# emilk/field_interpolation

Measured on NVIDIA B200. Metric: 3D SDF solve: lattice cells x CG iterations per second, higher is better.
Workload: dtype f32

## Files before the change

field_interpolation_b200/_lib.py:

```python
from __future__ import annotations

import ctypes as C
import os

HERE = os.path.dirname(os.path.abspath(__file__))
LIB_PATH = os.path.join(HERE, "libfi_b200.so")

FI_OK, FI_ERR_INVALID, FI_ERR_CUDA, FI_ERR_RANGE, FI_ERR_UNSUPPORTED, FI_ERR_COMM = range(6)
FI_HOST, FI_DEVICE = 0, 1
FI_F32, FI_F64, FI_MIXED = 0, 1, 2
FI_PRECOND_JACOBI, FI_PRECOND_MULTIGRID = 0, 1


class FiError(RuntimeError):
    def __init__(self, code, text):
        super().__init__(f"libfi_b200 status {code}: {text}")
        self.code = code


class fi_weights(C.Structure):
    _fields_ = [(n, C.c_float) for n in ("data_pos", "data_gradient", "model_0", "model_1", "model_2", "model_3",
                                         "model_4", "gradient_smoothness")] + [("value_kernel", C.c_int32),
                                                                               ("gradient_kernel", C.c_int32)]


class fi_triplet(C.Structure):
    _fields_ = [("row", C.c_int32), ("col", C.c_int32), ("value", C.c_float)]


class fi_solve_options(C.Structure):
    _fields_ = [("precision", C.c_int32), ("max_iterations", C.c_int32), ("tolerance", C.c_double),
                ("check_every", C.c_int32), ("use_fast_stencil", C.c_int32), ("refine_max_outer", C.c_int32),
                ("refine_inner_tolerance", C.c_double), ("preconditioner", C.c_int32), ("mg_smoothing_steps", C.c_int32),
                ("mg_cheb_ratio", C.c_double)]


class fi_solve_stats(C.Structure):
    _fields_ = [("iterations", C.c_int64), ("relative_residual", C.c_double), ("true_residual", C.c_double),
                ("initial_residual", C.c_double), ("setup_ms", C.c_double), ("solve_ms", C.c_double),
                ("converged", C.c_int32), ("outer_sweeps", C.c_int32), ("occupied_cells", C.c_int64),
                ("generic_rows", C.c_int64), ("widened_after", C.c_int64)]

    def as_dict(self):
        return {n: getattr(self, n) for n, _ in self._fields_}


class fi_cascade_options(C.Structure):
    _fields_ = [("fine", fi_solve_options), ("factor", C.c_int32), ("coarsest_size", C.c_int32),
                ("coarse_tolerance", C.c_double), ("max_levels", C.c_int32)]


class fi_cascade_stats(C.Structure):
    _fields_ = [("levels", C.c_int32), ("level_cells", C.c_int64 * 16), ("level_iterations", C.c_int64 * 16),
                ("level_ms", C.c_double * 16), ("level_initial_residual", C.c_double * 16), ("total_ms", C.c_double),
                ("cell_iterations", C.c_int64), ("finest", fi_solve_stats)]

    def as_dict(self):
        L = self.levels
        return {"levels": L, "level_cells": list(self.level_cells[:L]), "level_iterations": list(self.level_iterations[:L]),
                "level_ms": list(self.level_ms[:L]), "level_initial_residual": list(self.level_initial_residual[:L]),
                "total_ms": self.total_ms, "cell_iterations": self.cell_iterations, "finest": self.finest.as_dict()}


_p = C.POINTER
_vp, _i32, _i64, _f, _d = C.c_void_p, C.c_int32, C.c_int64, C.c_float, C.c_double
_pf, _pi32, _pi64, _pd = _p(C.c_float), _p(C.c_int32), _p(C.c_int64), _p(C.c_double)

SIGNATURES = {
    "fi_abi_version": (C.c_int, []),
    "fi_last_error": (C.c_char_p, []),
    "fi_device_count": (C.c_int, [_pi32]),
    "fi_set_device": (C.c_int, [_i32]),
    "fi_weights_default": (None, [_p(fi_weights)]),
    "fi_solve_options_default": (None, [_p(fi_solve_options)]),
    "fi_field_create": (C.c_int, [_i32, _pi32, _p(_vp)]),
    "fi_field_destroy": (C.c_int, [_vp]),
    "fi_field_clone": (C.c_int, [_vp, _p(_vp)]),
    "fi_field_add_model": (C.c_int, [_vp, _p(fi_weights)]),
    "fi_field_add_points": (C.c_int, [_vp, _f, _i32, _f, _i32, _i64, _vp, _vp, _vp, _vp, _i32, _pi64]),
    "fi_field_add_rows": (C.c_int, [_vp, _i64, _i64, _pi32, _pi32, _pf, _pf]),
    "fi_sdf_from_points": (C.c_int, [_i32, _pi32, _p(fi_weights), _i64, _vp, _vp, _vp, _i32, _p(_vp)]),
    "fi_field_counts": (C.c_int, [_vp, _pi64, _pi64]),
    "fi_field_export": (C.c_int, [_vp, _vp, _vp]),
    "fi_field_export_rows": (C.c_int, [_vp, _i64, _vp, _vp]),
    "fi_field_apply": (C.c_int, [_vp, _i32, _vp, _vp]),
    "fi_field_use_fast_stencil": (C.c_int, [_vp, _i32]),
    "fi_field_rhs": (C.c_int, [_vp, _i32, _vp]),
    "fi_field_diagonal": (C.c_int, [_vp, _i32, _vp]),
    "fi_field_solve": (C.c_int, [_vp, _p(fi_solve_options), _vp, _vp, _i32, _p(fi_solve_stats)]),
    "fi_field_solve_tiled": (C.c_int, [_vp, _p(fi_solve_options), _i32, _i32, _i32, _vp, _vp, _i32, _p(fi_solve_stats), _p(fi_solve_stats)]),
    "fi_field_jacobi": (C.c_int, [_vp, _pf, _i32, _f, _pf]),
    "fi_upscale_field": (C.c_int, [_i32, _pi32, _pi32, _vp, _vp, _i32]),
    "fi_error_map": (C.c_int, [_i64, _vp, _i64, _pf, _i64, _pf, _pf]),
    "fi_marching_squares": (C.c_int, [_i32, _i32, _vp, _f, _i32, _vp, _i64, _pi64, _pf]),
    "fi_calc_area": (C.c_int, [_i64, _vp, _i32, _pf]),
    "fi_bicubic_upsample": (C.c_int, [_i32, _i32, _vp, _i32, _vp, _i32]),
    "fi_sdf_solve_cascade": (C.c_int, [_i32, _pi32, _p(fi_weights), _i64, _vp, _vp, _vp, _p(fi_cascade_options), _vp, _i32,
                                       _p(fi_cascade_stats)]),
    "fi_comm_unique_id": (C.c_int, [_vp, _i64]),
    "fi_comm_create": (C.c_int, [_i32, _i32, _vp, _p(_vp)]),
    "fi_comm_destroy": (C.c_int, [_vp]),
    "fi_slab_balanced_cuts": (C.c_int, [_pi32, _i32, _i64, _vp, _i32, _d, _i32, _pi32]),
    "fi_comm_set_slab_cuts": (C.c_int, [_vp, _i32, _pi32]),
    "fi_slab_range": (C.c_int, [_i32, _i32, _i32, _pi32, _pi32]),
    "fi_slab_mg_plan": (C.c_int, [_pi32, _i32, _i32, _i64, _pi32, _pi32, _pi32, _pi32]),
    "fi_slab_sdf_solve": (C.c_int, [_vp, _pi32, _p(fi_weights), _i64, _vp, _vp, _vp, _i32, _p(fi_solve_options), _vp, _vp, _i32,
                                    _p(fi_solve_stats)]),
    "fi_trim_memory": (C.c_int, []),
    "fi_cached_bytes": (_i64, []),
    "fi_kernel_launches": (_i64, []),
    "fi_kernel_launches_reset": (None, []),
    "fi_field_time_iterations": (C.c_int, [_vp, _p(fi_solve_options), _i32, _pd]),
}

_dll = None


def lib():
    global _dll
    if _dll is None:
        if not os.path.exists(LIB_PATH):
            raise FiError(FI_ERR_CUDA, f"{LIB_PATH} not built; run python -m field_interpolation_b200.build "
                                       "(or __graft_entry__.build())")
        dll = C.CDLL(LIB_PATH)
        for name, (res, args) in SIGNATURES.items():
            fn = getattr(dll, name)
            fn.restype, fn.argtypes = res, args
        _dll = dll
    return _dll


def check(status):
    if status != FI_OK:
        raise FiError(status, lib().fi_last_error().decode("utf-8", "replace"))
```

field_interpolation_b200/api.py:

```python
from __future__ import annotations

import ctypes as C
import math
from dataclasses import dataclass, field as dc_field
from typing import Optional, Sequence

import numpy as np

from . import _lib as L
from ._lib import (FI_DEVICE, FI_F32, FI_F64, FI_HOST, FI_MIXED, FI_PRECOND_JACOBI, FI_PRECOND_MULTIGRID,
                   FiError)


class ValueKernel:
    kNearestNeighbor = 0
    kLinearInterpolation = 1


class GradientKernel:
    kNearestNeighbor = 0
    kCellEdges = 1
    kLinearInterpolation = 2


@dataclass
class Weights:
    data_pos: float = 1.0
    data_gradient: float = 1.0
    model_0: float = 0.0
    model_1: float = 0.0
    model_2: float = 0.5
    model_3: float = 0.0
    model_4: float = 0.0
    gradient_smoothness: float = 0.0
    value_kernel: int = ValueKernel.kLinearInterpolation
    gradient_kernel: int = GradientKernel.kCellEdges

    def c(self) -> L.fi_weights:
        return L.fi_weights(self.data_pos, self.data_gradient, self.model_0, self.model_1, self.model_2, self.model_3,
                            self.model_4, self.gradient_smoothness, int(self.value_kernel), int(self.gradient_kernel))


@dataclass
class SolveOptions:
    tile: bool = False
    tile_size: int = 16
    cg: bool = True
    max_iterations: int = 0
    error_tolerance: float = 1e-3


@dataclass
class LinearEquation:
    rows: np.ndarray
    cols: np.ndarray
    vals: np.ndarray
    rhs: np.ndarray

    @property
    def num_rows(self):
        return int(self.rhs.shape[0])

    @property
    def num_triplets(self):
        return int(self.vals.shape[0])


def _is_device(a) -> bool:
    return hasattr(a, "data_ptr") and bool(getattr(a, "is_cuda", False))


def _f32_host(a):
    return np.ascontiguousarray(a, dtype=np.float32)


class _Buf:

    def __init__(self, a, n_expected: Optional[int] = None):
        self.keep, self.ptr, self.loc = None, None, None
        if a is None:
            return
        if _is_device(a):
            import torch
            assert a.dtype == torch.float32 and a.is_contiguous(), "device inputs must be contiguous float32"
            self.keep, self.ptr, self.loc, n = a, C.c_void_p(a.data_ptr()), FI_DEVICE, a.numel()
        else:
            h = _f32_host(a)
            self.keep, self.ptr, self.loc, n = h, C.c_void_p(h.ctypes.data), FI_HOST, h.size
        if n_expected is not None and n != n_expected:
            raise ValueError(f"expected {n_expected} floats, got {n}")


def _common_loc(bufs):
    locs = {b.loc for b in bufs if b.loc is not None}
    if len(locs) > 1:
        raise ValueError("all point arrays must live in the same place (all host or all device)")
    return locs.pop() if locs else FI_HOST


def solve_options(precision=FI_F32, max_iterations=0, tolerance=1e-3, check_every=32, use_fast_stencil=True,
                  refine_max_outer=20, refine_inner_tolerance=1e-3, preconditioner=FI_PRECOND_JACOBI, mg_smoothing_steps=0,
                  mg_cheb_ratio=12.0) -> L.fi_solve_options:
    return L.fi_solve_options(int(precision), int(max_iterations), float(tolerance), int(check_every),
                              int(use_fast_stencil), int(refine_max_outer), float(refine_inner_tolerance), int(preconditioner),
                              int(mg_smoothing_steps), float(mg_cheb_ratio))


class LatticeField:

    def __init__(self, sizes: Sequence[int], _handle=None):
        self.sizes = [int(s) for s in sizes]
        self.strides = []
        s = 1
        for n in self.sizes:
            self.strides.append(s)
            s *= n
        self.num_unknowns = s
        if _handle is None:
            h = C.c_void_p()
            sz = (C.c_int32 * len(self.sizes))(*self.sizes)
            L.check(L.lib().fi_field_create(len(self.sizes), sz, C.byref(h)))
            _handle = h
        self._h = _handle

    def num_dim(self):
        return len(self.sizes)

    def close(self):
        if getattr(self, "_h", None):
            L.lib().fi_field_destroy(self._h)
            self._h = None

    def __del__(self):
        try:
            self.close()
        except Exception:
            pass

    def counts(self):
        r, t = C.c_int64(0), C.c_int64(0)
        L.check(L.lib().fi_field_counts(self._h, C.byref(r), C.byref(t)))
        return int(r.value), int(t.value)

    @property
    def eq(self) -> LinearEquation:
        nr, nt = self.counts()
        trips = np.empty(nt, dtype=np.dtype([("row", np.int32), ("col", np.int32), ("value", np.float32)]))
        rhs = np.empty(nr, np.float32)
        L.check(L.lib().fi_field_export(self._h, C.c_void_p(trips.ctypes.data), C.c_void_p(rhs.ctypes.data)))
        return LinearEquation(trips["row"].copy(), trips["col"].copy(), trips["value"].copy(), rhs)

    def _vec(self, fn, precision):
        out = np.empty(self.num_unknowns, np.float32 if precision == FI_F32 else np.float64)
        L.check(fn(self._h, precision, C.c_void_p(out.ctypes.data)))
        return out

    def rhs(self, precision=FI_F64):
        return self._vec(L.lib().fi_field_rhs, precision)

    def diagonal(self, precision=FI_F64):
        return self._vec(L.lib().fi_field_diagonal, precision)

    def use_fast_stencil(self, mode):
        L.check(L.lib().fi_field_use_fast_stencil(self._h, int(mode)))

    def apply(self, x, precision=FI_F64):
        dt = np.float32 if precision == FI_F32 else np.float64
        xi = np.ascontiguousarray(x, dtype=dt)
        assert xi.size == self.num_unknowns
        y = np.empty_like(xi)
        L.check(L.lib().fi_field_apply(self._h, precision, C.c_void_p(xi.ctypes.data), C.c_void_p(y.ctypes.data)))
        return y

    def solve(self, options: Optional[L.fi_solve_options] = None, guess=None, out=None):
        opt = options if options is not None else solve_options()
        g = _Buf(guess, self.num_unknowns)
        if out is None:
            if g.loc == FI_DEVICE:
                import torch
                out = torch.empty(self.num_unknowns, dtype=torch.float32, device=guess.device)
            else:
                out = np.empty(self.num_unknowns, np.float32)
        o = _Buf(out, self.num_unknowns)
        if g.loc is not None and g.loc != o.loc:
            raise ValueError("guess and out must live in the same place")
        st = L.fi_solve_stats()
        L.check(L.lib().fi_field_solve(self._h, C.byref(opt), g.ptr, o.ptr, o.loc, C.byref(st)))
        return (out if _is_device(out) else o.keep), st.as_dict()

    def time_iterations(self, iterations: int, options: Optional[L.fi_solve_options] = None):
        opt = options if options is not None else solve_options()
        ms = (C.c_double * 8)()
        L.check(L.lib().fi_field_time_iterations(self._h, C.byref(opt), int(iterations), ms))
        return {"iteration_ms": ms[0], "apply_ms": ms[1], "update_ms": ms[2], "direction_ms": ms[3], "fused": bool(ms[4]),
                "stencil_ms": ms[5], "data_term_ms": ms[6]}



def add_field_constraints(field: LatticeField, weights: Weights) -> None:
    w = weights.c()
    L.check(L.lib().fi_field_add_model(field._h, C.byref(w)))


def add_points(field: LatticeField, value_weight: float, value_kernel: int, gradient_weight: float, gradient_kernel: int,
               positions, normals=None, point_weights=None, values=None) -> int:
    D = field.num_dim()
    p = _Buf(positions)
    n = (p.keep.numel() if p.loc == FI_DEVICE else p.keep.size) // D if p.keep is not None else 0
    nr, pw, va = _Buf(normals, n * D if normals is not None else None), _Buf(point_weights, n if point_weights is not None else None), _Buf(values, n if values is not None else None)
    loc = _common_loc([p, nr, pw, va])
    added = C.c_int64(0)
    L.check(L.lib().fi_field_add_points(field._h, float(value_weight), int(value_kernel), float(gradient_weight),
                                        int(gradient_kernel), n, p.ptr, nr.ptr, pw.ptr, va.ptr, loc, C.byref(added)))
    return int(added.value)


def add_value_constraint(field: LatticeField, pos, value: float, weight: float) -> bool:
    return add_points(field, weight, ValueKernel.kLinearInterpolation, 0.0, GradientKernel.kCellEdges,
                      np.asarray(pos, np.float32).reshape(1, -1), None, None, np.asarray([value], np.float32)) > 0


def _round_half_away(x: float) -> int:
    return int(math.floor(abs(x) + 0.5) * (1 if x >= 0 else -1))


def add_value_constraint_nearest_neighbor(field: LatticeField, pos, gradient, value: float, weight: float) -> bool:
    p = np.asarray(pos, np.float32).reshape(-1)
    inside = all(0 <= _round_half_away(float(p[d])) < field.sizes[d] for d in range(field.num_dim()))
    if not inside:
        return False
    add_points(field, weight, ValueKernel.kNearestNeighbor, 0.0, GradientKernel.kCellEdges, p.reshape(1, -1),
               np.asarray(gradient, np.float32).reshape(1, -1), None, np.asarray([value], np.float32))
    return True


def add_gradient_constraint(field: LatticeField, pos, gradient, weight: float, kernel: int) -> bool:
    if kernel not in (0, 1, 2):
        raise FiError(L.FI_ERR_INVALID, f"Unknown gradient kernel: {kernel}")
    return add_points(field, 0.0, ValueKernel.kLinearInterpolation, weight, kernel,
                      np.asarray(pos, np.float32).reshape(1, -1), np.asarray(gradient, np.float32).reshape(1, -1)) > 0


def add_equation(field: LatticeField, weight: float, rhs: float, pairs) -> None:
    w = np.float32(weight)
    if w == 0:
        return
    cols = [int(c) for c, v in pairs if np.float32(v) != 0]
    vals = np.array([np.float32(v) * w for c, v in pairs if np.float32(v) != 0], np.float32)
    if not cols:
        return
    r = np.zeros(len(cols), np.int32)
    c = np.asarray(cols, np.int32)
    b = np.array([np.float32(rhs) * w], np.float32)
    L.check(L.lib().fi_field_add_rows(field._h, 1, len(cols), r.ctypes.data_as(L._pi32), c.ctypes.data_as(L._pi32),
                                      vals.ctypes.data_as(L._pf), b.ctypes.data_as(L._pf)))


def add_rows(field: LatticeField, trip_row, trip_col, trip_val, rhs) -> None:
    r, c = np.ascontiguousarray(trip_row, np.int32), np.ascontiguousarray(trip_col, np.int32)
    v, b = _f32_host(trip_val), _f32_host(rhs)
    L.check(L.lib().fi_field_add_rows(field._h, b.size, v.size, r.ctypes.data_as(L._pi32), c.ctypes.data_as(L._pi32),
                                      v.ctypes.data_as(L._pf), b.ctypes.data_as(L._pf)))


def sdf_from_points(sizes: Sequence[int], weights: Weights, positions, normals=None, point_weights=None) -> LatticeField:
    D = len(sizes)
    p = _Buf(positions)
    if p.keep is None:
        raise FiError(L.FI_ERR_INVALID, "positions is null")
    n = (p.keep.numel() if p.loc == FI_DEVICE else p.keep.size) // D
    nr, pw = _Buf(normals, n * D if normals is not None else None), _Buf(point_weights, n if point_weights is not None else None)
    loc = _common_loc([p, nr, pw])
    h = C.c_void_p()
    sz = (C.c_int32 * D)(*[int(s) for s in sizes])
    w = weights.c()
    L.check(L.lib().fi_sdf_from_points(D, sz, C.byref(w), n, p.ptr, nr.ptr, pw.ptr, loc, C.byref(h)))
    return LatticeField(sizes, _handle=h)


def upscale_field(small_field, small_sizes: Sequence[int], large_sizes: Sequence[int]):
    D = len(small_sizes)
    ss, ls = (C.c_int32 * D)(*map(int, small_sizes)), (C.c_int32 * D)(*map(int, large_sizes))
    src = _Buf(small_field, int(np.prod(small_sizes, dtype=np.int64)))
    nl = int(np.prod(large_sizes, dtype=np.int64))
    if src.loc == FI_DEVICE:
        import torch
        out = torch.empty(nl, dtype=torch.float32, device=small_field.device)
        dst = C.c_void_p(out.data_ptr())
    else:
        out = np.empty(nl, np.float32)
        dst = C.c_void_p(out.ctypes.data)
    L.check(L.lib().fi_upscale_field(D, ss, ls, src.ptr, dst, src.loc))
    return out


def _field_2d(values):
    shape = tuple(values.shape)
    if len(shape) != 2:
        raise ValueError("a 2D (height, width) field is expected")
    if _is_device(values):
        values = values.contiguous()
    return _Buf(values, shape[0] * shape[1]), int(shape[0]), int(shape[1])


def iso_surface(values, iso: float = 0.0, want_area: bool = False):
    buf, h, w = _field_2d(values)
    n = C.c_int64(0)
    L.check(L.lib().fi_marching_squares(w, h, buf.ptr, float(iso), buf.loc, None, 0, C.byref(n), None))
    ns = int(n.value)
    area = C.c_float(0.0)
    if buf.loc == FI_DEVICE:
        import torch
        out = torch.empty((ns, 4), dtype=torch.float32, device=values.device)
        dst = C.c_void_p(out.data_ptr()) if ns else None
# ... 113 lines not shown
```

field_interpolation_b200/csrc/abi.cu:

```cuda
#include <time.h>

#include <algorithm>
#include <cmath>
#include <cstdlib>
#include <exception>
#include <map>
#include <mutex>
#include <new>

#include "solver.hpp"

namespace fi {

int64_t                   g_launches = 0;
static thread_local std::string t_last_error;

void set_last_error(const std::string& s) { t_last_error = s; }

int sm_count()
{
	static thread_local int cached_dev = -1, cached = 0;
	int dev = 0;
	if (cudaGetDevice(&dev) != cudaSuccess) { return 148; }
	if (dev != cached_dev) {
// ... 697 lines not shown
}

int fi_field_counts(fi_field* f, int64_t* num_rows, int64_t* num_triplets)
{
	return guarded([&] {
		FI_REQUIRE(f != nullptr, FI_ERR_INVALID, "field is null");
		int64_t r = 0, t = 0;
		for (Segment& sg : f->segs) {
			segment_counts(f, sg);
			r += sg.rows;
			t += sg.trips;
		}
		if (num_rows) { *num_rows = r; }
		if (num_triplets) { *num_triplets = t; }
	});
}

static void export_impl(fi_field* f, int64_t row_begin, fi_triplet* triplets, float* rhs)
{
	FI_REQUIRE(f != nullptr, FI_ERR_INVALID, "field is null");
	FI_REQUIRE(row_begin >= 0, FI_ERR_INVALID, "negative row_begin");
	int64_t R = 0, T = 0;
	for (Segment& sg : f->segs) {
		segment_counts(f, sg);
		R += sg.rows;
		T += sg.trips;
	}
	FI_REQUIRE(R <= INT32_MAX && T <= INT32_MAX && f->g.N <= INT32_MAX, FI_ERR_RANGE,
	           "system does not fit the reference's int32 triplet view");
	size_t  first = 0;
	int64_t row_base = 0, trip_base = 0;
	while (first < f->segs.size() && row_base < row_begin) {
		row_base += f->segs[first].rows;
		trip_base += f->segs[first].trips;
		++first;
	}
	FI_REQUIRE(row_base == row_begin || (first == f->segs.size() && row_begin == R), FI_ERR_INVALID,
	           "row_begin is not a boundary between builder calls");
	const int64_t outR = R - row_base, outT = T - trip_base;
	if (outR == 0 && outT == 0) { return; }
	FI_REQUIRE((triplets || outT == 0) && (rhs || outR == 0), FI_ERR_INVALID, "output buffers are null");
	cudaStream_t       s = f->stream;
	DevBuf<fi_triplet> d_trips(std::max<int64_t>(outT, 1));
	DevBuf<float>      d_rhs(std::max<int64_t>(outR, 1));
	const int64_t      row0 = row_base, trip0 = trip_base;
	fi_triplet*        dt = d_trips.data() - trip0;
	float*             dr = d_rhs.data() - row0;
	for (size_t k = first; k < f->segs.size(); ++k) {
		Segment& sg = f->segs[k];
		if (sg.kind == Segment::kModel) {
			DevBuf<uint64_t> ro(f->g.N), to(f->g.N);
			uint64_t         hr = 0, ht = 0;
			count_model_rows(f->g, sg.w, ro.data(), to.data(), &hr, &ht, s);
			FI_REQUIRE(static_cast<int64_t>(hr) == sg.rows && static_cast<int64_t>(ht) == sg.trips, FI_ERR_INVALID,
			           "internal: model row count mismatch");
			emit_model_rows(f->g, sg.w, ro.data(), to.data(), row_base, trip_base, dt, dr, s);
			FI_CUDA(cudaStreamSynchronize(s));
		} else if (sg.kind == Segment::kPoints) {
			const int64_t    n = sg.p1 - sg.p0;
			DevBuf<uint64_t> ro(std::max<int64_t>(n, 1)), to(std::max<int64_t>(n, 1));
			uint64_t         hr = 0, ht = 0;
			count_point_rows(f->g, view(f->pts), sg.p0, sg.p1, ro.data(), to.data(), &hr, &ht, s);
			emit_point_rows(f->g, view(f->pts), sg.p0, sg.p1, ro.data(), to.data(), row_base, trip_base, dt, dr, s);
			FI_CUDA(cudaStreamSynchronize(s));
		} else {
			std::vector<fi_triplet> ht(static_cast<size_t>(sg.trips));
			size_t                  at = 0;
			for (int64_t r = sg.r0; r < sg.r1; ++r) {
				for (uint64_t kk = f->rows.ptr[r]; kk < f->rows.ptr[r + 1]; ++kk) {
					ht[at++] = fi_triplet{static_cast<int32_t>(row_base + (r - sg.r0)), f->rows.col[kk], f->rows.val[kk]};
				}
			}
			if (!ht.empty()) {
				FI_CUDA(cudaMemcpyAsync(dt + trip_base, ht.data(), ht.size() * sizeof(fi_triplet), cudaMemcpyHostToDevice, s));
			}
			if (sg.rows > 0) {
				FI_CUDA(cudaMemcpyAsync(dr + row_base, f->rows.rhs.data() + sg.r0, sg.rows * sizeof(float), cudaMemcpyHostToDevice, s));
			}
			FI_CUDA(cudaStreamSynchronize(s));
		}
		row_base += sg.rows;
		trip_base += sg.trips;
	}
	if (outT > 0) { FI_CUDA(cudaMemcpyAsync(triplets, d_trips.data(), outT * sizeof(fi_triplet), cudaMemcpyDeviceToHost, s)); }
	if (outR > 0) { FI_CUDA(cudaMemcpyAsync(rhs, d_rhs.data(), outR * sizeof(float), cudaMemcpyDeviceToHost, s)); }
	FI_CUDA(cudaStreamSynchronize(s));
}

int fi_field_export(fi_field* f, fi_triplet* triplets, float* rhs)
{
	return guarded([&] { export_impl(f, 0, triplets, rhs); });
}

int fi_field_export_rows(fi_field* f, int64_t row_begin, fi_triplet* triplets, float* rhs)
{
	return guarded([&] { export_impl(f, row_begin, triplets, rhs); });
}

int fi_field_use_fast_stencil(fi_field* f, int32_t enable)
{
	return guarded([&] {
		FI_REQUIRE(f != nullptr, FI_ERR_INVALID, "field is null");
		f->fast = enable;
	});
}

int fi_field_apply(fi_field* f, int32_t precision, const void* x, void* y)
{
	return guarded([&] {
		FI_REQUIRE(f && x && y, FI_ERR_INVALID, "null argument");
		const int64_t N = f->g.N;
		cudaStream_t  s = f->stream;
		if (precision == FI_F32) {
			Operator<float>& op = f->get32();
			op.use_fast = f->fast;
			DevBuf<float>    dx(N), dy(N);
			FI_CUDA(cudaMemcpyAsync(dx.data(), x, N * sizeof(float), cudaMemcpyHostToDevice, s));
			op.apply(dx.data(), dy.data(), nullptr, nullptr, s);
			FI_CUDA(cudaMemcpyAsync(y, dy.data(), N * sizeof(float), cudaMemcpyDeviceToHost, s));
		} else if (precision == FI_F64) {
			Operator<double>& op = f->get64();
			op.use_fast = f->fast;
			DevBuf<double>    dx(N), dy(N);
			FI_CUDA(cudaMemcpyAsync(dx.data(), x, N * sizeof(double), cudaMemcpyHostToDevice, s));
			op.apply(dx.data(), dy.data(), nullptr, nullptr, s);
			FI_CUDA(cudaMemcpyAsync(y, dy.data(), N * sizeof(double), cudaMemcpyDeviceToHost, s));
		} else {
			throw Error{FI_ERR_INVALID, "precision must be FI_F32 or FI_F64"};
		}
		FI_CUDA(cudaStreamSynchronize(s));
	});
}

static int copy_vector(fi_field* f, int32_t precision, void* out, int which)
{
	return guarded([&] {
		FI_REQUIRE(f && out, FI_ERR_INVALID, "null argument");
		const int64_t N = f->g.N;
		if (precision == FI_F32) {
			Operator<float>& op = f->get32();
			FI_CUDA(cudaMemcpy(out, which == 0 ? op.atb.data() : op.diag.data(), N * sizeof(float), cudaMemcpyDeviceToHost));
		} else if (precision == FI_F64) {
			Operator<double>& op = f->get64();
			FI_CUDA(cudaMemcpy(out, which == 0 ? op.atb.data() : op.diag.data(), N * sizeof(double), cudaMemcpyDeviceToHost));
		} else {
			throw Error{FI_ERR_INVALID, "precision must be FI_F32 or FI_F64"};
		}
	});
}

int fi_field_rhs(fi_field* f, int32_t precision, void* atb) { return copy_vector(f, precision, atb, 0); }
int fi_field_diagonal(fi_field* f, int32_t precision, void* diag) { return copy_vector(f, precision, diag, 1); }

int fi_field_solve(fi_field* f, const fi_solve_options* opt, const float* guess, float* solution, int32_t loc, fi_solve_stats* stats)
{
	return guarded([&] {
		TraceScope trace("fi_field_solve");
		FI_REQUIRE(f && solution, FI_ERR_INVALID, "null argument");
		fi_solve_options o;
		if (opt) { o = *opt; } else { fi_solve_options_default(&o); }
		const int64_t N = f->g.N;
		if (loc == FI_DEVICE) {
			FI_REQUIRE((reinterpret_cast<uintptr_t>(solution) & 15u) == 0 && (reinterpret_cast<uintptr_t>(guess) & 15u) == 0, FI_ERR_INVALID,
			           "FI_DEVICE solution / guess buffers must be 16-byte aligned");
			solve_device(f, o, guess, solution, stats);
		} else {
			DevBuf<float> d(N);
			if (guess) { FI_CUDA(cudaMemcpyAsync(d.data(), guess, N * sizeof(float), cudaMemcpyHostToDevice, f->stream)); }
			solve_device(f, o, guess ? d.data() : nullptr, d.data(), stats);
			FI_CUDA(cudaMemcpyAsync(solution, d.data(), N * sizeof(float), cudaMemcpyDeviceToHost, f->stream));
			FI_CUDA(cudaStreamSynchronize(f->stream));
		}
	});
}

int fi_field_solve_tiled(fi_field* f, const fi_solve_options* opt, int32_t tile, int32_t tile_size, int32_t cg, const float* guess,
                         float* solution, int32_t loc, fi_solve_stats* stats, fi_solve_stats* tile_stats)
{
	return guarded([&] {
		TraceScope trace("fi_field_solve_tiled");
		FI_REQUIRE(f && solution, FI_ERR_INVALID, "null argument");
		FI_REQUIRE(guess != nullptr, FI_ERR_INVALID, "incomplete guess");
		fi_solve_options o;
		if (opt) { o = *opt; } else { fi_solve_options_default(&o); }
		FI_REQUIRE(o.precision == FI_F32 || o.precision == FI_F64 || o.precision == FI_MIXED, FI_ERR_INVALID, "unknown precision");
		const int64_t N = f->g.N;
		cudaStream_t  s = f->stream;
		DevBuf<float> staged;
		float*        d_x = solution;
		if (loc == FI_DEVICE) {
			FI_REQUIRE((reinterpret_cast<uintptr_t>(solution) & 15u) == 0, FI_ERR_INVALID, "FI_DEVICE solution buffer must be 16-byte aligned");
			if (guess != solution) { FI_CUDA(cudaMemcpyAsync(solution, guess, N * sizeof(float), cudaMemcpyDeviceToDevice, s)); }
		} else {
			staged.resize(N);
			d_x = staged.data();
			FI_CUDA(cudaMemcpyAsync(d_x, guess, N * sizeof(float), cudaMemcpyHostToDevice, s));
		}
		if (stats) { std::memset(stats, 0, sizeof(*stats)); }
		if (tile_stats) { std::memset(tile_stats, 0, sizeof(*tile_stats)); }
		if (tile) {
			if (o.precision == FI_F32) {
				const bool       fresh = !f->op32;
				Operator<float>& op    = f->get32();
				op.use_fast            = o.use_fast_stencil;
				const PcgResult r      = tile_phase<float>(op, tile_size, d_x, 1e-6, 0, o.check_every, s);
				fill_stats(tile_stats, r, fresh ? op.setup_ms : 0.0, op.data.nocc, op.data.nrows);
			} else {
				const bool        fresh = !f->op64;
				Operator<double>& op    = f->get64();
				op.use_fast             = o.use_fast_stencil;
				DevBuf<double> x(N);
				convert(d_x, x.data(), N, s);
				const PcgResult r = tile_phase<double>(op, tile_size, x.data(), 1e-12, 0, o.check_every, s);
				convert(x.data(), d_x, N, s);
				fill_stats(tile_stats, r, fresh ? op.setup_ms : 0.0, op.data.nocc, op.data.nrows);
			}
		}
		if (cg) { solve_device(f, o, d_x, d_x, stats); }
		if (loc != FI_DEVICE) { FI_CUDA(cudaMemcpyAsync(solution, d_x, N * sizeof(float), cudaMemcpyDeviceToHost, s)); }
		FI_CUDA(cudaStreamSynchronize(s));
	});
}

int fi_field_jacobi(fi_field* f, const float* guess, int32_t num_iterations, float weight, float* solution)
{
	return guarded([&] {
		FI_REQUIRE(f && guess && solution, FI_ERR_INVALID, "null argument");
		const int64_t N = f->g.N;
		if (num_iterations <= 0) {
			if (solution != guess) { std::memcpy(solution, guess, N * sizeof(float)); }
			return;
		}
		Operator<float>& op = f->get32();
		DevBuf<float>    x(N);
		FI_CUDA(cudaMemcpyAsync(x.data(), guess, N * sizeof(float), cudaMemcpyHostToDevice, f->stream));
		jacobi_sweeps<float>(op, x.data(), num_iterations, weight, f->stream);
		FI_CUDA(cudaMemcpyAsync(solution, x.data(), N * sizeof(float), cudaMemcpyDeviceToHost, f->stream));
		FI_CUDA(cudaStreamSynchronize(f->stream));
	});
}

int fi_upscale_field(int32_t ndim, const int32_t* small_sizes, const int32_t* large_sizes, const float* small_field,
                     float* large_field, int32_t loc)
{
	return guarded([&] {
		FI_REQUIRE(1 <= ndim && ndim <= kMaxDim, FI_ERR_INVALID, "ndim must be 1..3");
		FI_REQUIRE(small_sizes && large_sizes && small_field && large_field, FI_ERR_INVALID, "null argument");
		for (int d = 0; d < ndim; ++d) { FI_REQUIRE(small_sizes[d] >= 1 && large_sizes[d] >= 1, FI_ERR_INVALID, "size must be >= 1"); }
		const Geom gs = make_geom(ndim, small_sizes), gl = make_geom(ndim, large_sizes);
		if (loc == FI_DEVICE) {
			upscale_device(gs, gl, small_field, large_field, 1.0f, nullptr);
			FI_CUDA(cudaStreamSynchronize(nullptr));
		} else {
			DevBuf<float> a(gs.N), b(gl.N);
			FI_CUDA(cudaMemcpy(a.data(), small_field, gs.N * sizeof(float), cudaMemcpyHostToDevice));
			upscale_device(gs, gl, a.data(), b.data(), 1.0f, nullptr);
			FI_CUDA(cudaMemcpy(large_field, b.data(), gl.N * sizeof(float), cudaMemcpyDeviceToHost));
		}
	});
}

int fi_error_map(int64_t num_triplets, const fi_triplet* triplets, int64_t num_columns, const float* solution, int64_t num_rows,
                 const float* rhs, float* heatmap)
{
	return guarded([&] {
		FI_REQUIRE(num_triplets >= 0 && num_columns >= 0 && num_rows >= 0, FI_ERR_INVALID, "negative count");
		FI_REQUIRE((triplets || num_triplets == 0) && (solution || num_columns == 0) && (rhs || num_rows == 0) && (heatmap || num_columns == 0),
		           FI_ERR_INVALID, "null argument");
		error_map(num_triplets, triplets, num_columns, solution, num_rows, rhs, heatmap);
	});
}

int fi_marching_squares(int32_t width, int32_t height, const float* values, float iso, int32_t loc, float* lines, int64_t capacity_segments,
                        int64_t* num_segments, float* area)
{
	return guarded([&] {
		FI_REQUIRE(width >= 1 && height >= 1 && values && num_segments, FI_ERR_INVALID, "marching squares: bad argument");
		FI_REQUIRE(lines == nullptr || capacity_segments >= 0, FI_ERR_INVALID, "marching squares: negative capacity");
		*num_segments = 0;
		if (area) { *area = 0.0f; }
		cudaStream_t  s = nullptr;
		Staged<float> v(values, static_cast<size_t>(width) * height, loc, s);
		const int64_t n = marching_squares_device(width, height, v.ptr, iso, nullptr, 0, s);
		*num_segments   = n;
		FI_REQUIRE(lines == nullptr || n <= capacity_segments, FI_ERR_RANGE, "marching squares: segment buffer too small");
		if (n == 0 || (lines == nullptr && area == nullptr)) { return; }
		DevBuf<float> own;
		float*        d_lines = lines;
		if (lines == nullptr || loc != FI_DEVICE) {
			own.resize(static_cast<size_t>(n) * 4);
			d_lines = own.data();
		}
		marching_squares_device(width, height, v.ptr, iso, d_lines, n, s);
		if (area) { *area = static_cast<float>(area_twice_device(n, d_lines, s) / 2); }
		if (lines && loc != FI_DEVICE) { FI_CUDA(cudaMemcpy(lines, d_lines, static_cast<size_t>(n) * 4 * sizeof(float), cudaMemcpyDeviceToHost)); }
	});
}

int fi_calc_area(int64_t num_segments, const float* lines, int32_t loc, float* area)
{
	return guarded([&] {
		FI_REQUIRE(num_segments >= 0 && area && (lines || num_segments == 0), FI_ERR_INVALID, "calc_area: bad argument");
		cudaStream_t  s = nullptr;
		Staged<float> l(lines, static_cast<size_t>(num_segments) * 4, loc, s);
		*area = static_cast<float>(area_twice_device(num_segments, l.ptr, s) / 2);
	});
// ... 216 lines not shown
```

field_interpolation_b200/csrc/internal.hpp:

```cpp
#pragma once

#include <memory>

#include "common.cuh"

namespace fi {

struct Geom
{
	int     ndim = 0;
	int     size[kMaxDim]   = {1, 1, 1};
	int64_t stride[kMaxDim] = {1, 1, 1};
	int64_t N = 1;
	int     zoff = 0;
	int     nzl = 1;
	int     zown0 = 0, zown1 = 1;
	int64_t shift = 0;
	int     tile = 0;
	float   tile_reg = 0.0f;

	__host__ __device__ bool sharded() const { return zown0 != 0 || zown1 != nzl; }
	__host__ __device__ int64_t own_offset() const { return static_cast<int64_t>(zown0) * (ndim == 3 ? stride[2] : 0); }
	__host__ __device__ int64_t own_cells() const { return ndim == 3 ? static_cast<int64_t>(zown1 - zown0) * stride[2] : N; }
};

__host__ __device__ inline int64_t tile_of_node(const Geom& g, int64_t index)
{
	int64_t t = 0, ts = 1;
	for (int d = 0; d < g.ndim; ++d) {
		const int c = static_cast<int>(index % g.size[d]);
		index /= g.size[d];
		t += static_cast<int64_t>(c / g.tile) * ts;
		ts *= (g.size[d] + g.tile - 1) / g.tile;
	}
	return t;
}

inline Geom make_geom(int ndim, const int32_t* sizes)
{
	Geom g;
	g.ndim    = ndim;
	int64_t s = 1;
	for (int d = 0; d < ndim; ++d) {
		g.size[d]   = sizes[d];
		g.stride[d] = s;
		s *= sizes[d];
	}
	g.N = s;
	g.nzl   = ndim == 3 ? sizes[2] : 1;
	g.zown1 = g.nzl;
	return g;
}

inline Geom make_slab_geom(const int32_t* sizes, int z0, int z1, int halo)
{
	Geom g  = make_geom(3, sizes);
	g.zoff  = z0 - halo;
	g.nzl   = (z1 - z0) + 2 * halo;
	g.zown0 = halo;
	g.zown1 = halo + (z1 - z0);
	g.shift = -g.stride[2] * g.zoff;
	g.N     = g.stride[2] * g.nzl;
	return g;
}

struct PointStore
{
	DevBuf<float>   pos, grad;
	DevBuf<float>   value, vw, gw;
	DevBuf<uint8_t> kind;
	int64_t         count = 0;
};

struct PointView
{
	const float *  pos, *grad, *value, *vw, *gw;
	const uint8_t* kind;
};

inline PointView view(const PointStore& s)
{
	return PointView{s.pos.data(), s.grad.data(), s.value.data(), s.vw.data(), s.gw.data(), s.kind.data()};
}

void exclusive_scan_u64(const uint64_t* in, uint64_t* out, int64_t n, uint64_t* total_dev, cudaStream_t s);
void radix_sort_pairs(DevBuf<uint64_t>& keys, DevBuf<uint32_t>& vals, int64_t n, int bits, cudaStream_t s);

void canonicalise_points(const Geom& g, PointStore& store, float value_weight, int value_kernel, float gradient_weight,
                         int gradient_kernel, int64_t n, const float* d_pos, const float* d_nrm, const float* d_pw,
                         const float* d_val, cudaStream_t s);
void count_point_rows(const Geom& g, PointView pv, int64_t p0, int64_t p1, uint64_t* d_rowoff, uint64_t* d_tripoff,
                      uint64_t* h_rows, uint64_t* h_trips, cudaStream_t s);
void emit_point_rows(const Geom& g, PointView pv, int64_t p0, int64_t p1, const uint64_t* d_rowoff,
                     const uint64_t* d_tripoff, int64_t row_base, int64_t trip_base, fi_triplet* d_trips, float* d_rhs,
                     cudaStream_t s);
void count_model_rows(const Geom& g, const fi_weights& w, uint64_t* d_rowoff, uint64_t* d_tripoff, uint64_t* h_rows,
                      uint64_t* h_trips, cudaStream_t s);
void emit_model_rows(const Geom& g, const fi_weights& w, const uint64_t* d_rowoff, const uint64_t* d_tripoff,
                     int64_t row_base, int64_t trip_base, fi_triplet* d_trips, float* d_rhs, cudaStream_t s);
void upscale_device(const Geom& small, const Geom& large, const float* d_small, float* d_large, float post_scale,
                    cudaStream_t s);

template <typename T>
struct DataTerm
{
	int64_t            nocc = 0;
	DevBuf<uint64_t>   cell_key;
	DevBuf<int64_t>    cell_base;
	DevBuf<uint32_t>   cell_mask;
	DevBuf<T>          blocks;
	int64_t            nnode = 0;
	DevBuf<int64_t>    node_index;
	DevBuf<T>          node_coef;
	int64_t            nrows = 0;
	DevBuf<uint64_t>   row_ptr;
	DevBuf<int32_t>    col;
	DevBuf<float>      val;
	DevBuf<double>     partial;
	DevBuf<unsigned>   ticket;
};

struct HostRows
{
	std::vector<uint64_t> ptr{0};
	std::vector<int32_t>  col;
	std::vector<float>    val, rhs;
	int64_t rows() const { return static_cast<int64_t>(rhs.size()); }
};

template <typename T>
void build_data_term(const Geom& g, const PointStore& pts, const HostRows& user_rows, DataTerm<T>& out, T* d_atb,
                     T* d_diag, cudaStream_t s);

struct PeerPublish;
template <typename T>
bool apply_data_term(const Geom& g, const DataTerm<T>& dt, const T* p, T* q, double* d_dot_accum, const int* d_done,
                     cudaStream_t s, const PeerPublish* pub = nullptr);

template <typename T>
bool apply_data_term_epilogue(const Geom& g, const DataTerm<T>& dt, const T* in, T* res_out, const T* minv, T* e, T* d_new, T b,
                              cudaStream_t s);

void error_map(int64_t nt, const fi_triplet* h_trips, int64_t n, const float* h_x, int64_t nrows, const float* h_rhs, float* h_out);

int64_t marching_squares_device(int width, int height, const float* d_values, float iso, float* d_lines, int64_t capacity, cudaStream_t s);
double  area_twice_device(int64_t nseg, const float* d_lines, cudaStream_t s);
void    bicubic_upsample_device(int width, int height, const float* d_values, int upsample, float* d_large, cudaStream_t s);

struct StencilTables
{
	double band[kMaxDim][9][9];
	double gs2;
	int    radius;
	bool   any;
};

struct ModelAccum
{
	double cc[5][5][5] = {};
	bool   on[5]       = {false, false, false, false, false};
	double gs_sq       = 0;
};

StencilTables make_tables(const Geom& g, const ModelAccum& m);

template <typename T>
void stencil_diagonal(const Geom& g, const StencilTables& t, T* d_diag , T* d_minv , cudaStream_t s);

enum StencilMode { kStencilGeneric = 0, kStencilAuto = 1, kStencilTiled = 2 };
template <typename T>
void stencil_apply(const Geom& g, const StencilTables& t, const T* p, T* q, double* d_dot_out, double* d_partial,
                   unsigned* d_ticket, const int* d_done, int mode, cudaStream_t s);
int stencil_partial_slots(const Geom& g);

void     slab_range(int nz, int world, int rank, int* z0, int* z1);
void     comm_slab_range(const fi_comm* c, int nz, int rank, int* z0, int* z1);
const int* comm_cuts(const fi_comm* c, int nz);
void     comm_set_cuts(fi_comm* c, int nz, const int32_t* cuts);
void     balanced_cuts(const int32_t* sizes, int world, int64_t num_points, const float* positions, int loc, double point_weight, int min_planes,
                       int32_t* cuts);
void     comm_unique_id(void* id, int64_t capacity);
fi_comm* comm_create(int rank, int world, const void* id);
void     comm_destroy(fi_comm* c);
void     slab_sdf_solve(fi_comm* c, const int32_t* sizes, const fi_weights& w, int64_t num_points, const float* positions, const float* normals,
                        const float* point_weights, int loc, const fi_solve_options& o, const float* guess_own, float* solution_own,
                        int sol_loc, fi_solve_stats* st);

}
```

field_interpolation_b200/csrc/solver.cu:

```cuda
#include "solver.hpp"

#include <algorithm>
#include <cmath>
#include <cstdlib>

namespace fi {

namespace {

constexpr int kThreads = 256;

int vec_grid(int64_t n)
{
	const int64_t want = (n + kThreads - 1) / kThreads;
	return static_cast<int>(std::max<int64_t>(1, std::min<int64_t>(want, static_cast<int64_t>(sm_count()) * 8)));
}

template <typename T>
struct Pack;
template <>
struct Pack<float>
{
	using type = float4;
	static constexpr int V = 4;
};
template <>
struct Pack<double>
{
	using type = double2;
	static constexpr int V = 2;
};

template <typename T, typename F>
__device__ __forceinline__ void for_each_pack(int64_t n, F&& f)
{
	constexpr int V      = Pack<T>::V;
	const int64_t npacks = n / V;
	const int64_t stride = static_cast<int64_t>(gridDim.x) * blockDim.x;
	for (int64_t k = static_cast<int64_t>(blockIdx.x) * blockDim.x + threadIdx.x; k < npacks; k += stride) { f(k, true); }
	if (blockIdx.x == 0) {
		for (int64_t i = npacks * V + threadIdx.x; i < n; i += blockDim.x) { f(i, false); }
	}
}

template <typename T, typename F>
__device__ __forceinline__ void for_each_pack_blocked(int64_t n, int64_t* first, int64_t* last, F&& f)
{
	constexpr int V      = Pack<T>::V;
	const int64_t npacks = n / V;
	const int64_t chunk  = (npacks + gridDim.x - 1) / gridDim.x;
	const int64_t k0 = static_cast<int64_t>(blockIdx.x) * chunk, k1 = min(k0 + chunk, npacks);
	for (int64_t k = k0 + threadIdx.x; k < k1; k += blockDim.x) { f(k, true); }
	*first = k0 * V;
	*last  = k1 * V;
	if (blockIdx.x == gridDim.x - 1) {
		for (int64_t i = npacks * V + threadIdx.x; i < n; i += blockDim.x) { f(i, false); }
		*last = n;
	}
}

template <typename T>
__global__ void __launch_bounds__(kThreads) pcg_init_kernel(int64_t n, const T* __restrict__ b, const T* __restrict__ q,
                                                            const T* __restrict__ minv, T* __restrict__ r, T* __restrict__ p,
                                                            PcgState* st, double tol, long long max_iters, double* partial,
                                                            unsigned* ticket, int dist)
{
	__shared__ double red[32];
	double            acc[3] = {0, 0, 0};
	const int64_t     stride = static_cast<int64_t>(gridDim.x) * blockDim.x;
	for (int64_t i = static_cast<int64_t>(blockIdx.x) * blockDim.x + threadIdx.x; i < n; i += stride) {
		const T bi = b[i], ri = q ? bi - q[i] : bi, zi = minv[i] * ri;
		r[i] = ri;
		p[i] = zi;
		acc[0] += static_cast<double>(ri) * static_cast<double>(zi);
		acc[1] += static_cast<double>(ri) * static_cast<double>(ri);
		acc[2] += static_cast<double>(bi) * static_cast<double>(bi);
	}
	acc[0] = block_sum(acc[0], red);
	acc[1] = block_sum(acc[1], red);
	acc[2] = block_sum(acc[2], red);
	grid_sum<3>(acc, partial, ticket, red, [&](const double(&tot)[3]) {
		if (dist) {
			st->part[0] = tot[0];
			st->part[1] = tot[1];
			st->part[2] = tot[2];
			return;
		}
		st->rho[0]    = tot[0];
		st->rho[1]    = 0;
		st->pq        = 0;
		st->rr        = tot[1];
		st->rr0       = tot[1];
		st->bb        = tot[2];
		st->tol2bb    = tol * tol * tot[2];
		st->iters     = 0;
		st->max_iters = max_iters;
		st->breakdown = 0;
		st->done      = (tot[2] == 0.0 || tot[1] <= tol * tol * tot[2] || max_iters <= 0) ? 1 : 0;
	});
}

__global__ void peer_publish_kernel(PeerLink L, int which, int par, unsigned long long base, const PcgState* st, const double* src, int count,
                                    const int* done)
{
	if (blockIdx.x != 0 || threadIdx.x >= 32) { return; }
	const unsigned long long seq = seq_of(base, st, which);
	double v[2] = {0.0, 0.0};
	if (!(done && *done)) {
		for (int k = 0; k < count; ++k) { v[k] = src[k]; }
		if (threadIdx.x == 0) { L.local->stamp[0][st->iters & 511] = global_ns(); }
	}
	peer_publish_warp(L, which, par, seq, v, count);
}

__global__ void pcg_update_finish_peer_kernel(PcgState* st, int par, PeerLink L, unsigned long long base)
{
	if (blockIdx.x != 0 || threadIdx.x >= 32) { return; }
	const unsigned long long seq = seq_of(base, st, 1);
	double tot[2];
	const bool ok = peer_collect_warp(L, 1, par, seq, tot, 2);
	if (threadIdx.x != 0 || st->done) { return; }
	if (!ok) {
		st->breakdown = 2;
		st->done      = 1;
		return;
	}
	L.local->stamp[2][st->iters & 511] = global_ns();
	st->rho[par ^ 1] = tot[0];
	st->rr           = tot[1];
	st->iters += 1;
	if (tot[1] <= st->tol2bb || st->iters >= st->max_iters || !(tot[0] > 0.0)) { st->done = 1; }
}

__global__ void pcg_init_finish_kernel(PcgState* st, double tol, long long max_iters)
{
	const double rho = st->part[0], rr = st->part[1], bb = st->part[2];
	st->rho[0]    = rho;
	st->rho[1]    = 0;
	st->pq        = 0;
	st->rr        = rr;
	st->rr0       = rr;
	st->bb        = bb;
	st->tol2bb    = tol * tol * bb;
	st->iters     = 0;
	st->max_iters = max_iters;
	st->breakdown = 0;
	st->done      = (bb == 0.0 || rr <= tol * tol * bb || max_iters <= 0) ? 1 : 0;
}

__global__ void pcg_update_finish_kernel(PcgState* st, int par)
{
	if (st->done) { return; }
	const double rho = st->part[0], rr = st->part[1];
	st->rho[par ^ 1] = rho;
	st->rr           = rr;
	st->iters += 1;
	if (rr <= st->tol2bb || st->iters >= st->max_iters || !(rho > 0.0)) { st->done = 1; }
}

enum XMode { kXClassic = 0, kXSkip = 1, kXBoth = 2 };

template <typename T, int XM, bool PACKED>
__device__ __forceinline__ void update_elements(int64_t k, T* __restrict__ x, T* __restrict__ r, const T* __restrict__ p, const T* __restrict__ p_prev,
                                                const T* __restrict__ q, const T* __restrict__ minv, T alpha, T alpha_prev, double (&acc)[2],
                                                typename Pack<T>::type* r_out)
{
	using P         = typename Pack<T>::type;
	constexpr int V = PACKED ? Pack<T>::V : 1;
	T xa[V], ra[V], pa[V], ppa[V], qa[V], ma[V];
	if (PACKED) {
		*reinterpret_cast<P*>(ra) = reinterpret_cast<const P*>(r)[k];
		*reinterpret_cast<P*>(qa) = reinterpret_cast<const P*>(q)[k];
		*reinterpret_cast<P*>(ma) = reinterpret_cast<const P*>(minv)[k];
		if (XM != kXSkip) {
			*reinterpret_cast<P*>(xa) = reinterpret_cast<const P*>(x)[k];
			*reinterpret_cast<P*>(pa) = reinterpret_cast<const P*>(p)[k];
		}
		if (XM == kXBoth) { *reinterpret_cast<P*>(ppa) = reinterpret_cast<const P*>(p_prev)[k]; }
	} else {
		ra[0] = r[k];
		qa[0] = q[k];
		ma[0] = minv[k];
		if (XM != kXSkip) {
			xa[0] = x[k];
			pa[0] = p[k];
		}
		if (XM == kXBoth) { ppa[0] = p_prev[k]; }
	}
#pragma unroll
	for (int j = 0; j < V; ++j) {
		if (XM == kXClassic) { xa[j] += alpha * pa[j]; }
		if (XM == kXBoth) { xa[j] += alpha_prev * ppa[j] + alpha * pa[j]; }
		ra[j] -= alpha * qa[j];
		const double rd = static_cast<double>(ra[j]);
		acc[0] += rd * static_cast<double>(ma[j] * ra[j]);
		acc[1] += rd * rd;
	}
	if (PACKED) {
		if (XM != kXSkip) { reinterpret_cast<P*>(x)[k] = *reinterpret_cast<const P*>(xa); }
		reinterpret_cast<P*>(r)[k] = *reinterpret_cast<const P*>(ra);
		if (r_out) { *r_out = *reinterpret_cast<const P*>(ra); }
	} else {
		if (XM != kXSkip) { x[k] = xa[0]; }
		r[k] = ra[0];
		if (r_out) { reinterpret_cast<T*>(r_out)[0] = ra[0]; }
	}
}

template <typename T, int XM>
__global__ void __launch_bounds__(kThreads) pcg_update_kernel(int64_t n, T* __restrict__ x, T* __restrict__ r,
                                                              const T* __restrict__ p, const T* __restrict__ p_prev, const T* __restrict__ q,
                                                              const T* __restrict__ minv, PcgState* st, int par,
                                                              double* partial, unsigned* ticket, int dist)
{
	__shared__ double red[32];
	if (st->done) { return; }
	const double pq = st->pq;
	if (!(pq > 0.0)) {
		if (blockIdx.x == 0 && threadIdx.x == 0) {
			st->breakdown = 1;
			st->done      = 1;
		}
		return;
	}
	const double alpha_d = st->rho[par] / pq;
	const T      alpha = static_cast<T>(alpha_d), alpha_prev = XM == kXBoth ? static_cast<T>(st->alpha_prev) : T(0);
	double acc[2] = {0, 0};
	for_each_pack<T>(n, [&](int64_t k, bool packed) {
		if (packed) {
			update_elements<T, XM, true>(k, x, r, p, p_prev, q, minv, alpha, alpha_prev, acc, nullptr);
		} else {
			update_elements<T, XM, false>(k, x, r, p, p_prev, q, minv, alpha, alpha_prev, acc, nullptr);
		}
	});
	acc[0] = block_sum(acc[0], red);
	acc[1] = block_sum(acc[1], red);
	grid_sum<2>(acc, partial, ticket, red, [&](const double(&tot)[2]) {
		if (XM == kXSkip) { st->alpha_prev = alpha_d; }
		if (dist) {
			st->part[0] = tot[0];
			st->part[1] = tot[1];
			return;
		}
		st->rho[par ^ 1] = tot[0];
		st->rr           = tot[1];
		st->iters += 1;
		if (tot[1] <= st->tol2bb || st->iters >= st->max_iters || !(tot[0] > 0.0)) { st->done = 1; }
	});
}

template <typename T, int XM>
__global__ void __launch_bounds__(kThreads) pcg_update_peer_kernel(int64_t n, T* __restrict__ x, T* __restrict__ r,
                                                                   const T* __restrict__ p, const T* __restrict__ p_prev, const T* __restrict__ q,
                                                                   const T* __restrict__ minv, PcgState* st, int par, double* partial,
                                                                   unsigned* ticket, PeerLink L, HaloPush<T> push, unsigned long long base, int fold,
                                                                   int blocked)
{
	__shared__ double red[32];
	__shared__ double s_pq, s_tot[2];
	__shared__ int    s_ok, s_pub;
	const bool was_done = st->done != 0;
	const unsigned long long seq_pq = seq_of(base, st, 0), seq_rr = seq_of(base, st, 1);
	if ((fold & 1) && blockIdx.x == 0 && threadIdx.x < 32) {
		double mine[1] = {was_done ? 0.0 : st->pq};
		if (threadIdx.x == 0 && !was_done) { L.local->stamp[0][st->iters & 511] = global_ns(); }
		peer_publish_warp(L, 0, par, seq_pq, mine, 1);
	}
	if (threadIdx.x < 32) {
		double     pq = 0.0;
		const bool ok = peer_collect_warp(L, 0, par, seq_pq, &pq, 1);
		if (threadIdx.x == 0) {
			s_ok  = ok ? 1 : 0;
			s_pq  = pq;
			s_pub = 0;
			if (blockIdx.x == 0 && !was_done) { L.local->stamp[1][st->iters & 511] = global_ns(); }
		}
	}
	__syncthreads();
	const double pq    = s_pq;
	const bool   bad   = !s_ok || !(pq > 0.0);
	double       acc[2] = {0, 0};
	const double alpha_d = (!was_done && !bad) ? st->rho[par] / pq : 0.0;
	bool         pushed  = false;
	if (!was_done && !bad) {
		const T alpha = static_cast<T>(alpha_d), alpha_prev = XM == kXBoth ? static_cast<T>(st->alpha_prev) : T(0);
		using P       = typename Pack<T>::type;
		constexpr int V = Pack<T>::V;
		const int64_t hi_from = n - push.count;
		auto element = [&](int64_t k, bool packed) {
			if (packed) {
				P rv;
				update_elements<T, XM, true>(k, x, r, p, p_prev, q, minv, alpha, alpha_prev, acc, &rv);
				const int64_t i = k * V;
				if (push.lo && i < push.count) { *reinterpret_cast<P*>(push.lo + i) = rv; }
				if (push.hi && i >= hi_from) { *reinterpret_cast<P*>(push.hi + (i - hi_from)) = rv; }
			} else {
				P rv;
				update_elements<T, XM, false>(k, x, r, p, p_prev, q, minv, alpha, alpha_prev, acc, &rv);
				const T ri = reinterpret_cast<const T*>(&rv)[0];
				if (push.lo && k < push.count) { push.lo[k] = ri; }
				if (push.hi && k >= hi_from) { push.hi[k - hi_from] = ri; }
			}
		};
		if (blocked) {
			int64_t first = 0, last = 0;
			for_each_pack_blocked<T>(n, &first, &last, element);
			pushed = (push.lo && first < push.count) || (push.hi && last > hi_from);
		} else {
			for_each_pack<T>(n, element);
			pushed = push.lo != nullptr || push.hi != nullptr;
		}
	}
	acc[0] = block_sum(acc[0], red);
	acc[1] = block_sum(acc[1], red);
	if (threadIdx.x == 0 && pushed) { __threadfence_system(); }
	grid_sum<2>(acc, partial, ticket, red, [&](const double(&tot)[2]) {
		if (!was_done && bad) {
			st->breakdown = s_ok ? 1 : 2;
			st->done      = 1;
		}
		if (XM == kXSkip && !was_done && !bad) { st->alpha_prev = alpha_d; }
		s_tot[0] = tot[0];
		s_tot[1] = tot[1];
		s_pub    = 1;
	});
	__syncthreads();
	if (s_pub && threadIdx.x < 32) {
		const double tot[2] = {s_tot[0], s_tot[1]};
		peer_publish_warp(L, 1, par, seq_rr, tot, 2);
		if (fold & 2) {
			double     all[2];
			const bool ok = peer_collect_warp(L, 1, par, seq_rr, all, 2);
			if (threadIdx.x == 0 && !st->done) {
				if (!ok) {
					st->breakdown = 2;
					st->done      = 1;
				} else {
					L.local->stamp[2][st->iters & 511] = global_ns();
					st->rho[par ^ 1] = all[0];
					st->rr           = all[1];
					st->iters += 1;
					if (all[1] <= st->tol2bb || st->iters >= st->max_iters || !(all[0] > 0.0)) { st->done = 1; }
				}
			}
		}
	}
}

template <typename T>
__global__ void __launch_bounds__(kThreads) pcg_direction_kernel(int64_t n, const T* __restrict__ r, const T* __restrict__ minv,
                                                                 T* __restrict__ p, const PcgState* st, int par)
{
	if (st->done) { return; }
	const T beta  = static_cast<T>(st->rho[par ^ 1] / st->rho[par]);
	using P       = typename Pack<T>::type;
	constexpr int V = Pack<T>::V;
	for_each_pack<T>(n, [&](int64_t k, bool packed) {
		if (packed) {
			const P  rv = reinterpret_cast<const P*>(r)[k], mv = reinterpret_cast<const P*>(minv)[k];
			P        pv = reinterpret_cast<P*>(p)[k];
			const T* ra = reinterpret_cast<const T*>(&rv);
			const T* ma = reinterpret_cast<const T*>(&mv);
			T*       pa = reinterpret_cast<T*>(&pv);
#pragma unroll
			for (int j = 0; j < V; ++j) { pa[j] = ma[j] * ra[j] + beta * pa[j]; }
			reinterpret_cast<P*>(p)[k] = pv;
		} else {
			p[k] = minv[k] * r[k] + beta * p[k];
		}
	});
}

template <typename T>
__global__ void __launch_bounds__(kThreads) residual_kernel(int64_t n, const T* __restrict__ b, const T* __restrict__ q, T* __restrict__ r,
                                                            double* out, double* partial, unsigned* ticket)
{
	__shared__ double red[32];
	double            acc[2] = {0, 0};
	const int64_t     stride = static_cast<int64_t>(gridDim.x) * blockDim.x;
	for (int64_t i = static_cast<int64_t>(blockIdx.x) * blockDim.x + threadIdx.x; i < n; i += stride) {
		const T bi = b[i], ri = bi - q[i];
		if (r) { r[i] = ri; }
		acc[0] += static_cast<double>(ri) * static_cast<double>(ri);
		acc[1] += static_cast<double>(bi) * static_cast<double>(bi);
	}
	acc[0] = block_sum(acc[0], red);
	acc[1] = block_sum(acc[1], red);
	grid_sum<2>(acc, partial, ticket, red, [&](const double(&tot)[2]) {
		out[0] = tot[0];
		out[1] = tot[1];
	});
}

template <typename T>
__global__ void jacobi_kernel(int64_t n, const T* __restrict__ atb, const T* __restrict__ q, const T* __restrict__ diag, T* __restrict__ x, T w)
{
	const int64_t stride = static_cast<int64_t>(gridDim.x) * blockDim.x;
	for (int64_t i = static_cast<int64_t>(blockIdx.x) * blockDim.x + threadIdx.x; i < n; i += stride) {
		const T temp = atb[i] - (q[i] - diag[i] * x[i]);
		x[i]         = w * temp / diag[i] + (T(1) - w) * x[i];
	}
}

template <typename A, typename B>
__global__ void convert_kernel(int64_t n, const A* __restrict__ a, B* __restrict__ b)
{
	const int64_t stride = static_cast<int64_t>(gridDim.x) * blockDim.x;
	for (int64_t i = static_cast<int64_t>(blockIdx.x) * blockDim.x + threadIdx.x; i < n; i += stride) { b[i] = static_cast<B>(a[i]); }
}

__global__ void add_f32_f64_kernel(int64_t n, const float* __restrict__ e, double* __restrict__ x)
{
	const int64_t stride = static_cast<int64_t>(gridDim.x) * blockDim.x;
	for (int64_t i = static_cast<int64_t>(blockIdx.x) * blockDim.x + threadIdx.x; i < n; i += stride) { x[i] += static_cast<double>(e[i]); }
}

template <typename T>
__global__ void __launch_bounds__(kThreads) pcg_flush_x_kernel(int64_t n, T* __restrict__ x, const T* __restrict__ p, const PcgState* st)
{
	const T       a      = static_cast<T>(st->alpha_prev);
	const int64_t stride = static_cast<int64_t>(gridDim.x) * blockDim.x;
	for (int64_t i = static_cast<int64_t>(blockIdx.x) * blockDim.x + threadIdx.x; i < n; i += stride) { x[i] += a * p[i]; }
}

template <typename T>
void ensure_work(Operator<T>& op, cudaStream_t s)
{
	PcgWork<T>& w = op.work;
	const size_t n = static_cast<size_t>(op.g.N);
	if (w.r.size() != n) {
		w.r.resize(n);
		w.p.resize(n);
		w.q.resize(n);
		w.p2.resize(n);
		w.p.zero(s);
		w.p2.zero(s);
		if (op.g.sharded()) {
			w.r.zero(s);
			w.q.zero(s);
		}
		w.partial.resize(static_cast<size_t>(3) * (static_cast<size_t>(sm_count()) * 8 + 8));
		w.ticket.resize(1);
		w.state.resize(1);
		w.ticket.zero(s);
	}
}

}

void convert(const float* src, double* dst, int64_t n, cudaStream_t s)
{
	auto kern = convert_kernel<float, double>;
	FI_LAUNCH(kern, vec_grid(n), kThreads, 0, s, n, src, dst);
}
void convert(const double* src, float* dst, int64_t n, cudaStream_t s)
{
	auto kern = convert_kernel<double, float>;
	FI_LAUNCH(kern, vec_grid(n), kThreads, 0, s, n, src, dst);
}
void axpy_f32_into_f64(const float* e, double* x, int64_t n, cudaStream_t s)
{
	FI_LAUNCH(add_f32_f64_kernel, vec_grid(n), kThreads, 0, s, n, e, x);
}

template <typename T>
std::unique_ptr<Operator<T>> build_operator(const Geom& g, const ModelAccum& m, const PointStore& pts, const HostRows& rows,
                                            cudaStream_t s)
{
	TraceScope  trace("build_operator (data term, diagonal, preconditioner)");
	cudaEvent_t e0, e1;
	FI_CUDA(cudaEventCreate(&e0));
	FI_CUDA(cudaEventCreate(&e1));
	FI_CUDA(cudaEventRecord(e0, s));
	auto op  = std::make_unique<Operator<T>>();
	op->g    = g;
	op->tabs = make_tables(g, m);
	op->atb.resize(g.N);
	op->diag.resize(g.N);
	op->minv.resize(g.N);
	op->atb.zero(s);
	op->diag.zero(s);
	build_data_term<T>(g, pts, rows, op->data, op->atb.data(), op->diag.data(), s);
	stencil_diagonal<T>(g, op->tabs, op->diag.data(), op->minv.data(), s);
	op->partial.resize(static_cast<size_t>(stencil_partial_slots(g)));
	op->ticket.resize(1);
	op->ticket.zero(s);
	FI_CUDA(cudaEventRecord(e1, s));
	FI_CUDA(cudaEventSynchronize(e1));
	float ms = 0;
	FI_CUDA(cudaEventElapsedTime(&ms, e0, e1));
	op->setup_ms = ms;
	cudaEventDestroy(e0);
	cudaEventDestroy(e1);
	return op;
}

template <typename T>
void residual(Operator<T>& op, const T* b, const T* x, T* r, double* rr, double* bb, cudaStream_t s)
{
	ensure_work(op, s);
	PcgWork<T>&   w   = op.work;
	const int64_t off = op.g.own_offset(), n = op.g.own_cells();
	if (op.dist) { op.dist->exchange_halo(const_cast<T*>(x), sizeof(T), s); }
	op.apply(x, w.q.data(), nullptr, nullptr, s);
	DevBuf<double> out(2);
	auto kern = residual_kernel<T>;
	FI_LAUNCH(kern, vec_grid(n), kThreads, 0, s, n, (b ? b : op.atb.data()) + off, w.q.data() + off, r ? r + off : nullptr, out.data(),
	          w.partial.data(), w.ticket.data());
	if (op.dist) { op.dist->allreduce(out.data(), 2, s); }
	double h[2];
	FI_CUDA(cudaMemcpyAsync(h, out.data(), sizeof(h), cudaMemcpyDeviceToHost, s));
	FI_CUDA(cudaStreamSynchronize(s));
	*rr = h[0];
	*bb = h[1];
}

template <typename T>
PcgResult pcg_solve(Operator<T>& op, const T* b, T* x, double tol, long long max_iter, int check_every, bool want_true_residual,
                    cudaStream_t s)
{
	TraceScope trace("pcg_solve");
	ensure_work(op, s);
	PcgWork<T>&   w = op.work;
	const int64_t off = op.g.own_offset(), n = op.g.own_cells();
	DistHooks*    dist = op.dist;
	const T*      rhs = b ? b : op.atb.data();
	if (max_iter <= 0) {
		max_iter = 2 * static_cast<long long>(op.g.size[0]) * op.g.size[1] * op.g.size[2];
	}
	if (!(tol > 0)) { tol = std::is_same<T, float>::value ? 1.1920929e-07 : 2.220446049250313e-16; }
	check_every = std::max(2, check_every <= 0 ? 32 : check_every);
	check_every += check_every & 1;

	cudaEvent_t e0, e1;
	FI_CUDA(cudaEventCreate(&e0));
	FI_CUDA(cudaEventCreate(&e1));
	FI_CUDA(cudaEventRecord(e0, s));

	const int grid = vec_grid(n);
	const PeerLink* link = dist ? dist->link() : nullptr;
	T*              r_vec = w.r.data();
	HaloPush<T>     push;
	if (link) {
		void *lo = nullptr, *hi = nullptr;
		r_vec = static_cast<T*>(dist->shared_vector(static_cast<size_t>(op.g.N) * sizeof(T), &lo, &hi, s));
		const int64_t plane = op.g.stride[2], halo = op.g.zown0;
		push.count = halo * plane;
		if (lo) { push.lo = static_cast<T*>(lo) + halo * plane + dist->peer_own_cells(link->rank - 1); }
		if (hi) { push.hi = static_cast<T*>(hi); }
	}
	const bool zero_guess = op.guess_is_zero;
	op.guess_is_zero      = false;
	if (!zero_guess) {
		if (dist) { dist->exchange_halo(x, sizeof(T), s); }
		op.apply(x, w.q.data(), nullptr, nullptr, s);
	}
	{
		auto kern = pcg_init_kernel<T>;
		FI_LAUNCH(kern, grid, kThreads, 0, s, n, rhs + off, zero_guess ? static_cast<const T*>(nullptr) : w.q.data() + off, op.minv.data() + off, r_vec + off, w.p.data() + off,
		          w.state.data(), tol, max_iter, w.partial.data(), w.ticket.data(), dist ? 1 : 0);
		if (dist) {
			dist->allreduce(w.state.data()->part, 3, s);
			FI_LAUNCH(pcg_init_finish_kernel, 1, 1, 0, s, w.state.data(), tol, max_iter);
			dist->exchange_halo(r_vec, sizeof(T), s);
		}
	}
	PcgState h;
	FI_CUDA(cudaMemcpyAsync(&h, w.state.data(), sizeof(h), cudaMemcpyDeviceToHost, s));
	FI_CUDA(cudaStreamSynchronize(s));

	PcgResult res;
	res.zero_rhs         = (h.bb == 0.0);
	res.initial_residual = h.bb > 0 ? std::sqrt(h.rr0 / h.bb) : 0.0;
	if (res.zero_rhs) {
		FI_CUDA(cudaMemsetAsync(x + off, 0, n * sizeof(T), s));
	} else if (!h.done) {
		const int* d_done = &w.state.data()->done;
		double*    d_pq   = &w.state.data()->pq;
		T*   pp[2] = {w.p.data(), w.p2.data()};
		const unsigned long long seq_base = link ? (dist->next_seq() << 40) : 0ull;
		const char* fold_env  = std::getenv("FI_B200_PEER_FOLD");
		const int   fold_mode = !link ? 0 : (fold_env && *fold_env >= '0' && *fold_env <= '3' ? *fold_env - '0' : 2);
		const bool  data_publishes = fold_mode >= 2, update_finishes = fold_mode == 1 || fold_mode == 2;
		const char* walk_env = std::getenv("FI_B200_PEER_UPDATE");
		const bool  peer_update_blocked = walk_env ? walk_env[0] == 'b' : n < (48ll << 20);
		bool deferred_x = false;
		auto enqueue_round = [&] {
			for (int it = 0; it < check_every; ++it) {
				const int par = it & 1;
				const bool fused = stencil_fused_step<T>(op.use_fast, op.g, op.tabs, r_vec, op.minv.data(), pp[par], pp[par ^ 1], w.q.data(),
				                                         w.state.data(), par, d_pq, op.partial.data(), op.ticket.data(), d_done, s);
				deferred_x = deferred_x || fused;
				if (fused && link) {
					PeerPublish pub;
					pub.link  = *link;
					pub.which = 0;
					pub.par   = par;
					pub.base  = seq_base;
					pub.st    = w.state.data();
					const bool published = apply_data_term<T>(op.g, op.data, pp[par ^ 1], w.q.data(), d_pq, d_done, s, data_publishes ? &pub : nullptr);
					const bool in_update = fold_mode == 1;
					if (!published && !in_update) { FI_LAUNCH(peer_publish_kernel, 1, 32, 0, s, *link, 0, par, seq_base, w.state.data(), d_pq, 1, d_done); }
					auto ku = par == 0 ? pcg_update_peer_kernel<T, kXSkip> : pcg_update_peer_kernel<T, kXBoth>;
					FI_LAUNCH(ku, grid, kThreads, 0, s, n, x + off, r_vec + off, pp[par ^ 1] + off, pp[par] + off, w.q.data() + off, op.minv.data() + off,
					          w.state.data(), par, w.partial.data(), w.ticket.data(), *link, push, seq_base, (in_update ? 1 : 0) | (update_finishes ? 2 : 0),
					          peer_update_blocked ? 1 : 0);
					if (!update_finishes) { FI_LAUNCH(pcg_update_finish_peer_kernel, 1, 32, 0, s, w.state.data(), par, *link, seq_base); }
				} else if (fused) {
					apply_data_term<T>(op.g, op.data, pp[par ^ 1], w.q.data(), d_pq, d_done, s);
					if (dist) { dist->allreduce(d_pq, 1, s); }
					auto ku = par == 0 ? pcg_update_kernel<T, kXSkip> : pcg_update_kernel<T, kXBoth>;
					FI_LAUNCH(ku, grid, kThreads, 0, s, n, x + off, r_vec + off, pp[par ^ 1] + off, pp[par] + off, w.q.data() + off, op.minv.data() + off,
					          w.state.data(), par, w.partial.data(), w.ticket.data(), dist ? 1 : 0);
					if (dist) {
						dist->allreduce(w.state.data()->part, 2, s);
						FI_LAUNCH(pcg_update_finish_kernel, 1, 1, 0, s, w.state.data(), par);
						dist->exchange_halo(r_vec, sizeof(T), s);
					}
				} else {
					FI_REQUIRE(dist == nullptr, FI_ERR_UNSUPPORTED, "a slab-sharded solve needs the fused 3D stencil kernel");
					op.apply(w.p.data(), w.q.data(), d_pq, d_done, s);
					auto ku = pcg_update_kernel<T, kXClassic>;
					FI_LAUNCH(ku, grid, kThreads, 0, s, n, x, w.r.data(), w.p.data(), static_cast<const T*>(nullptr), w.q.data(), op.minv.data(), w.state.data(), par,
					          w.partial.data(), w.ticket.data(), 0);
					auto kd = pcg_direction_kernel<T>;
					FI_LAUNCH(kd, grid, kThreads, 0, s, n, w.r.data(), op.minv.data(), w.p.data(), w.state.data(), par);
				}
			}
		};
		cudaEvent_t l0, l1;
		FI_CUDA(cudaEventCreate(&l0));
		FI_CUDA(cudaEventCreate(&l1));
		if (dist && !link) {
			TraceScope trl("iteration loop (direct launches)");
			FI_CUDA(cudaEventRecord(l0, s));
			while (true) {
				enqueue_round();
				FI_CUDA(cudaMemcpyAsync(&h, w.state.data(), sizeof(h), cudaMemcpyDeviceToHost, s));
				FI_CUDA(cudaStreamSynchronize(s));
				if (h.done) { break; }
			}
		} else {
			cudaGraph_t     graph = nullptr;
			cudaGraphExec_t exec  = nullptr;
			const int64_t   before = g_launches;
			FI_CUDA(cudaStreamBeginCapture(s, cudaStreamCaptureModeThreadLocal));
			try {
				enqueue_round();
			} catch (...) {
				cudaStreamEndCapture(s, &graph);
				if (graph) { cudaGraphDestroy(graph); }
				throw;
			}
			FI_CUDA(cudaStreamEndCapture(s, &graph));
			const int64_t per_graph = g_launches - before;
			g_launches              = before;
			{
				TraceScope tr("cudaGraphInstantiate");
				FI_CUDA(cudaGraphInstantiate(&exec, graph, 0));
			}
			TraceScope trl("iteration loop (graph launches)");
			FI_CUDA(cudaEventRecord(l0, s));
			while (true) {
				FI_CUDA(cudaGraphLaunch(exec, s));
				count_launch(static_cast<int>(per_graph));
				FI_CUDA(cudaMemcpyAsync(&h, w.state.data(), sizeof(h), cudaMemcpyDeviceToHost, s));
				FI_CUDA(cudaStreamSynchronize(s));
				if (h.done) { break; }
			}
			cudaGraphExecDestroy(exec);
			cudaGraphDestroy(graph);
		}
		if (deferred_x && (h.iters & 1)) {
			auto kf = pcg_flush_x_kernel<T>;
			FI_LAUNCH(kf, grid, kThreads, 0, s, n, x + off, static_cast<const T*>(pp[1] + off), static_cast<const PcgState*>(w.state.data()));
		}
		FI_CUDA(cudaEventRecord(l1, s));
		FI_CUDA(cudaEventSynchronize(l1));
		if (link && trace_enabled() && h.iters >= 8) {
			std::vector<unsigned long long> st3(3 * 512);
			FI_CUDA(cudaMemcpy(st3.data(), link->local->stamp, sizeof(unsigned long long) * 3 * 512, cudaMemcpyDeviceToHost));
			const long long last = h.iters - 1, first = std::max<long long>(1, h.iters - 400);
			double a = 0, b = 0, c = 0;
			for (long long k = first; k <= last; ++k) {
				a += static_cast<double>(st3[0 * 512 + (k & 511)] - st3[2 * 512 + ((k - 1) & 511)]);
				b += static_cast<double>(st3[1 * 512 + (k & 511)] - st3[0 * 512 + (k & 511)]);
				c += static_cast<double>(st3[2 * 512 + (k & 511)] - st3[1 * 512 + (k & 511)]);
			}
			const double cnt = static_cast<double>(last - first + 1) * 1e3;
			fprintf(stderr, "[fi_b200] rank %d per-iteration us: stencil+data %.1f | wait p.Ap %.1f | update+wait r.r %.1f\n", link->rank, a / cnt,
			        b / cnt, c / cnt);
		}
		float lms = 0;
		FI_CUDA(cudaEventElapsedTime(&lms, l0, l1));
		res.loop_ms = lms;
		cudaEventDestroy(l0);
		cudaEventDestroy(l1);
	}
	FI_CUDA(cudaEventRecord(e1, s));
	FI_CUDA(cudaEventSynchronize(e1));
	float ms = 0;
	FI_CUDA(cudaEventElapsedTime(&ms, e0, e1));
	cudaEventDestroy(e0);
	cudaEventDestroy(e1);

	res.solve_ms     = ms;
	res.iterations   = h.iters;
	res.rel_residual = h.bb > 0 ? std::sqrt(h.rr / h.bb) : 0.0;
	res.converged    = res.zero_rhs || (h.rr <= h.tol2bb);
	res.true_residual = res.rel_residual;
	if (want_true_residual && !res.zero_rhs) {
		double rr = 0, bb = 0;
		residual<T>(op, rhs, x, nullptr, &rr, &bb, s);
		res.true_residual = bb > 0 ? std::sqrt(rr / bb) : 0.0;
		const bool recurrence_met = res.converged;
		res.converged             = res.true_residual <= kConvergedSlack * tol;
		res.stalled               = (recurrence_met && !res.converged) || h.breakdown != 0;
	}
	return res;
}

template <typename T>
void jacobi_sweeps(Operator<T>& op, T* x, int iterations, T weight, cudaStream_t s)
{
	ensure_work(op, s);
	PcgWork<T>& w = op.work;
	for (int it = 0; it < iterations; ++it) {
		op.apply(x, w.q.data(), nullptr, nullptr, s);
		auto kern = jacobi_kernel<T>;
		FI_LAUNCH(kern, vec_grid(op.g.N), kThreads, 0, s, op.g.N, op.atb.data(), w.q.data(), op.diag.data(), x, weight);
	}
	FI_CUDA(cudaStreamSynchronize(s));
}

template <typename T>
__global__ void tile_prepare_kernel(Geom g, const T* __restrict__ atb, const T* __restrict__ Ag, const T* __restrict__ Bg,
                                    const T* __restrict__ diag, T* __restrict__ rhs, T* __restrict__ minv, int* __restrict__ tile_active)
{
	const int64_t i = static_cast<int64_t>(blockIdx.x) * blockDim.x + threadIdx.x;
	if (i >= g.N) { return; }
	rhs[i]  = atb[i] - T(2) * (Ag[i] - Bg[i]);
	minv[i] = T(1) / (diag[i] + static_cast<T>(g.tile_reg));
	if (diag[i] != T(0)) { tile_active[tile_of_node(g, i)] = 1; }
}

template <typename T>
__global__ void tile_merge_kernel(Geom g, const T* __restrict__ y, const int* __restrict__ tile_active, T* __restrict__ x)
{
	const int64_t i = static_cast<int64_t>(blockIdx.x) * blockDim.x + threadIdx.x;
	if (i >= g.N) { return; }
	if (tile_active[tile_of_node(g, i)]) { x[i] = y[i]; }
}

template <typename T>
PcgResult tile_phase(Operator<T>& op, int tile_size, T* x, double tol, long long max_iter, int check_every, cudaStream_t s)
{
	TraceScope trace("tile_phase");
	FI_REQUIRE(tile_size >= 2, FI_ERR_INVALID, "tile_size must be >= 2");
	FI_REQUIRE(op.dist == nullptr && !op.g.sharded(), FI_ERR_UNSUPPORTED, "the tile phase runs on an unsharded lattice");
	const int64_t n = op.g.N;
	int64_t       tiles = 1;
	for (int d = 0; d < op.g.ndim; ++d) { tiles *= (op.g.size[d] + tile_size - 1) / tile_size; }
	DevBuf<T>   Ag(n), Bg(n), rhs(n), y(n), minv(n);
	DevBuf<int> active(static_cast<size_t>(tiles));
	active.zero(s);
	const int  old_fast = op.use_fast;
	const Geom old_g    = op.g;
	bool       swapped  = false;
	auto restore = [&] {
		op.g        = old_g;
		op.use_fast = old_fast;
		if (swapped) { op.minv.swap(minv); swapped = false; }
	};
	PcgResult r;
	try {
		op.apply(x, Ag.data(), nullptr, nullptr, s);
		op.g.tile     = tile_size;
		op.g.tile_reg = 0.0f;
		op.use_fast   = kStencilGeneric;
		op.apply(x, Bg.data(), nullptr, nullptr, s);
		op.g.tile_reg = 1e-6f;
		{
			auto kern = tile_prepare_kernel<T>;
			FI_LAUNCH(kern, div_up(n, kThreads), kThreads, 0, s, op.g, op.atb.data(), Ag.data(), Bg.data(), op.diag.data(), rhs.data(), minv.data(),
			          active.data());
		}
		op.minv.swap(minv);
		swapped = true;
		FI_CUDA(cudaMemcpyAsync(y.data(), x, n * sizeof(T), cudaMemcpyDeviceToDevice, s));
		r = pcg_solve<T>(op, rhs.data(), y.data(), tol, max_iter, check_every, false, s);
		auto kern = tile_merge_kernel<T>;
		FI_LAUNCH(kern, div_up(n, kThreads), kThreads, 0, s, op.g, y.data(), active.data(), x);
		FI_CUDA(cudaStreamSynchronize(s));
	} catch (...) {
		restore();
		throw;
	}
	restore();
	return r;
}

template <typename T>
void time_kernels(Operator<T>& op, int iterations, int check_every, double* out, cudaStream_t s)
{
	ensure_work(op, s);
	PcgWork<T>&   w = op.work;
	const int64_t n = op.g.N;
	DevBuf<T>     x(n);
	x.zero(s);
	const PcgResult r = pcg_solve<T>(op, nullptr, x.data(), 1e-300, iterations, check_every, false, s);
	out[0] = r.loop_ms;
	PcgState h;
	FI_CUDA(cudaMemcpyAsync(&h, w.state.data(), sizeof(h), cudaMemcpyDeviceToHost, s));
	FI_CUDA(cudaStreamSynchronize(s));
	h.done      = 0;
	h.max_iters = 1ll << 60;
	h.tol2bb    = 0;
	h.iters     = 1;
	h.alpha_prev = 0;
	if (!(h.rho[0] > 0)) { h.rho[0] = 1; }
	if (!(h.rho[1] > 0)) { h.rho[1] = 1; }
	if (!(h.pq > 0)) { h.pq = 1; }
	FI_CUDA(cudaMemcpyAsync(w.state.data(), &h, sizeof(h), cudaMemcpyHostToDevice, s));
	FI_CUDA(cudaStreamSynchronize(s));
	cudaEvent_t e0, e1;
	FI_CUDA(cudaEventCreate(&e0));
	FI_CUDA(cudaEventCreate(&e1));
	auto timed = [&](auto&& body) {
		FI_CUDA(cudaEventRecord(e0, s));
		for (int i = 0; i < iterations; ++i) { body(i); }
		FI_CUDA(cudaEventRecord(e1, s));
		FI_CUDA(cudaEventSynchronize(e1));
		float ms = 0;
		FI_CUDA(cudaEventElapsedTime(&ms, e0, e1));
		return static_cast<double>(ms);
	};
	DevBuf<double> dot(1);
	T*             pp[2] = {w.p.data(), w.p2.data()};
	bool           fused = false;
	out[1] = timed([&](int i) {
		const int par = i & 1;
		fused = stencil_fused_step<T>(op.use_fast, op.g, op.tabs, w.r.data(), op.minv.data(), pp[par], pp[par ^ 1], w.q.data(),
		                              w.state.data(), par, dot.data(), op.partial.data(), op.ticket.data(), nullptr, s);
		if (fused) {
			apply_data_term<T>(op.g, op.data, pp[par ^ 1], w.q.data(), dot.data(), nullptr, s);
		} else {
			op.apply(w.p.data(), w.q.data(), dot.data(), nullptr, s);
		}
	});
	h.pq = 1e30;
	FI_CUDA(cudaMemcpyAsync(w.state.data(), &h, sizeof(h), cudaMemcpyHostToDevice, s));
	FI_CUDA(cudaStreamSynchronize(s));
	out[2] = timed([&](int i) {
		if (!fused) {
			auto ku = pcg_update_kernel<T, kXClassic>;
			FI_LAUNCH(ku, vec_grid(n), kThreads, 0, s, n, x.data(), w.r.data(), w.p.data(), static_cast<const T*>(nullptr), w.q.data(), op.minv.data(), w.state.data(), 0,
			          w.partial.data(), w.ticket.data(), 0);
		} else if ((i & 1) == 0) {
			auto ku = pcg_update_kernel<T, kXSkip>;
			FI_LAUNCH(ku, vec_grid(n), kThreads, 0, s, n, x.data(), w.r.data(), w.p2.data(), w.p.data(), w.q.data(), op.minv.data(), w.state.data(), 0,
			          w.partial.data(), w.ticket.data(), 0);
		} else {
			auto ku = pcg_update_kernel<T, kXBoth>;
			FI_LAUNCH(ku, vec_grid(n), kThreads, 0, s, n, x.data(), w.r.data(), w.p.data(), w.p2.data(), w.q.data(), op.minv.data(), w.state.data(), 0,
			          w.partial.data(), w.ticket.data(), 0);
		}
	});
	out[3] = 0.0;
	if (!fused) {
		out[3] = timed([&](int) {
			auto kd = pcg_direction_kernel<T>;
			FI_LAUNCH(kd, vec_grid(n), kThreads, 0, s, n, w.r.data(), op.minv.data(), w.p.data(), w.state.data(), 0);
		});
	}
	out[4] = fused ? 1.0 : 0.0;
	out[7] = 0.0;
	out[5] = timed([&](int i) {
		const int par = i & 1;
		if (fused) {
			stencil_fused_step<T>(op.use_fast, op.g, op.tabs, w.r.data(), op.minv.data(), pp[par], pp[par ^ 1], w.q.data(), w.state.data(), par,
			                      dot.data(), op.partial.data(), op.ticket.data(), nullptr, s);
		} else {
			stencil_apply<T>(op.g, op.tabs, w.p.data(), w.q.data(), dot.data(), op.partial.data(), op.ticket.data(), nullptr, op.use_fast, s);
		}
	});
	out[6] = timed([&](int i) {
		const int par = i & 1;
		apply_data_term<T>(op.g, op.data, fused ? pp[par ^ 1] : w.p.data(), w.q.data(), dot.data(), nullptr, s);
	});
	cudaEventDestroy(e0);
	cudaEventDestroy(e1);
}

template void time_kernels<float>(Operator<float>&, int, int, double*, cudaStream_t);
template void time_kernels<double>(Operator<double>&, int, int, double*, cudaStream_t);
template std::unique_ptr<Operator<float>> build_operator<float>(const Geom&, const ModelAccum&, const PointStore&, const HostRows&, cudaStream_t);
template std::unique_ptr<Operator<double>> build_operator<double>(const Geom&, const ModelAccum&, const PointStore&, const HostRows&, cudaStream_t);
template PcgResult pcg_solve<float>(Operator<float>&, const float*, float*, double, long long, int, bool, cudaStream_t);
template PcgResult pcg_solve<double>(Operator<double>&, const double*, double*, double, long long, int, bool, cudaStream_t);
template PcgResult tile_phase<float>(Operator<float>&, int, float*, double, long long, int, cudaStream_t);
template PcgResult tile_phase<double>(Operator<double>&, int, double*, double, long long, int, cudaStream_t);
template void jacobi_sweeps<float>(Operator<float>&, float*, int, float, cudaStream_t);
template void jacobi_sweeps<double>(Operator<double>&, double*, int, double, cudaStream_t);
template void residual<float>(Operator<float>&, const float*, const float*, float*, double*, double*, cudaStream_t);
template void residual<double>(Operator<double>&, const double*, const double*, double*, double*, double*, cudaStream_t);

}
```

field_interpolation_b200/csrc/solver.hpp:

```cpp
#pragma once

#include <utility>
#include <vector>

#include "internal.hpp"
#include "peer.cuh"

namespace fi {

struct DistHooks
{
	virtual ~DistHooks() = default;
	virtual const PeerLink* link() { return nullptr; }
	virtual void* shared_vector(size_t bytes, void** lo, void** hi, cudaStream_t s)
	{
		(void)bytes; (void)lo; (void)hi; (void)s;
		return nullptr;
	}
	virtual int64_t peer_own_cells(int peer) { (void)peer; return 0; }
	virtual unsigned long long next_seq() { return 0; }
	virtual void allreduce(double* d_ptr, int count, cudaStream_t s) = 0;
	virtual void exchange_halo(void* d_vec, size_t elem_size, cudaStream_t s) = 0;
	virtual int rank() const { return 0; }
	virtual int world() const { return 1; }
	virtual std::unique_ptr<DistHooks> for_geom(const Geom& g, int halo)
	{
		(void)g; (void)halo;
		return nullptr;
	}
	virtual void allgather_planes(float* full, int64_t plane_cells, const std::vector<std::pair<int, int>>& own, cudaStream_t s)
	{
		(void)full; (void)plane_cells; (void)own; (void)s;
	}
};

template <typename T>
struct PcgWork
{
	DevBuf<T>        r, p, q;
	DevBuf<T>        p2;
	DevBuf<double>   partial;
	DevBuf<unsigned> ticket;
	DevBuf<PcgState> state;
};

template <typename T>
struct Operator
{
	Geom             g;
	StencilTables    tabs;
	DataTerm<T>      data;
	DevBuf<T>        atb, diag, minv;
	DevBuf<double>   partial;
	DevBuf<unsigned> ticket;
	int              use_fast = kStencilAuto;
	double           setup_ms = 0;
	PcgWork<T>       work;
	DistHooks*       dist = nullptr;
	bool             guess_is_zero = false;

	void apply(const T* p, T* q, double* d_dot, const int* d_done, cudaStream_t s)
	{
		stencil_apply<T>(g, tabs, p, q, d_dot, partial.data(), ticket.data(), d_done, use_fast, s);
		apply_data_term<T>(g, data, p, q, d_dot, d_done, s);
	}
};

template <typename T>
std::unique_ptr<Operator<T>> build_operator(const Geom& g, const ModelAccum& m, const PointStore& pts, const HostRows& rows,
                                            cudaStream_t s);

struct PcgResult
{
	long long iterations = 0;
	double    rel_residual = 0, initial_residual = 0, true_residual = 0, solve_ms = 0;
	double    loop_ms = 0;
	bool      converged = false, zero_rhs = false;
	bool      stalled = false;
};

constexpr double kConvergedSlack = 1.25;

template <typename T>
PcgResult pcg_solve(Operator<T>& op, const T* b, T* x, double tol, long long max_iter, int check_every, bool want_true_residual,
                    cudaStream_t s);

template <typename T>
bool stencil_fast_3d_fused(const Geom& g, const StencilTables& t, const T* r, const T* minv, const T* p_old, T* p_new, T* q,
                           const PcgState* st, int par, double* d_dot_out, double* d_partial, unsigned* d_ticket, const int* d_done,
                           cudaStream_t s);

template <typename T>
bool stencil_tma_3d_fused(const Geom& g, const StencilTables& t, const T* r, const T* minv, const T* p_old, T* p_new, T* q,
                          const PcgState* st, int par, double* d_dot_out, double* d_partial, unsigned* d_ticket, const int* d_done,
                          cudaStream_t s);

template <typename T>
bool stencil_tma_3d_epilogue(const Geom& g, const StencilTables& t, const T* in, const T* res_in, T* res_out, const T* minv, T* e, T* d_new,
                             T a, T b, cudaStream_t s);

template <typename T>
bool stencil_tma_2d_fused(const Geom& g, const StencilTables& t, const T* r, const T* minv, const T* p_old, T* p_new, T* q, const PcgState* st, int par,
                          double* d_dot_out, double* d_partial, unsigned* d_ticket, const int* d_done, cudaStream_t s);
template <typename T>
bool stencil_tma_2d_epilogue(const Geom& g, const StencilTables& t, const T* in, const T* res_in, T* res_out, const T* minv, T* e, T* d_new, T a, T b,
                             cudaStream_t s);

template <typename T>
inline bool stencil_fused_step(int mode, const Geom& g, const StencilTables& t, const T* r, const T* minv, const T* p_old, T* p_new,
                               T* q, const PcgState* st, int par, double* d_dot_out, double* d_partial, unsigned* d_ticket,
                               const int* d_done, cudaStream_t s)
{
	if (g.tile) { return false; }
	if (mode == kStencilAuto && g.ndim == 2) { return stencil_tma_2d_fused<T>(g, t, r, minv, p_old, p_new, q, st, par, d_dot_out, d_partial, d_ticket, d_done, s); }
	if (mode == kStencilAuto && stencil_tma_3d_fused<T>(g, t, r, minv, p_old, p_new, q, st, par, d_dot_out, d_partial, d_ticket, d_done, s)) { return true; }
	if (mode != kStencilGeneric && stencil_fast_3d_fused<T>(g, t, r, minv, p_old, p_new, q, st, par, d_dot_out, d_partial, d_ticket, d_done, s)) { return true; }
	return false;
}

struct MgOptions
{
	int    nu               = 3;
	int    nu_coarse        = 0;
	int    gamma            = 1;
	int    w_levels         = 3;
	double cheb_ratio       = 12.0;
	int    coarsest_cells   = 600;
	int    power_iterations = 12;
	int    tail_cells       = 0;
};

inline MgOptions default_mg_options(const ModelAccum& m, const Geom& g, bool sharded, int user_nu, double user_ratio)
{
	MgOptions o;
	const bool high_order = m.on[3] || m.on[4];
	o.nu        = high_order ? 5 : 2;
	o.nu_coarse = high_order ? 0 : 4;
	const int64_t cells = static_cast<int64_t>(g.size[0]) * g.size[1] * g.size[2];
	if (g.ndim == 3 && !sharded && !high_order && cells >= 50000000) {
		o.gamma     = 2;
		o.nu_coarse = 6;
		o.w_levels  = 3;
	}
	if (user_nu > 0) {
		o.nu = user_nu;
		if (o.nu_coarse > 0 && o.nu_coarse < user_nu) { o.nu_coarse = user_nu; }
	}
	if (user_ratio > 1.0) { o.cheb_ratio = user_ratio; }
	return o;
}

void mg_options_from_env(MgOptions& o);

struct Multigrid
{
	struct Level;
	MgOptions                           opt;
	std::vector<std::unique_ptr<Level>> levels;
	DevBuf<float>                       coarse_inv;
	int                                 nc = 0;
	int                                 base_level = 0;
	DevBuf<unsigned char>               tail_plan;
	int                                 tail_from = 0, tail_nlev = 0;
	cudaGraphExec_t                     exec = nullptr;
	const float*                        graph_r = nullptr;
	float*                              graph_z = nullptr;
	int64_t                             graph_launches = 0;

	Multigrid();
	~Multigrid();
	void vcycle(const float* r, float* z, cudaStream_t s);
	bool demote_to_v_cycle();
};

std::unique_ptr<Multigrid> build_multigrid(Operator<float>& fine, const ModelAccum& model, const PointStore& pts, const MgOptions& opt, cudaStream_t s,
                                           const int* root_size = nullptr, int fine_level = 0);

constexpr int kMaxSlabLevels = 8;

struct SlabMgPlan
{
	int nd   = 0;
	int halo = 2;
	int world = 1;
	int size[kMaxSlabLevels + 1][kMaxDim] = {};
	std::vector<std::pair<int, int>> own[kMaxSlabLevels + 1];
};

SlabMgPlan plan_slab_multigrid(const int32_t* sizes, int world, int radius, int64_t gather_cells, const int* cuts = nullptr);

struct SlabMultigrid
{
	struct DLevel;
	MgOptions                             opt;
	SlabMgPlan                            plan;
	int                                   rank = 0;
	std::vector<std::unique_ptr<DLevel>>  dl;
	std::unique_ptr<Operator<float>>      tail_op;
	PointStore                            tail_pts;
	std::unique_ptr<Multigrid>            tail;
	DevBuf<float>                         tail_r, tail_e;

	SlabMultigrid();
	~SlabMultigrid();
	void vcycle(const float* r, float* z, cudaStream_t s);
	bool demote_to_v_cycle() { return false; }
};

std::unique_ptr<SlabMultigrid> build_slab_multigrid(Operator<float>& fine, const ModelAccum& model, const PointStore& pts, const MgOptions& opt,
                                                    const SlabMgPlan& plan, cudaStream_t s);

template <typename T>
PcgResult mgpcg_solve(Operator<T>& op, Multigrid& mg, const T* b, T* x, double tol, long long max_iter, cudaStream_t s, int guard_every = 0);
template <typename T>
PcgResult slab_mgpcg_solve(Operator<T>& op, SlabMultigrid& mg, const T* b, T* x, double tol, long long max_iter, cudaStream_t s, int guard_every = 0);

template <typename T>
PcgResult tile_phase(Operator<T>& op, int tile_size, T* x, double tol, long long max_iter, int check_every, cudaStream_t s);

template <typename T>
void jacobi_sweeps(Operator<T>& op, T* x, int iterations, T weight, cudaStream_t s);

template <typename T>
void time_kernels(Operator<T>& op, int iterations, int check_every, double* out, cudaStream_t s);

template <typename T>
void residual(Operator<T>& op, const T* b, const T* x, T* r, double* rr, double* bb, cudaStream_t s);

void convert(const float* src, double* dst, int64_t n, cudaStream_t s);
void convert(const double* src, float* dst, int64_t n, cudaStream_t s);
void axpy_f32_into_f64(const float* e, double* x, int64_t n, cudaStream_t s);

}
```

field_interpolation_b200/csrc/stencil.cu:

```cuda
#include <algorithm>

#include "internal.hpp"

namespace fi {

namespace {

constexpr int kThreads = 256;

__host__ __device__ __forceinline__ int row_class(int i, int n)
{
	return n <= 9 ? i : (i < 4 ? i : (i >= n - 4 ? i - n + 9 : 4));
}

template <typename T>
struct DevTables
{
	T   band[kMaxDim][9][9];
	T   gs2;
	int radius;
	bool any;
};

template <typename T>
DevTables<T> to_dev(const StencilTables& t)
{
	DevTables<T> d;
	for (int a = 0; a < kMaxDim; ++a) {
		for (int c = 0; c < 9; ++c) {
			for (int k = 0; k < 9; ++k) { d.band[a][c][k] = static_cast<T>(t.band[a][c][k]); }
		}
	}
	d.gs2    = static_cast<T>(t.gs2);
	d.radius = t.radius;
	d.any    = t.any;
	return d;
}

__device__ __forceinline__ int lap1(int i, int n, int o)
{
	if (o == 0) { return (i > 0 ? 1 : 0) + (i < n - 1 ? 1 : 0); }
	const int j = i + o;
	return (j >= 0 && j < n) ? -1 : 0;
}

__device__ __forceinline__ void coords_of(const Geom& g, int64_t index, int* c)
{
	c[0] = c[1] = c[2] = 0;
	for (int d = 0; d < g.ndim; ++d) {
		if (d == g.ndim - 1) {
			c[d] = static_cast<int>(index) + (d == 2 ? g.zoff : 0);
		} else {
			c[d] = static_cast<int>(index % g.size[d]);
			index /= g.size[d];
		}
	}
}

constexpr int kDiagRows = 8;

template <typename T>
__global__ void __launch_bounds__(kThreads) diagonal_kernel(Geom g, DevTables<T> tab, T* __restrict__ diag, T* __restrict__ minv)
{
	const int nx = g.size[0], ny = g.ndim >= 2 ? g.size[1] : 1;
	const int zl = blockIdx.z;
	const int z  = g.ndim == 3 ? zl + g.zoff : 0;
	const bool outside = g.ndim == 3 && (z < 0 || z >= g.size[2]);
	T   zpart = 0;
	int lz    = 0;
	if (g.ndim == 3 && !outside) {
		zpart = tab.band[2][row_class(z, g.size[2])][4];
		lz    = lap1(z, g.size[2], 0);
	}
	for (int r = 0; r < kDiagRows; ++r) {
		const int y = blockIdx.y * kDiagRows + r;
		if (y >= ny) { break; }
		T   rest = zpart;
		int ly   = 0;
		if (g.ndim >= 2) {
			rest += tab.band[1][row_class(y, ny)][4];
			ly = lap1(y, ny, 0);
			if (tab.gs2 != T(0)) { rest += tab.gs2 * static_cast<T>(ly * lz); }
		}
		const int64_t at = (static_cast<int64_t>(zl) * ny + y) * nx;
		for (int x = blockIdx.x * blockDim.x + threadIdx.x; x < nx; x += gridDim.x * blockDim.x) {
			T d = diag[at + x];
			if (!outside && tab.any) {
				T acc = rest + tab.band[0][row_class(x, nx)][4];
				if (tab.gs2 != T(0) && g.ndim >= 2) { acc += tab.gs2 * static_cast<T>(lap1(x, nx, 0) * (ly + lz)); }
				d += acc;
				diag[at + x] = d;
			}
			if (minv) { minv[at + x] = d != T(0) ? T(1) / d : T(1); }
		}
	}
}

template <typename T>
__global__ void __launch_bounds__(kThreads) stencil_generic_kernel(Geom g, DevTables<T> tab, const T* __restrict__ p, T* __restrict__ q,
                                                                   double* dot_out, double* partial, unsigned* ticket, const int* done)
{
	__shared__ T      band[kMaxDim][9][9];
	__shared__ double red[32];
	if (done && *done) { return; }
	for (int k = threadIdx.x; k < kMaxDim * 81; k += blockDim.x) { (&band[0][0][0])[k] = (&tab.band[0][0][0])[k]; }
	__syncthreads();
	const int64_t i = static_cast<int64_t>(blockIdx.x) * blockDim.x + threadIdx.x;
	double        mine[1] = {0.0};
	if (i < g.N) {
		int c[kMaxDim];
		coords_of(g, i, c);
		T         acc = 0;
		const int R   = tab.radius;
		const int tl  = g.tile;
		for (int d = 0; d < g.ndim; ++d) {
			const T* row = band[d][row_class(c[d], g.size[d])];
			for (int o = -R; o <= R; ++o) {
				const T coef = row[o + 4];
				if (coef == T(0)) { continue; }
				if (tl && (c[d] + o < 0 || (c[d] + o) / tl != c[d] / tl)) { continue; }
				acc += coef * p[i + o * g.stride[d]];
			}
		}
		if (tl) { acc += static_cast<T>(g.tile_reg) * p[i]; }
		if (tab.gs2 != T(0)) {
			for (int d = 0; d < g.ndim; ++d) {
				for (int o = d + 1; o < g.ndim; ++o) {
					for (int a = -1; a <= 1; ++a) {
						const int la = lap1(c[d], g.size[d], a);
						if (la == 0) { continue; }
						for (int b = -1; b <= 1; ++b) {
							const int lb = lap1(c[o], g.size[o], b);
							if (lb == 0) { continue; }
							if (tl && ((c[d] + a) / tl != c[d] / tl || (c[o] + b) / tl != c[o] / tl)) { continue; }
							acc += tab.gs2 * static_cast<T>(la * lb) * p[i + a * g.stride[d] + b * g.stride[o]];
						}
					}
				}
			}
		}
		q[i]    = acc;
		mine[0] = static_cast<double>(p[i]) * static_cast<double>(acc);
	}
	if (dot_out) {
		mine[0] = block_sum(mine[0], red);
		grid_sum<1>(mine, partial, ticket, red, [&](const double(&tot)[1]) { *dot_out = tot[0]; });
	}
}

}

StencilTables make_tables(const Geom& g, const ModelAccum& m)
{
	StencilTables t;
	std::memset(&t, 0, sizeof(t));
	t.gs2    = 2.0 * m.gs_sq;
	t.radius = 0;
	for (int k = 0; k <= 4; ++k) {
		if (m.on[k]) { t.radius = k; }
	}
	t.any = t.gs2 > 0;
	for (int k = 0; k <= 4; ++k) { t.any = t.any || m.on[k]; }
	for (int d = 0; d < g.ndim; ++d) {
		const int n = g.size[d];
		for (int cls = 0; cls < 9; ++cls) {
			int i;
			if (n <= 9) {
				if (cls >= n) { continue; }
				i = cls;
			} else {
				i = cls < 4 ? cls : (cls == 4 ? 4 : n - 9 + cls);
			}
			for (int k = 0; k <= 4; ++k) {
				if (!m.on[k]) { continue; }
				for (int j = std::max(0, i - k); j <= std::min(i, n - k - 1); ++j) {
					for (int mm = 0; mm <= k; ++mm) {
						const int o = j + mm - i;
						t.band[d][cls][o + 4] += m.cc[k][i - j][mm];
					}
				}
			}
		}
	}
	if (g.ndim > 1 && t.gs2 > 0 && t.radius < 1) { t.radius = 1; }
	return t;
}

template <typename T>
void stencil_diagonal(const Geom& g, const StencilTables& t, T* d_diag, T* d_minv, cudaStream_t s)
{
	if (!t.any && !d_minv) { return; }
	auto kern = diagonal_kernel<T>;
	const dim3 grid(std::min(div_up(g.size[0], kThreads), 64), g.ndim >= 2 ? div_up(g.size[1], kDiagRows) : 1, g.ndim == 3 ? g.nzl : 1);
	FI_REQUIRE(grid.y <= 65535 && grid.z <= 65535, FI_ERR_RANGE, "lattice too large along y or z for the diagonal kernel's grid");
	FI_LAUNCH(kern, grid, kThreads, 0, s, g, to_dev<T>(t), d_diag, d_minv);
}

int stencil_partial_slots(const Geom& g) { return div_up(g.N, kThreads) + 8; }

template <typename T>
bool stencil_fast_3d(const Geom& g, const StencilTables& t, const T* p, T* q, double* d_dot_out, double* d_partial,
                     unsigned* d_ticket, const int* d_done, cudaStream_t s);
template <typename T>
bool stencil_tma_3d(const Geom& g, const StencilTables& t, const T* p, T* q, double* d_dot_out, double* d_partial,
                    unsigned* d_ticket, const int* d_done, cudaStream_t s);
template <typename T>
bool stencil_tma_2d(const Geom& g, const StencilTables& t, const T* p, T* q, double* d_dot_out, double* d_partial,
                    unsigned* d_ticket, const int* d_done, cudaStream_t s);

template <typename T>
void stencil_apply(const Geom& g, const StencilTables& t, const T* p, T* q, double* d_dot_out, double* d_partial,
                   unsigned* d_ticket, const int* d_done, int mode, cudaStream_t s)
{
	if (g.tile) { mode = kStencilGeneric; }
	if (mode == kStencilAuto && g.ndim == 2 && stencil_tma_2d<T>(g, t, p, q, d_dot_out, d_partial, d_ticket, d_done, s)) { return; }
	if (mode == kStencilAuto && stencil_tma_3d<T>(g, t, p, q, d_dot_out, d_partial, d_ticket, d_done, s)) { return; }
	if (mode != kStencilGeneric && stencil_fast_3d<T>(g, t, p, q, d_dot_out, d_partial, d_ticket, d_done, s)) { return; }
	FI_REQUIRE(!g.sharded(), FI_ERR_UNSUPPORTED, "a slab-sharded lattice needs the TMA-staged 3D stencil kernel (x size a multiple of 16 bytes and >= 32, y size >= 8)");
	auto kern = stencil_generic_kernel<T>;
	FI_LAUNCH(kern, div_up(g.N, kThreads), kThreads, 0, s, g, to_dev<T>(t), p, q, d_dot_out, d_partial, d_ticket, d_done);
}

template void stencil_diagonal<float>(const Geom&, const StencilTables&, float*, float*, cudaStream_t);
template void stencil_diagonal<double>(const Geom&, const StencilTables&, double*, double*, cudaStream_t);
template void stencil_apply<float>(const Geom&, const StencilTables&, const float*, float*, double*, double*, unsigned*, const int*, int, cudaStream_t);
template void stencil_apply<double>(const Geom&, const StencilTables&, const double*, double*, double*, double*, unsigned*, const int*, int, cudaStream_t);

}
```

field_interpolation_b200/csrc/stencil_tma.cu:

```cuda
#include <cstdlib>
#include <type_traits>

#include "solver.hpp"
#include "tma.cuh"

namespace fi {

namespace {

using namespace tma;

template <typename T, int R, int TY_ = 8>
struct Tile
{
	static constexpr int V    = 16 / sizeof(T);
	static constexpr int NP   = (R + V - 1) / V;
	static constexpr int TXP  = 32;
	static constexpr int TY   = TY_;
	static constexpr int BXP  = TXP + 2 * NP;
	static constexpr int BY   = TY + 2 * R;
	__host__ __device__ static constexpr int ring(bool gs) { return R + 2 + (gs ? 1 : 0); }
	static constexpr int TILE_BYTES = ((BXP * BY * 16 + 127) / 128) * 128;
	static constexpr int BOX_BYTES  = BXP * BY * 16;
};

template <typename T, int R, int S, bool Fused, bool GS, int TY = 8>
constexpr size_t smem_bytes()
{
	using G = Tile<T, R, TY>;
	return 128  + static_cast<size_t>(S) * (Fused ? 3 : 1) * G::TILE_BYTES + static_cast<size_t>(G::ring(GS)) * G::TILE_BYTES +
	       S * sizeof(uint64_t) + 9 * (2 * R + 1) * sizeof(T) + 32 * sizeof(double) + 64;
}

template <typename T, int R, int S, bool Fused, int MINB, bool Epi, bool GS, int TY>
__global__ void __launch_bounds__(256, MINB)
    stencil3d_tma_kernel(const __grid_constant__ CUtensorMap map_a,
                         const __grid_constant__ CUtensorMap map_b,
                         const __grid_constant__ CUtensorMap map_c,
                         int nx, int ny, int nzl, int zo0, int zo1, int zoff, int nzg, int zchunk, TmaTables<T> tab, T gs2,
                         T* __restrict__ q, T* __restrict__ p_new,
                         const PcgState* st, int par, double* dot_out, double* partial, unsigned* ticket, const int* done, EpiArgs<T> epi)
{
	static_assert(!(Fused && Epi), "the epilogue mode takes a plain input");
	using G           = Tile<T, R, TY>;
	constexpr int V   = G::V;
	constexpr int NP  = G::NP;
	constexpr int NA  = Fused ? 3 : 1;
	constexpr int W   = 2 * R + 1;
	constexpr int RING = G::ring(GS);
	using Pack        = typename PackOf<T>::type;
	using PU          = PackU<T, V>;

	if (done && *done) { return; }

#ifdef FI_B200_EMU
	unsigned char* smem_raw = ::cuda_emu::dynamic_smem();
#else
	extern __shared__ unsigned char smem_raw[];
#endif
	unsigned char* base = smem_raw + ((128u - (smem_u32(smem_raw) & 127u)) & 127u);
	auto stage_ptr = [&](int s, int a) { return reinterpret_cast<Pack*>(base + (static_cast<size_t>(s) * NA + a) * G::TILE_BYTES); };
	unsigned char* ring_base = base + static_cast<size_t>(S) * NA * G::TILE_BYTES;
	auto ring_ptr = [&](int slot) { return reinterpret_cast<Pack*>(ring_base + static_cast<size_t>(slot) * G::TILE_BYTES); };
	uint64_t* full  = reinterpret_cast<uint64_t*>(ring_base + static_cast<size_t>(RING) * G::TILE_BYTES);
	T*        zband = reinterpret_cast<T*>(full + S);
	double*   red   = reinterpret_cast<double*>((reinterpret_cast<uintptr_t>(zband + 9 * W) + 7) & ~uintptr_t(7));

	const int tid = threadIdx.x, tx = tid & 31, ty = tid >> 5;
	const int x0t = blockIdx.x * (G::TXP * V);
	const int y0t = blockIdx.y * G::TY;
	const int x0  = x0t + tx * V;
	const int y   = y0t + ty;
	const int zb  = zo0 + blockIdx.z * zchunk;
	const int ze  = min(zo1, zb + zchunk);
	const int wlo = blockIdx.z == 0 ? max(0, zo0 - R) : zb;
	const int whi = ze == zo1 ? min(nzl, zo1 + R) : ze;
	const bool   has_own = ty < G::TY;
	const bool   in_xy = has_own && (x0 < nx) && (y < ny);
	const size_t plane = static_cast<size_t>(nx) * ny;

	if (tid == 0) {
#pragma unroll
		for (int s = 0; s < S; ++s) { mbar_init(&full[s], 1); }
		fence_barrier_init();
	}
	for (int k = tid; k < 9 * W; k += 256) { zband[k] = tab.band[2][k / W][k % W + 4 - R]; }

	T beta = 0;
	if (Fused) { beta = st->iters == 0 ? T(0) : static_cast<T>(st->rho[par] / st->rho[par ^ 1]); }

	T cx[V][W], cy[W];
#pragma unroll
	for (int j = 0; j < V; ++j) {
		const int cls = row_class(min(x0 + j, nx - 1), nx);
#pragma unroll
		for (int t = 0; t < W; ++t) { cx[j][t] = tab.band[0][cls][t + 4 - R]; }
	}
	{
		const int cls = row_class(min(y, ny - 1), ny);
#pragma unroll
		for (int t = 0; t < W; ++t) { cy[t] = tab.band[1][cls][t + 4 - R]; }
	}
	T lx0[V], ly0 = T(0);
	if (GS) {
#pragma unroll
		for (int j = 0; j < V; ++j) {
			const int xi = min(x0 + j, nx - 1);
			lx0[j]       = static_cast<T>((xi > 0 ? 1 : 0) + (xi < nx - 1 ? 1 : 0));
		}
		const int yi = min(y, ny - 1);
		ly0          = static_cast<T>((yi > 0 ? 1 : 0) + (yi < ny - 1 ? 1 : 0));
	}

	const int lp0    = zb - R;
	const int n_iter = ze + R - lp0;
	auto issue = [&](int i) {
		const int s = i % S;
		mbar_expect_tx(&full[s], NA * G::BOX_BYTES);
		tma_load_3d(stage_ptr(s, 0), &map_a, &full[s], x0t - NP * V, y0t - R, lp0 + i);
		if (Fused) {
			tma_load_3d(stage_ptr(s, 1), &map_b, &full[s], x0t - NP * V, y0t - R, lp0 + i);
			tma_load_3d(stage_ptr(s, 2), &map_c, &full[s], x0t - NP * V, y0t - R, lp0 + i);
		}
	};
	__syncthreads();
	if (tid == 0) {
		for (int i = 0; i < S && i < n_iter; ++i) { issue(i); }
	}

	const bool has_yh = ty < 2 * R;
	const int  yh_row = ty < R ? ty : G::TY + ty;
	const bool has_xh = tid < 2 * NP * G::TY;
	const int  xh_r   = (tid / (2 * NP)) + R;
	const int  xh_k   = tid % (2 * NP);
	const int  xh_col = xh_k < NP ? xh_k : G::TXP + xh_k;
	const int  own_at = (ty + R) * G::BXP + tx + NP;
	const int  yh_at  = yh_row * G::BXP + tx + NP;
	const int  xh_at  = xh_r * G::BXP + xh_col;
	const bool has_ch = GS && has_yh && tx < 2 * NP;
	const int  ch_at  = yh_row * G::BXP + (tx < NP ? tx : G::TXP + tx);

	auto direction = [&](const Pack* sa, const Pack* sb, const Pack* sc, int at) -> Pack {
		if (!Fused) { return sa[at]; }
		PU rr, mm, pp, out;
		rr.v = sa[at];
		mm.v = sb[at];
		pp.v = sc[at];
#pragma unroll
		for (int j = 0; j < V; ++j) { out.a[j] = mm.a[j] * rr.a[j] + beta * pp.a[j]; }
		return out.v;
	};

	PU     pipe[W];
	double acc = 0.0;
	T*       qout = q + static_cast<size_t>(y) * nx + x0;
	T*       pout = Fused ? p_new + static_cast<size_t>(y) * nx + x0 : nullptr;

	PU         pre_r, pre_m, pre_e;
	const bool epi_upd = Epi && epi.d_new != nullptr;
	const size_t xy_off = static_cast<size_t>(y) * nx + x0;
	auto epi_load = [&](int z) {
		const size_t at = static_cast<size_t>(z) * plane + xy_off;
		pre_r.v = *reinterpret_cast<const Pack*>(epi.res_in + at);
		if (epi_upd) {
			pre_m.v = *reinterpret_cast<const Pack*>(epi.minv + at);
			pre_e.v = *reinterpret_cast<const Pack*>(epi.e + at);
		}
	};
	if (Epi && in_xy && zb < ze) { epi_load(zb); }

	int stage = 0, slot = 0;
	uint32_t phase = 0;
	for (int i0 = 0; i0 < n_iter; i0 += W) {
#pragma unroll
		for (int k = 0; k < W; ++k) {
			const int i = i0 + k;
			if (i >= n_iter) { break; }
			const int lp = lp0 + i;
			mbar_wait(&full[stage], phase);
			const Pack* sa = stage_ptr(stage, 0);
			const Pack* sb = Fused ? stage_ptr(stage, 1) : nullptr;
			const Pack* sc = Fused ? stage_ptr(stage, 2) : nullptr;
			Pack*       rg = ring_ptr(slot);
			if (has_own) {
				pipe[k].v  = direction(sa, sb, sc, own_at);
				rg[own_at] = pipe[k].v;
			}
			if (has_yh) { rg[yh_at] = direction(sa, sb, sc, yh_at); }
			if (has_xh) { rg[xh_at] = direction(sa, sb, sc, xh_at); }
			if (has_ch) { rg[ch_at] = direction(sa, sb, sc, ch_at); }
			if (Fused && in_xy && lp >= wlo && lp < whi) { *reinterpret_cast<Pack*>(pout + static_cast<size_t>(lp) * plane) = pipe[k].v; }
			__syncthreads();
			if (tid == 0 && i + S < n_iter) { issue(i + S); }

			const int z = lp - R;
			if (z >= zb && in_xy) {
				int zslot = slot - R;
				if (zslot < 0) { zslot += RING; }
				const Pack* pz = ring_ptr(zslot);
				const T*    cz = zband + row_class(z + zoff, nzg) * W;
				const PU&   ctr = pipe[(k + 1 + R) % W];
				PU          out;
				PU          cur_r, cur_m, cur_e;
				if (Epi) {
					cur_r = pre_r;
					cur_m = pre_m;
					cur_e = pre_e;
					if (z + 1 < ze) { epi_load(z + 1); }
				}
#pragma unroll
				for (int j = 0; j < V; ++j) {
					T s = T(0);
#pragma unroll
					for (int t = 0; t < W; ++t) { s += cz[t] * pipe[(k + 1 + t) % W].a[j]; }
					out.a[j] = s;
				}
				PU y_lo, y_hi;
#pragma unroll
				for (int t = 0; t < W; ++t) {
					if (t == R) {
#pragma unroll
						for (int j = 0; j < V; ++j) { out.a[j] += cy[t] * ctr.a[j]; }
					} else {
						PU nb;
						nb.v = pz[(ty + t) * G::BXP + tx + NP];
#pragma unroll
						for (int j = 0; j < V; ++j) { out.a[j] += cy[t] * nb.a[j]; }
						if (GS && t == R - 1) { y_lo = nb; }
						if (GS && t == R + 1) { y_hi = nb; }
					}
				}
				T xs[(2 * NP + 1) * V];
#pragma unroll
				for (int kk = 0; kk < 2 * NP + 1; ++kk) {
					PU nb;
					if (kk == NP) { nb = ctr; } else { nb.v = pz[(ty + R) * G::BXP + tx + kk]; }
#pragma unroll
					for (int j = 0; j < V; ++j) { xs[kk * V + j] = nb.a[j]; }
				}
#pragma unroll
				for (int j = 0; j < V; ++j) {
#pragma unroll
					for (int t = 0; t < W; ++t) { out.a[j] += cx[j][t] * xs[NP * V + j + t - R]; }
				}
				if (GS) {
					const int zg  = z + zoff;
					const T   lz0 = static_cast<T>((zg > 0 ? 1 : 0) + (zg < nzg - 1 ? 1 : 0));
					int       sm  = zslot - 1, sp = zslot + 1;
					if (sm < 0) { sm += RING; }
					if (sp >= RING) { sp -= RING; }
					const Pack* pm = ring_ptr(sm);
					const Pack* pp = ring_ptr(sp);
					const PU&   z_lo = pipe[(k + R) % W];
					const PU&   z_hi = pipe[(k + 2 + R) % W];
					T a_lo[3 * V], a_hi[3 * V], b_lo[3 * V], b_hi[3 * V];
#pragma unroll
					for (int kk = 0; kk < 3; ++kk) {
						PU u0, u1, u2, u3;
						if (kk == 1) {
							u0 = y_lo;
							u1 = y_hi;
							u2 = z_lo;
							u3 = z_hi;
						} else {
							u0.v = pz[(ty + R - 1) * G::BXP + tx + NP - 1 + kk];
							u1.v = pz[(ty + R + 1) * G::BXP + tx + NP - 1 + kk];
							u2.v = pm[(ty + R) * G::BXP + tx + NP - 1 + kk];
							u3.v = pp[(ty + R) * G::BXP + tx + NP - 1 + kk];
						}
#pragma unroll
						for (int j = 0; j < V; ++j) {
							a_lo[kk * V + j] = u0.a[j];
							a_hi[kk * V + j] = u1.a[j];
							b_lo[kk * V + j] = u2.a[j];
							b_hi[kk * V + j] = u3.a[j];
						}
					}
					PU c0, c1, c2, c3;
					c0.v = pm[(ty + R - 1) * G::BXP + tx + NP];
					c1.v = pm[(ty + R + 1) * G::BXP + tx + NP];
					c2.v = pp[(ty + R - 1) * G::BXP + tx + NP];
					c3.v = pp[(ty + R + 1) * G::BXP + tx + NP];
#pragma unroll
					for (int j = 0; j < V; ++j) {
						const int cc = V + j, cx0 = NP * V + j;
						const T   lx = lx0[j];
						T g = (lx * ly0 + lx * lz0 + ly0 * lz0) * ctr.a[j];
						g -= (ly0 + lz0) * (xs[cx0 - 1] + xs[cx0 + 1]);
						g -= (lx + lz0) * (y_lo.a[j] + y_hi.a[j]);
						g -= (lx + ly0) * (z_lo.a[j] + z_hi.a[j]);
						g += a_lo[cc - 1] + a_lo[cc + 1] + a_hi[cc - 1] + a_hi[cc + 1];
						g += b_lo[cc - 1] + b_lo[cc + 1] + b_hi[cc - 1] + b_hi[cc + 1];
						g += c0.a[j] + c1.a[j] + c2.a[j] + c3.a[j];
						out.a[j] += gs2 * g;
					}
				}
				if (Epi) {
					const size_t at = static_cast<size_t>(z) * plane + xy_off;
					PU           rn;
#pragma unroll
					for (int j = 0; j < V; ++j) { rn.a[j] = cur_r.a[j] - out.a[j]; }
					if (epi.res_out) { *reinterpret_cast<Pack*>(epi.res_out + at) = rn.v; }
					if (epi_upd) {
						PU dn, en;
#pragma unroll
						for (int j = 0; j < V; ++j) {
							dn.a[j] = epi.a * ctr.a[j] + epi.b * cur_m.a[j] * rn.a[j];
							en.a[j] = cur_e.a[j] + dn.a[j];
						}
						*reinterpret_cast<Pack*>(epi.d_new + at) = dn.v;
						*reinterpret_cast<Pack*>(epi.e + at)     = en.v;
					}
				} else {
					*reinterpret_cast<Pack*>(qout + static_cast<size_t>(z) * plane) = out.v;
					T d = T(0);
#pragma unroll
					for (int j = 0; j < V; ++j) { d += out.a[j] * ctr.a[j]; }
					acc += static_cast<double>(d);
				}
			}
			if (++stage == S) { stage = 0; phase ^= 1u; }
			if (++slot == RING) { slot = 0; }
		}
	}

	if (dot_out) {
		double mine[1] = {block_sum(acc, red)};
		grid_sum<1>(mine, partial, ticket, red, [&](const double(&tot)[1]) { *dot_out = tot[0]; });
	}
}

template <typename T, int R, int TY>
CUtensorMap make_map(const Geom& g, const T* ptr)
{
	using G = Tile<T, R, TY>;
	CUtensorMap m;
	std::memset(&m, 0, sizeof(m));
	EncodeFn fn = encode_fn();
	FI_REQUIRE(fn != nullptr, FI_ERR_CUDA, "cuTensorMapEncodeTiled is not available from this driver");
	const cuuint64_t dims[3]    = {static_cast<cuuint64_t>(g.size[0]), static_cast<cuuint64_t>(g.size[1]), static_cast<cuuint64_t>(g.nzl)};
	const cuuint64_t strides[2] = {static_cast<cuuint64_t>(g.size[0]) * sizeof(T), static_cast<cuuint64_t>(g.size[0]) * g.size[1] * sizeof(T)};
	const cuuint32_t box[3]     = {static_cast<cuuint32_t>(G::BXP * G::V), static_cast<cuuint32_t>(G::BY), 1u};
	const cuuint32_t estr[3]    = {1u, 1u, 1u};
	const CUresult   r = fn(&m, sizeof(T) == 4 ? CU_TENSOR_MAP_DATA_TYPE_FLOAT32 : CU_TENSOR_MAP_DATA_TYPE_FLOAT64, 3,
	                        const_cast<T*>(ptr), dims, strides, box, estr, CU_TENSOR_MAP_INTERLEAVE_NONE, CU_TENSOR_MAP_SWIZZLE_NONE,
	                        CU_TENSOR_MAP_L2_PROMOTION_L2_256B, CU_TENSOR_MAP_FLOAT_OOB_FILL_NONE);
	FI_REQUIRE(r == CUDA_SUCCESS, FI_ERR_CUDA, "cuTensorMapEncodeTiled failed with CUresult " + std::to_string(static_cast<int>(r)));
	return m;
}

inline double plan_chunks(const Geom& g, int R, int S, int minb, int tx_cells, int ty, int* out_chunks)
{
	const int     tiles_x = div_up(g.size[0], tx_cells), tiles_y = div_up(g.size[1], ty);
	const int64_t resident = static_cast<int64_t>(sm_count()) * minb;
	const int64_t tiles    = static_cast<int64_t>(tiles_x) * tiles_y;
	const int     nown     = g.zown1 - g.zown0;
	int           chunks   = 1;
	double        best     = 1e300;
	for (int c = 1; c <= std::max(1, nown / (2 * R + 1)) && c <= 256; ++c) {
		const int     zc    = div_up(nown, c);
		const int     cc    = div_up(nown, zc);
		const int64_t waves = (tiles * cc + resident - 1) / resident;
		const double  frac  = static_cast<double>(tiles * cc) / static_cast<double>(resident);
		const double  cost  = std::max(static_cast<double>(waves) - 0.5, frac) * (zc + 2 * R + S + 1);
		if (cost < best - 1e-9) {
			best   = cost;
			chunks = cc;
		}
	}
	*out_chunks = chunks;
	return best;
}

template <typename T, int R, int S, bool Fused, int MINB, bool Epi, bool GS, int TY>
void launch_ty(const Geom& g, const StencilTables& t, int chunks, const T* a, const T* b, const T* c, T* q, T* p_new, const PcgState* st, int par,
               double* d_dot_out, double* d_partial, unsigned* d_ticket, const int* d_done, cudaStream_t s, const EpiArgs<T>& epi)
{
	using G = Tile<T, R, TY>;
	TmaTables<T> tab;
	for (int ax = 0; ax < kMaxDim; ++ax) {
		for (int cl = 0; cl < 9; ++cl) {
			for (int k = 0; k < 9; ++k) { tab.band[ax][cl][k] = static_cast<T>(t.band[ax][cl][k]); }
		}
	}
	const CUtensorMap ma = make_map<T, R, TY>(g, a);
	const CUtensorMap mb = Fused ? make_map<T, R, TY>(g, b) : ma;
	const CUtensorMap mc = Fused ? make_map<T, R, TY>(g, c) : ma;
	const int tiles_x = div_up(g.size[0], G::TXP * G::V), tiles_y = div_up(g.size[1], G::TY);
	const int nown    = g.zown1 - g.zown0;
	const int zchunk  = div_up(nown, chunks);
	chunks            = div_up(nown, zchunk);
	dim3 grid(tiles_x, tiles_y, chunks);
	auto kern = stencil3d_tma_kernel<T, R, S, Fused, MINB, Epi, GS, TY>;
	constexpr size_t smem = smem_bytes<T, R, S, Fused, GS, TY>();
	static bool configured = false;
	if (!configured) {
		FI_CUDA(cudaFuncSetAttribute(kern, cudaFuncAttributeMaxDynamicSharedMemorySize, static_cast<int>(smem)));
		configured = true;
	}
	FI_LAUNCH(kern, grid, 256, smem, s, ma, mb, mc, g.size[0], g.size[1], g.nzl, g.zown0, g.zown1, g.zoff, g.size[2], zchunk, tab,
	          static_cast<T>(t.gs2), q, p_new, st, par, d_dot_out, d_partial, d_ticket, d_done, epi);
}

template <typename T, int R, int S, bool Fused, int MINB, bool Epi, bool GS>
void launch_gs(const Geom& g, const StencilTables& t, const T* a, const T* b, const T* c, T* q, T* p_new, const PcgState* st, int par,
               double* d_dot_out, double* d_partial, unsigned* d_ticket, const int* d_done, cudaStream_t s, const EpiArgs<T>& epi = EpiArgs<T>())
{
	using G8 = Tile<T, R, 8>;
	int c8 = 1, c7 = 1;
	plan_chunks(g, R, S, MINB, G8::TXP * G8::V, 8, &c8);
	bool seven = false;
	if (R <= 2) {
		static const int forced = [] {
			const char* e = getenv("FI_B200_STENCIL_TY");
			return e ? atoi(e) : 0;
		}();
		plan_chunks(g, R, S, MINB, G8::TXP * G8::V, 7, &c7);
		auto busiest = [&](int ty, int chunks) {
			const int64_t blocks = static_cast<int64_t>(div_up(g.size[0], G8::TXP * G8::V)) * div_up(g.size[1], ty) * chunks;
			const int64_t waves  = (blocks + static_cast<int64_t>(sm_count()) * MINB - 1) / (static_cast<int64_t>(sm_count()) * MINB);
			return static_cast<double>(waves) * (div_up(g.zown1 - g.zown0, chunks) + 2 * R + S + 1) * ty;
		};
		seven = forced == 7 || (forced != 8 && busiest(7, c7) < 0.97 * busiest(8, c8));
	}
	if constexpr (R <= 2) {
		if (seven) {
			launch_ty<T, R, S, Fused, MINB, Epi, GS, 7>(g, t, c7, a, b, c, q, p_new, st, par, d_dot_out, d_partial, d_ticket, d_done, s, epi);
			return;
		}
	}
	launch_ty<T, R, S, Fused, MINB, Epi, GS, 8>(g, t, c8, a, b, c, q, p_new, st, par, d_dot_out, d_partial, d_ticket, d_done, s, epi);
}

template <typename T, int R, int S, bool Fused, int MINB, bool Epi = false>
void launch(const Geom& g, const StencilTables& t, const T* a, const T* b, const T* c, T* q, T* p_new, const PcgState* st, int par,
            double* d_dot_out, double* d_partial, unsigned* d_ticket, const int* d_done, cudaStream_t s, const EpiArgs<T>& epi = EpiArgs<T>())
{
	if (t.gs2 != 0.0) {
		launch_gs<T, R, S, Fused, MINB, Epi, true>(g, t, a, b, c, q, p_new, st, par, d_dot_out, d_partial, d_ticket, d_done, s, epi);
	} else {
		launch_gs<T, R, S, Fused, MINB, Epi, false>(g, t, a, b, c, q, p_new, st, par, d_dot_out, d_partial, d_ticket, d_done, s, epi);
	}
}

template <typename T>
bool eligible(const Geom& g, const StencilTables& t)
{
	constexpr int V = 16 / sizeof(T);
	return g.ndim == 3 && t.radius >= 1 && g.size[0] % V == 0 && g.size[0] >= 32 && g.size[1] >= 8 && g.zown1 - g.zown0 >= 1 &&
	       (g.sharded() || g.size[2] >= 8) && encode_fn() != nullptr;
}

template <typename T, bool Fused>
void dispatch(const Geom& g, const StencilTables& t, const T* a, const T* b, const T* c, T* q, T* p_new, const PcgState* st, int par,
              double* d_dot_out, double* d_partial, unsigned* d_ticket, const int* d_done, cudaStream_t s)
{
	if (t.radius <= 1) {
		launch<T, 1, 3, Fused, 2>(g, t, a, b, c, q, p_new, st, par, d_dot_out, d_partial, d_ticket, d_done, s);
	} else if (t.radius == 2) {
		static const int variant = [] {
			const char* e = getenv("FI_B200_STENCIL_VARIANT");
			return e ? atoi(e) : 0;
		}();
		if (variant == 3 && std::is_same<T, float>::value) {
			launch<T, 2, 2, Fused, 3>(g, t, a, b, c, q, p_new, st, par, d_dot_out, d_partial, d_ticket, d_done, s);
		} else if (variant == 4 && std::is_same<T, float>::value) {
			launch<T, 2, 4, Fused, 2>(g, t, a, b, c, q, p_new, st, par, d_dot_out, d_partial, d_ticket, d_done, s);
		} else {
			launch<T, 2, 3, Fused, 2>(g, t, a, b, c, q, p_new, st, par, d_dot_out, d_partial, d_ticket, d_done, s);
		}
	} else {
		launch<T, 4, 2, Fused, 1>(g, t, a, b, c, q, p_new, st, par, d_dot_out, d_partial, d_ticket, d_done, s);
	}
}

}

template <typename T>
bool stencil_tma_3d(const Geom& g, const StencilTables& t, const T* p, T* q, double* d_dot_out, double* d_partial, unsigned* d_ticket,
                    const int* d_done, cudaStream_t s)
{
	if (!eligible<T>(g, t)) { return false; }
	dispatch<T, false>(g, t, p, nullptr, nullptr, q, nullptr, nullptr, 0, d_dot_out, d_partial, d_ticket, d_done, s);
	return true;
}

template <typename T>
bool stencil_tma_3d_fused(const Geom& g, const StencilTables& t, const T* r, const T* minv, const T* p_old, T* p_new, T* q,
                          const PcgState* st, int par, double* d_dot_out, double* d_partial, unsigned* d_ticket, const int* d_done,
                          cudaStream_t s)
{
	if (!eligible<T>(g, t)) { return false; }
	dispatch<T, true>(g, t, r, minv, p_old, q, p_new, st, par, d_dot_out, d_partial, d_ticket, d_done, s);
	return true;
}

template <typename T>
bool stencil_tma_3d_epilogue(const Geom& g, const StencilTables& t, const T* in, const T* res_in, T* res_out, const T* minv, T* e, T* d_new,
                             T a, T b, cudaStream_t s)
{
	if (!eligible<T>(g, t)) { return false; }
	EpiArgs<T> epi;
	epi.res_in  = res_in;
	epi.res_out = res_out;
	epi.minv    = minv;
	epi.e       = e;
	epi.d_new   = d_new;
	epi.a       = a;
	epi.b       = b;
	if (t.radius <= 1) {
		launch<T, 1, 3, false, 2, true>(g, t, in, nullptr, nullptr, nullptr, nullptr, nullptr, 0, nullptr, nullptr, nullptr, nullptr, s, epi);
	} else if (t.radius == 2) {
		launch<T, 2, 3, false, 2, true>(g, t, in, nullptr, nullptr, nullptr, nullptr, nullptr, 0, nullptr, nullptr, nullptr, nullptr, s, epi);
	} else {
		launch<T, 4, 2, false, 1, true>(g, t, in, nullptr, nullptr, nullptr, nullptr, nullptr, 0, nullptr, nullptr, nullptr, nullptr, s, epi);
	}
	return true;
}

template bool stencil_tma_3d_epilogue<float>(const Geom&, const StencilTables&, const float*, const float*, float*, const float*, float*, float*, float, float, cudaStream_t);
template bool stencil_tma_3d<float>(const Geom&, const StencilTables&, const float*, float*, double*, double*, unsigned*, const int*, cudaStream_t);
template bool stencil_tma_3d<double>(const Geom&, const StencilTables&, const double*, double*, double*, double*, unsigned*, const int*, cudaStream_t);
template bool stencil_tma_3d_fused<float>(const Geom&, const StencilTables&, const float*, const float*, const float*, float*, float*, const PcgState*, int, double*, double*, unsigned*, const int*, cudaStream_t);
template bool stencil_tma_3d_fused<double>(const Geom&, const StencilTables&, const double*, const double*, const double*, double*, double*, const PcgState*, int, double*, double*, unsigned*, const int*, cudaStream_t);

}
```

include/fi_b200.h:

```cpp
#ifndef FI_B200_H
#define FI_B200_H

#include <stdint.h>

#ifdef __cplusplus
extern "C" {
#endif

#define FI_B200_ABI_VERSION 3

#if defined(__GNUC__)
#define FI_API __attribute__((visibility("default")))
#else
#define FI_API
#endif

enum fi_status {
	FI_OK              = 0,
	FI_ERR_INVALID     = 1,
	FI_ERR_CUDA        = 2,
	FI_ERR_RANGE       = 3,
	FI_ERR_UNSUPPORTED = 4,
	FI_ERR_COMM        = 5
};

enum fi_location { FI_HOST = 0, FI_DEVICE = 1 };

enum fi_value_kernel { FI_VALUE_NEAREST_NEIGHBOR = 0, FI_VALUE_LINEAR_INTERPOLATION = 1 };
enum fi_gradient_kernel { FI_GRADIENT_NEAREST_NEIGHBOR = 0, FI_GRADIENT_CELL_EDGES = 1, FI_GRADIENT_LINEAR_INTERPOLATION = 2 };

enum fi_precision { FI_F32 = 0, FI_F64 = 1, FI_MIXED = 2 };

enum fi_preconditioner { FI_PRECOND_JACOBI = 0, FI_PRECOND_MULTIGRID = 1 };

typedef struct fi_weights {
	float   data_pos, data_gradient;
	float   model_0, model_1, model_2, model_3, model_4;
	float   gradient_smoothness;
	int32_t value_kernel, gradient_kernel;
} fi_weights;

typedef struct fi_triplet {
	int32_t row, col;
	float   value;
} fi_triplet;

typedef struct fi_solve_options {
	int32_t precision;
	int32_t max_iterations;
	double  tolerance;
	int32_t check_every;
	int32_t use_fast_stencil;
	int32_t refine_max_outer;
	double  refine_inner_tolerance;
	int32_t preconditioner;
	int32_t mg_smoothing_steps;
	double  mg_cheb_ratio;
} fi_solve_options;

typedef struct fi_solve_stats {
	int64_t iterations;
	double  relative_residual;
	double  true_residual;
	double  initial_residual;
	double  setup_ms;
	double  solve_ms;
	int32_t converged;
	int32_t outer_sweeps;
	int64_t occupied_cells;
	int64_t generic_rows;
	int64_t widened_after;
} fi_solve_stats;

typedef struct fi_field fi_field;

FI_API int         fi_abi_version(void);
FI_API const char* fi_last_error(void);
FI_API int         fi_device_count(int32_t* count);
FI_API int         fi_set_device(int32_t device);
FI_API void        fi_weights_default(fi_weights* w);
FI_API void        fi_solve_options_default(fi_solve_options* o);

FI_API int fi_field_create(int32_t ndim, const int32_t* sizes, fi_field** out);
FI_API int fi_field_destroy(fi_field* f);
FI_API int fi_field_clone(const fi_field* f, fi_field** out);

FI_API int fi_field_add_model(fi_field* f, const fi_weights* w);

FI_API int fi_field_add_points(fi_field* f, float value_weight, int32_t value_kernel, float gradient_weight,
                        int32_t gradient_kernel, int64_t num_points, const float* positions, const float* normals,
                        const float* point_weights, const float* values, int32_t loc, int64_t* rows_added);

FI_API int fi_field_add_rows(fi_field* f, int64_t num_rows, int64_t num_triplets, const int32_t* trip_row,
                      const int32_t* trip_col, const float* trip_val, const float* rhs);

FI_API int fi_sdf_from_points(int32_t ndim, const int32_t* sizes, const fi_weights* w, int64_t num_points,
                       const float* positions, const float* normals, const float* point_weights, int32_t loc,
                       fi_field** out);

FI_API int fi_field_counts(fi_field* f, int64_t* num_rows, int64_t* num_triplets);
FI_API int fi_field_export(fi_field* f, fi_triplet* triplets, float* rhs);
FI_API int fi_field_export_rows(fi_field* f, int64_t row_begin, fi_triplet* triplets, float* rhs);

FI_API int fi_field_apply(fi_field* f, int32_t precision, const void* x, void* y);
FI_API int fi_field_use_fast_stencil(fi_field* f, int32_t enable);
FI_API int fi_field_rhs(fi_field* f, int32_t precision, void* atb);
FI_API int fi_field_diagonal(fi_field* f, int32_t precision, void* diag);

FI_API int fi_field_solve(fi_field* f, const fi_solve_options* opt, const float* guess, float* solution, int32_t loc,
                   fi_solve_stats* stats);

FI_API int fi_field_solve_tiled(fi_field* f, const fi_solve_options* opt, int32_t tile, int32_t tile_size, int32_t cg,
                         const float* guess, float* solution, int32_t loc, fi_solve_stats* stats, fi_solve_stats* tile_stats);

FI_API int fi_field_jacobi(fi_field* f, const float* guess, int32_t num_iterations, float weight, float* solution);

FI_API int fi_upscale_field(int32_t ndim, const int32_t* small_sizes, const int32_t* large_sizes, const float* small_field,
                     float* large_field, int32_t loc);

FI_API int fi_error_map(int64_t num_triplets, const fi_triplet* triplets, int64_t num_columns, const float* solution,
                 int64_t num_rows, const float* rhs, float* heatmap);

FI_API int fi_marching_squares(int32_t width, int32_t height, const float* values, float iso, int32_t loc, float* lines,
                        int64_t capacity_segments, int64_t* num_segments, float* area);
FI_API int fi_calc_area(int64_t num_segments, const float* lines, int32_t loc, float* area);
FI_API int fi_bicubic_upsample(int32_t width, int32_t height, const float* values, int32_t upsample, float* large, int32_t loc);

typedef struct fi_cascade_options {
	fi_solve_options fine;
	int32_t factor;
	int32_t coarsest_size;
	double  coarse_tolerance;
	int32_t max_levels;
} fi_cascade_options;

typedef struct fi_cascade_stats {
	int32_t levels;
	int64_t level_cells[16];
	int64_t level_iterations[16];
	double  level_ms[16];
	double  level_initial_residual[16];
	double  total_ms;
	int64_t cell_iterations;
	fi_solve_stats finest;
} fi_cascade_stats;

FI_API int fi_sdf_solve_cascade(int32_t ndim, const int32_t* sizes, const fi_weights* w, int64_t num_points,
                         const float* unit_positions, const float* normals, const float* point_weights,
                         const fi_cascade_options* opt, float* solution, int32_t loc, fi_cascade_stats* stats);

typedef struct fi_comm fi_comm;
FI_API int fi_comm_unique_id(void* id, int64_t capacity );
FI_API int fi_comm_create(int32_t rank, int32_t world, const void* id, fi_comm** out);
FI_API int fi_comm_destroy(fi_comm* c);
FI_API int fi_slab_range(int32_t nz, int32_t world, int32_t rank, int32_t* z0, int32_t* z1);
FI_API int fi_slab_balanced_cuts(const int32_t* sizes , int32_t world, int64_t num_points, const float* positions, int32_t loc,
                          double point_weight, int32_t min_planes, int32_t* cuts );
FI_API int fi_comm_set_slab_cuts(fi_comm* c, int32_t nz, const int32_t* cuts );
FI_API int fi_slab_mg_plan(const int32_t* sizes , int32_t world, int32_t stencil_radius, int64_t gather_cells, int32_t* sharded_levels,
                    int32_t* halo, int32_t* level_sizes, int32_t* plane_ranges);
FI_API int fi_slab_sdf_solve(fi_comm* c, const int32_t* sizes , const fi_weights* w, int64_t num_points,
                      const float* positions, const float* normals, const float* point_weights, int32_t loc,
                      const fi_solve_options* opt, const float* guess_own, float* solution_own, int32_t solution_loc,
                      fi_solve_stats* stats);

FI_API int     fi_trim_memory(void);
FI_API int64_t fi_cached_bytes(void);

FI_API int64_t fi_kernel_launches(void);
FI_API void    fi_kernel_launches_reset(void);

FI_API int fi_field_time_iterations(fi_field* f, const fi_solve_options* opt, int32_t iterations, double* ms);

#ifdef __cplusplus
}
#endif
#endif
```

Baseline: 134.4 billion.

## Compress Jacobi preconditioner into boundary-class table with per-segment exception bits

Result: faster. 138.5 billion, median of 6 (+3.1%).

```diff
diff --git a/field_interpolation_b200/_lib.py b/field_interpolation_b200/_lib.py
--- a/field_interpolation_b200/_lib.py
+++ b/field_interpolation_b200/_lib.py
@@ -87,6 +87,7 @@
     "fi_field_use_fast_stencil": (C.c_int, [_vp, _i32]),
     "fi_field_rhs": (C.c_int, [_vp, _i32, _vp]),
     "fi_field_diagonal": (C.c_int, [_vp, _i32, _vp]),
+    "fi_field_preconditioner": (C.c_int, [_vp, _i32, _vp, _vp, _vp, _pd]),
     "fi_field_solve": (C.c_int, [_vp, _p(fi_solve_options), _vp, _vp, _i32, _p(fi_solve_stats)]),
     "fi_field_solve_tiled": (C.c_int, [_vp, _p(fi_solve_options), _i32, _i32, _i32, _vp, _vp, _i32, _p(fi_solve_stats), _p(fi_solve_stats)]),
     "fi_field_jacobi": (C.c_int, [_vp, _pf, _i32, _f, _pf]),
diff --git a/field_interpolation_b200/api.py b/field_interpolation_b200/api.py
--- a/field_interpolation_b200/api.py
+++ b/field_interpolation_b200/api.py
@@ -160,6 +160,20 @@
 
     def diagonal(self, precision=FI_F64):
         return self._vec(L.lib().fi_field_diagonal, precision)
+
+    def preconditioner(self, precision=FI_F64, views=True):
+        dt = np.float32 if precision == FI_F32 else np.float64
+        n = self.num_unknowns
+        minv = np.empty(n, dt)
+        upd = np.empty(n, dt) if views else None
+        sten = np.empty(n, dt) if views else None
+        st = (C.c_double * 8)()
+        ptr = lambda a: C.c_void_p(a.ctypes.data) if a is not None else None
+        L.check(L.lib().fi_field_preconditioner(self._h, precision, ptr(minv), ptr(upd), ptr(sten), st))
+        stats = {"table": bool(st[0]), "segments": int(st[1]), "flagged_segments": int(st[2]), "tile_planes": int(st[3]),
+                 "flagged_tile_planes": int(st[4]), "update_uses_table": bool(int(st[5]) & 1),
+                 "stencil_uses_table": bool(int(st[5]) & 2), "tile_rows": int(st[6]), "build_ms": st[7]}
+        return minv, upd, sten, stats
 
     def use_fast_stencil(self, mode):
         L.check(L.lib().fi_field_use_fast_stencil(self._h, int(mode)))
diff --git a/field_interpolation_b200/csrc/abi.cu b/field_interpolation_b200/csrc/abi.cu
--- a/field_interpolation_b200/csrc/abi.cu
+++ b/field_interpolation_b200/csrc/abi.cu
@@ -873,6 +873,42 @@
 int fi_field_rhs(fi_field* f, int32_t precision, void* atb) { return copy_vector(f, precision, atb, 0); }
 int fi_field_diagonal(fi_field* f, int32_t precision, void* diag) { return copy_vector(f, precision, diag, 1); }
 
+int fi_field_preconditioner(fi_field* f, int32_t precision, void* minv, void* minv_update, void* minv_stencil, double* stats)
+{
+	return guarded([&] {
+		FI_REQUIRE(f, FI_ERR_INVALID, "null argument");
+		auto view = [&](auto& op) {
+			using T = typename std::remove_reference<decltype(*op.minv.data())>::type;
+			const int64_t N = f->g.N;
+			const MinvClasses<T>& mc = op.mc;
+			const bool have = mc.of != nullptr && mc.of == op.minv.data();
+			if (minv) { FI_CUDA(cudaMemcpy(minv, op.minv.data(), N * sizeof(T), cudaMemcpyDeviceToHost)); }
+			if (minv_update || minv_stencil) {
+				FI_REQUIRE(have, FI_ERR_UNSUPPORTED, "this lattice has no M^-1 class table");
+				DevBuf<T> upd(N), sten(N);
+				minv_as_seen<T>(op.g, op.minv.data(), mc, upd.data(), sten.data(), f->stream);
+				FI_CUDA(cudaStreamSynchronize(f->stream));
+				if (minv_update) { FI_CUDA(cudaMemcpy(minv_update, upd.data(), N * sizeof(T), cudaMemcpyDeviceToHost)); }
+				if (minv_stencil) { FI_CUDA(cudaMemcpy(minv_stencil, sten.data(), N * sizeof(T), cudaMemcpyDeviceToHost)); }
+			}
+			if (stats) {
+				const double v[8] = {have ? 1.0 : 0.0, static_cast<double>(mc.segments), static_cast<double>(mc.flagged_segments),
+				                     static_cast<double>(mc.tile_planes), static_cast<double>(mc.flagged_tile_planes),
+				                     static_cast<double>((mc.update_ok ? 1 : 0) | (mc.stencil_ok ? 2 : 0)), static_cast<double>(mc.tile_rows),
+				                     static_cast<double>(mc.build_ms)};
+				for (int k = 0; k < 8; ++k) { stats[k] = v[k]; }
+			}
+		};
+		if (precision == FI_F32) {
+			view(f->get32());
+		} else if (precision == FI_F64) {
+			view(f->get64());
+		} else {
+			throw Error{FI_ERR_INVALID, "precision must be FI_F32 or FI_F64"};
+		}
+	});
+}
+
 int fi_field_solve(fi_field* f, const fi_solve_options* opt, const float* guess, float* solution, int32_t loc, fi_solve_stats* stats)
 {
 	return guarded([&] {
diff --git a/field_interpolation_b200/csrc/internal.hpp b/field_interpolation_b200/csrc/internal.hpp
--- a/field_interpolation_b200/csrc/internal.hpp
+++ b/field_interpolation_b200/csrc/internal.hpp
@@ -173,6 +173,98 @@
                    unsigned* d_ticket, const int* d_done, int mode, cudaStream_t s);
 int stencil_partial_slots(const Geom& g);
 
+template <typename T>
+struct MinvClassView
+{
+	static constexpr int V   = 16 / sizeof(T);
+	static constexpr int NPX = 2 * (4 / V) + 1;
+	const T*        table       = nullptr;
+	const uint32_t* seg_bits    = nullptr;
+	const uint8_t*  plane_flags = nullptr;
+};
+
+template <typename T>
+struct MinvClasses
+{
+	const T*         of = nullptr;
+	DevBuf<T>        table;
+	DevBuf<uint32_t> seg_bits;
+	DevBuf<uint8_t>  plane_flags;
+	int              tile_rows = 0, radius = 0, tile_x = 0, halo_x = 0;
+	int64_t          segments = 0, flagged_segments = 0, tile_planes = 0, flagged_tile_planes = 0;
+	bool             update_ok = false, stencil_ok = false;
+	float            build_ms = 0;
+
+	MinvClassView<T> view() const
+	{
+		MinvClassView<T> v;
+		v.table       = table.data();
+		v.seg_bits    = seg_bits.data();
+		v.plane_flags = plane_flags.data();
+		return v;
+	}
+	bool for_update(const T* minv) const { return of != nullptr && of == minv && update_ok; }
+	bool for_stencil(const T* minv) const { return of != nullptr && of == minv && stencil_ok; }
+};
+
+__host__ __device__ __forceinline__ int minv_row_class(int i, int n)
+{
+	return n <= 9 ? i : (i < 4 ? i : (i >= n - 4 ? i - n + 9 : 4));
+}
+
+template <int V>
+__host__ __device__ __forceinline__ int minv_pack_xclass(int x0, int nx)
+{
+	return x0 < 4 ? x0 / V : (x0 >= nx - 4 ? 4 / V + 1 + (x0 - (nx - 4)) / V : 4 / V);
+}
+
+template <int V>
+__host__ __device__ __forceinline__ int minv_slot(int x0, int y, int nx, int ny)
+{
+	x0 = x0 < 0 ? 0 : (x0 > nx - V ? nx - V : x0);
+	y  = y < 0 ? 0 : (y > ny - 1 ? ny - 1 : y);
+	return minv_row_class(y, ny) * (2 * (4 / V) + 1) + minv_pack_xclass<V>(x0, nx);
+}
+template <int V>
+__host__ __device__ __forceinline__ int minv_plane_slot(int z, int nz)
+{
+	z = z < 0 ? 0 : (z > nz - 1 ? nz - 1 : z);
+	return minv_row_class(z, nz) * 9 * (2 * (4 / V) + 1);
+}
+
+template <typename T>
+struct MinvPack;
+template <>
+struct MinvPack<float>
+{
+	using type = float4;
+};
+template <>
+struct MinvPack<double>
+{
+	using type = double2;
+};
+
+template <typename T, typename P>
+__device__ __forceinline__ P minv_pack_at(const MinvClassView<T>& mc, const P* tab, const T* minv, int64_t k, int slot)
+{
+	const int64_t seg = (k * MinvClassView<T>::V) >> 5;
+	if ((mc.seg_bits[seg >> 5] >> (seg & 31)) & 1u) { return reinterpret_cast<const P*>(minv)[k]; }
+	return tab[slot];
+}
+
+template <typename T>
+bool stencil_tma_3d_fused_box(const Geom& g, const StencilTables& t, int* rows, int* radius, int* tile_x, int* halo_x);
+
+template <typename T>
+void build_minv_classes(const Geom& g, const StencilTables& t, const T* minv, MinvClasses<T>& mc, cudaStream_t s);
+
+template <typename T>
+void minv_as_seen(const Geom& g, const T* minv, const MinvClasses<T>& mc, T* upd, T* sten, cudaStream_t s);
+
+enum MinvMode { kMinvStored = 0, kMinvUpdate = 1, kMinvAll = 2 };
+int minv_classes_mode();
+
 void     slab_range(int nz, int world, int rank, int* z0, int* z1);
 void     comm_slab_range(const fi_comm* c, int nz, int rank, int* z0, int* z1);
 const int* comm_cuts(const fi_comm* c, int nz);
diff --git a/field_interpolation_b200/csrc/solver.cu b/field_interpolation_b200/csrc/solver.cu
--- a/field_interpolation_b200/csrc/solver.cu
+++ b/field_interpolation_b200/csrc/solver.cu
@@ -3,6 +3,7 @@
 #include <algorithm>
 #include <cmath>
 #include <cstdlib>
+#include <type_traits>
 
 namespace fi {
 
@@ -160,10 +161,25 @@
 
 enum XMode { kXClassic = 0, kXSkip = 1, kXBoth = 2 };
 
-template <typename T, int XM, bool PACKED>
+struct StoredMinv
+{
+};
+
+template <typename T>
+struct ClassMinv
+{
+	const T*                      minv;
+	const typename Pack<T>::type* tab;
+	MinvClassView<T>              mc;
+	int64_t                       k;
+	int                           slot;
+	__device__ __forceinline__ typename Pack<T>::type operator()() const { return minv_pack_at(mc, tab, minv, k, slot); }
+};
+
+template <typename T, int XM, bool PACKED, typename MF = StoredMinv>
 __device__ __forceinline__ void update_elements(int64_t k, T* __restrict__ x, T* __restrict__ r, const T* __restrict__ p, const T* __restrict__ p_prev,
                                                 const T* __restrict__ q, const T* __restrict__ minv, T alpha, T alpha_prev, double (&acc)[2],
-                                                typename Pack<T>::type* r_out)
+                                                typename Pack<T>::type* r_out, MF m_pack = MF())
 {
 	using P         = typename Pack<T>::type;
 	constexpr int V = PACKED ? Pack<T>::V : 1;
@@ -171,12 +187,16 @@
 	if (PACKED) {
 		*reinterpret_cast<P*>(ra) = reinterpret_cast<const P*>(r)[k];
 		*reinterpret_cast<P*>(qa) = reinterpret_cast<const P*>(q)[k];
-		*reinterpret_cast<P*>(ma) = reinterpret_cast<const P*>(minv)[k];
 		if (XM != kXSkip) {
 			*reinterpret_cast<P*>(xa) = reinterpret_cast<const P*>(x)[k];
 			*reinterpret_cast<P*>(pa) = reinterpret_cast<const P*>(p)[k];
 		}
 		if (XM == kXBoth) { *reinterpret_cast<P*>(ppa) = reinterpret_cast<const P*>(p_prev)[k]; }
+		if constexpr (std::is_same<MF, StoredMinv>::value) {
+			*reinterpret_cast<P*>(ma) = reinterpret_cast<const P*>(minv)[k];
+		} else {
+			*reinterpret_cast<P*>(ma) = m_pack();
+		}
 	} else {
 		ra[0] = r[k];
 		qa[0] = q[k];
@@ -207,13 +227,21 @@
 	}
 }
 
-template <typename T, int XM>
+template <typename T, int XM, bool CLS = false>
 __global__ void __launch_bounds__(kThreads) pcg_update_kernel(int64_t n, T* __restrict__ x, T* __restrict__ r,
                                                               const T* __restrict__ p, const T* __restrict__ p_prev, const T* __restrict__ q,
                                                               const T* __restrict__ minv, PcgState* st, int par,
-                                                              double* partial, unsigned* ticket, int dist)
-{
+                                                              double* partial, unsigned* ticket, int dist, MinvClassView<T> mc, int nx, int ny,
+                                                              int nz)
+{
+	using P         = typename Pack<T>::type;
+	constexpr int V = Pack<T>::V, NPX = MinvClassView<T>::NPX;
 	__shared__ double red[32];
+	__shared__ P      mtab[CLS ? 81 * NPX : 1];
+	if (CLS) {
+		for (int i = threadIdx.x; i < 81 * NPX; i += blockDim.x) { mtab[i] = reinterpret_cast<const P*>(mc.table)[i]; }
+		__syncthreads();
+	}
 	if (st->done) { return; }
 	const double pq = st->pq;
 	if (!(pq > 0.0)) {
@@ -226,13 +254,40 @@
 	const double alpha_d = st->rho[par] / pq;
 	const T      alpha = static_cast<T>(alpha_d), alpha_prev = XM == kXBoth ? static_cast<T>(st->alpha_prev) : T(0);
 	double acc[2] = {0, 0};
-	for_each_pack<T>(n, [&](int64_t k, bool packed) {
-		if (packed) {
-			update_elements<T, XM, true>(k, x, r, p, p_prev, q, minv, alpha, alpha_prev, acc, nullptr);
-		} else {
-			update_elements<T, XM, false>(k, x, r, p, p_prev, q, minv, alpha, alpha_prev, acc, nullptr);
-		}
-	});
+	if (CLS) {
+		const int64_t npacks = n / V, stride = static_cast<int64_t>(gridDim.x) * blockDim.x;
+		const int     nxp = nx / V;
+		int64_t       k   = static_cast<int64_t>(blockIdx.x) * blockDim.x + threadIdx.x;
+		const int64_t row = k / nxp, srow = stride / nxp;
+		int           xp = static_cast<int>(k % nxp), y = static_cast<int>(row % ny), z = static_cast<int>(row / ny);
+		const int     sx = static_cast<int>(stride % nxp), sy = static_cast<int>(srow % ny), sz = static_cast<int>(srow / ny);
+		for (; k < npacks; k += stride) {
+			const ClassMinv<T> m{minv, mtab, mc, k, minv_plane_slot<V>(z, nz) + minv_slot<V>(xp * V, y, nx, ny)};
+			update_elements<T, XM, true>(k, x, r, p, p_prev, q, minv, alpha, alpha_prev, acc, nullptr, m);
+			xp += sx;
+			const int carry = xp >= nxp ? 1 : 0;
+			xp -= carry * nxp;
+			y += sy + carry;
+			if (y >= ny) {
+				y -= ny;
+				z += 1;
+			}
+			z += sz;
+		}
+		if (blockIdx.x == 0) {
+			for (int64_t i = npacks * V + threadIdx.x; i < n; i += blockDim.x) {
+				update_elements<T, XM, false>(i, x, r, p, p_prev, q, minv, alpha, alpha_prev, acc, nullptr);
+			}
+		}
+	} else {
+		for_each_pack<T>(n, [&](int64_t k, bool packed) {
+			if (packed) {
+				update_elements<T, XM, true>(k, x, r, p, p_prev, q, minv, alpha, alpha_prev, acc, nullptr);
+			} else {
+				update_elements<T, XM, false>(k, x, r, p, p_prev, q, minv, alpha, alpha_prev, acc, nullptr);
+			}
+		});
+	}
 	acc[0] = block_sum(acc[0], red);
 	acc[1] = block_sum(acc[1], red);
 	grid_sum<2>(acc, partial, ticket, red, [&](const double(&tot)[2]) {
@@ -423,6 +478,20 @@
 	for (int64_t i = static_cast<int64_t>(blockIdx.x) * blockDim.x + threadIdx.x; i < n; i += stride) { x[i] += a * p[i]; }
 }
 
+template <typename T, int XM>
+void launch_update(const Operator<T>& op, const MinvClasses<T>* mcl, int grid, cudaStream_t s, int64_t n, T* x, T* r, const T* p, const T* p_prev,
+                   const T* q, const T* minv, PcgState* st, int par, double* partial, unsigned* ticket, int dist)
+{
+	if (mcl && mcl->for_update(minv) && !dist) {
+		auto ku = pcg_update_kernel<T, XM, true>;
+		FI_LAUNCH(ku, grid, kThreads, 0, s, n, x, r, p, p_prev, q, minv, st, par, partial, ticket, 0, mcl->view(), op.g.size[0], op.g.size[1],
+		          op.g.size[2]);
+	} else {
+		auto ku = pcg_update_kernel<T, XM>;
+		FI_LAUNCH(ku, grid, kThreads, 0, s, n, x, r, p, p_prev, q, minv, st, par, partial, ticket, dist, MinvClassView<T>(), 0, 0, 0);
+	}
+}
+
 template <typename T>
 void ensure_work(Operator<T>& op, cudaStream_t s)
 {
@@ -482,6 +551,7 @@
 	op->diag.zero(s);
 	build_data_term<T>(g, pts, rows, op->data, op->atb.data(), op->diag.data(), s);
 	stencil_diagonal<T>(g, op->tabs, op->diag.data(), op->minv.data(), s);
+	build_minv_classes<T>(g, op->tabs, op->minv.data(), op->mc, s);
 	op->partial.resize(static_cast<size_t>(stencil_partial_slots(g)));
 	op->ticket.resize(1);
 	op->ticket.zero(s);
@@ -585,11 +655,14 @@
 		const char* walk_env = std::getenv("FI_B200_PEER_UPDATE");
 		const bool  peer_update_blocked = walk_env ? walk_env[0] == 'b' : n < (48ll << 20);
 		bool deferred_x = false;
+		const int             mode = dist ? kMinvStored : minv_classes_mode();
+		const MinvClasses<T>* mcl  = mode != kMinvStored ? &op.mc : nullptr;
+		const MinvClasses<T>* mcs  = mode == kMinvAll ? &op.mc : nullptr;
 		auto enqueue_round = [&] {
 			for (int it = 0; it < check_every; ++it) {
 				const int par = it & 1;
 				const bool fused = stencil_fused_step<T>(op.use_fast, op.g, op.tabs, r_vec, op.minv.data(), pp[par], pp[par ^ 1], w.q.data(),
-				                                         w.state.data(), par, d_pq, op.partial.data(), op.ticket.data(), d_done, s);
+				                                         w.state.data(), par, d_pq, op.partial.data(), op.ticket.data(), d_done, s, mcs);
 				deferred_x = deferred_x || fused;
 				if (fused && link) {
 					PeerPublish pub;
@@ -609,9 +682,9 @@
 				} else if (fused) {
 					apply_data_term<T>(op.g, op.data, pp[par ^ 1], w.q.data(), d_pq, d_done, s);
 					if (dist) { dist->allreduce(d_pq, 1, s); }
-					auto ku = par == 0 ? pcg_update_kernel<T, kXSkip> : pcg_update_kernel<T, kXBoth>;
-					FI_LAUNCH(ku, grid, kThreads, 0, s, n, x + off, r_vec + off, pp[par ^ 1] + off, pp[par] + off, w.q.data() + off, op.minv.data() + off,
-					          w.state.data(), par, w.partial.data(), w.ticket.data(), dist ? 1 : 0);
+					auto lu = par == 0 ? launch_update<T, kXSkip> : launch_update<T, kXBoth>;
+					lu(op, mcl, grid, s, n, x + off, r_vec + off, pp[par ^ 1] + off, pp[par] + off, w.q.data() + off, op.minv.data() + off,
+					   w.state.data(), par, w.partial.data(), w.ticket.data(), dist ? 1 : 0);
 					if (dist) {
 						dist->allreduce(w.state.data()->part, 2, s);
 						FI_LAUNCH(pcg_update_finish_kernel, 1, 1, 0, s, w.state.data(), par);
@@ -622,7 +695,7 @@
 					op.apply(w.p.data(), w.q.data(), d_pq, d_done, s);
 					auto ku = pcg_update_kernel<T, kXClassic>;
 					FI_LAUNCH(ku, grid, kThreads, 0, s, n, x, w.r.data(), w.p.data(), static_cast<const T*>(nullptr), w.q.data(), op.minv.data(), w.state.data(), par,
-					          w.partial.data(), w.ticket.data(), 0);
+					          w.partial.data(), w.ticket.data(), 0, MinvClassView<T>(), 0, 0, 0);
 					auto kd = pcg_direction_kernel<T>;
 					FI_LAUNCH(kd, grid, kThreads, 0, s, n, w.r.data(), op.minv.data(), w.p.data(), w.state.data(), par);
 				}
@@ -838,10 +911,13 @@
 	DevBuf<double> dot(1);
 	T*             pp[2] = {w.p.data(), w.p2.data()};
 	bool           fused = false;
+	const int             mode = op.dist ? kMinvStored : minv_classes_mode();
+	const MinvClasses<T>* mcl  = mode != kMinvStored ? &op.mc : nullptr;
+	const MinvClasses<T>* mcs  = mode == kMinvAll ? &op.mc : nullptr;
 	out[1] = timed([&](int i) {
 		const int par = i & 1;
 		fused = stencil_fused_step<T>(op.use_fast, op.g, op.tabs, w.r.data(), op.minv.data(), pp[par], pp[par ^ 1], w.q.data(),
-		                              w.state.data(), par, dot.data(), op.partial.data(), op.ticket.data(), nullptr, s);
+		                              w.state.data(), par, dot.data(), op.partial.data(), op.ticket.data(), nullptr, s, mcs);
 		if (fused) {
 			apply_data_term<T>(op.g, op.data, pp[par ^ 1], w.q.data(), dot.data(), nullptr, s);
 		} else {
@@ -855,15 +931,13 @@
 		if (!fused) {
 			auto ku = pcg_update_kernel<T, kXClassic>;
 			FI_LAUNCH(ku, vec_grid(n), kThreads, 0, s, n, x.data(), w.r.data(), w.p.data(), static_cast<const T*>(nullptr), w.q.data(), op.minv.data(), w.state.data(), 0,
-			          w.partial.data(), w.ticket.data(), 0);
+			          w.partial.data(), w.ticket.data(), 0, MinvClassView<T>(), 0, 0, 0);
 		} else if ((i & 1) == 0) {
-			auto ku = pcg_update_kernel<T, kXSkip>;
-			FI_LAUNCH(ku, vec_grid(n), kThreads, 0, s, n, x.data(), w.r.data(), w.p2.data(), w.p.data(), w.q.data(), op.minv.data(), w.state.data(), 0,
-			          w.partial.data(), w.ticket.data(), 0);
+			launch_update<T, kXSkip>(op, mcl, vec_grid(n), s, n, x.data(), w.r.data(), w.p2.data(), w.p.data(), w.q.data(), op.minv.data(), w.state.data(), 0,
+			                         w.partial.data(), w.ticket.data(), 0);
 		} else {
-			auto ku = pcg_update_kernel<T, kXBoth>;
-			FI_LAUNCH(ku, vec_grid(n), kThreads, 0, s, n, x.data(), w.r.data(), w.p.data(), w.p2.data(), w.q.data(), op.minv.data(), w.state.data(), 0,
-			          w.partial.data(), w.ticket.data(), 0);
+			launch_update<T, kXBoth>(op, mcl, vec_grid(n), s, n, x.data(), w.r.data(), w.p.data(), w.p2.data(), w.q.data(), op.minv.data(), w.state.data(), 0,
+			                         w.partial.data(), w.ticket.data(), 0);
 		}
 	});
 	out[3] = 0.0;
@@ -879,7 +953,7 @@
 		const int par = i & 1;
 		if (fused) {
 			stencil_fused_step<T>(op.use_fast, op.g, op.tabs, w.r.data(), op.minv.data(), pp[par], pp[par ^ 1], w.q.data(), w.state.data(), par,
-			                      dot.data(), op.partial.data(), op.ticket.data(), nullptr, s);
+			                      dot.data(), op.partial.data(), op.ticket.data(), nullptr, s, mcs);
 		} else {
 			stencil_apply<T>(op.g, op.tabs, w.p.data(), w.q.data(), dot.data(), op.partial.data(), op.ticket.data(), nullptr, op.use_fast, s);
 		}
diff --git a/field_interpolation_b200/csrc/solver.hpp b/field_interpolation_b200/csrc/solver.hpp
--- a/field_interpolation_b200/csrc/solver.hpp
+++ b/field_interpolation_b200/csrc/solver.hpp
@@ -51,6 +51,7 @@
 	StencilTables    tabs;
 	DataTerm<T>      data;
 	DevBuf<T>        atb, diag, minv;
+	MinvClasses<T>   mc;
 	DevBuf<double>   partial;
 	DevBuf<unsigned> ticket;
 	int              use_fast = kStencilAuto;
@@ -93,7 +94,7 @@
 template <typename T>
 bool stencil_tma_3d_fused(const Geom& g, const StencilTables& t, const T* r, const T* minv, const T* p_old, T* p_new, T* q,
                           const PcgState* st, int par, double* d_dot_out, double* d_partial, unsigned* d_ticket, const int* d_done,
-                          cudaStream_t s);
+                          cudaStream_t s, const MinvClasses<T>* mcl = nullptr);
 
 template <typename T>
 bool stencil_tma_3d_epilogue(const Geom& g, const StencilTables& t, const T* in, const T* res_in, T* res_out, const T* minv, T* e, T* d_new,
@@ -109,11 +110,11 @@
 template <typename T>
 inline bool stencil_fused_step(int mode, const Geom& g, const StencilTables& t, const T* r, const T* minv, const T* p_old, T* p_new,
                                T* q, const PcgState* st, int par, double* d_dot_out, double* d_partial, unsigned* d_ticket,
-                               const int* d_done, cudaStream_t s)
+                               const int* d_done, cudaStream_t s, const MinvClasses<T>* mcl = nullptr)
 {
 	if (g.tile) { return false; }
 	if (mode == kStencilAuto && g.ndim == 2) { return stencil_tma_2d_fused<T>(g, t, r, minv, p_old, p_new, q, st, par, d_dot_out, d_partial, d_ticket, d_done, s); }
-	if (mode == kStencilAuto && stencil_tma_3d_fused<T>(g, t, r, minv, p_old, p_new, q, st, par, d_dot_out, d_partial, d_ticket, d_done, s)) { return true; }
+	if (mode == kStencilAuto && stencil_tma_3d_fused<T>(g, t, r, minv, p_old, p_new, q, st, par, d_dot_out, d_partial, d_ticket, d_done, s, mcl)) { return true; }
 	if (mode != kStencilGeneric && stencil_fast_3d_fused<T>(g, t, r, minv, p_old, p_new, q, st, par, d_dot_out, d_partial, d_ticket, d_done, s)) { return true; }
 	return false;
 }
diff --git a/field_interpolation_b200/csrc/stencil.cu b/field_interpolation_b200/csrc/stencil.cu
--- a/field_interpolation_b200/csrc/stencil.cu
+++ b/field_interpolation_b200/csrc/stencil.cu
@@ -1,4 +1,5 @@
 #include <algorithm>
+#include <type_traits>
 
 #include "internal.hpp"
 
@@ -57,6 +58,37 @@
 	}
 }
 
+template <typename T>
+__device__ __forceinline__ T diag_zpart(const DevTables<T>& tab, int z, int nz, int* lz)
+{
+	*lz = lap1(z, nz, 0);
+	return tab.band[2][row_class(z, nz)][4];
+}
+template <typename T>
+__device__ __forceinline__ T diag_rest(const DevTables<T>& tab, int ndim, T zpart, int y, int ny, int lz, int* ly)
+{
+	T rest = zpart;
+	*ly    = 0;
+	if (ndim >= 2) {
+		rest += tab.band[1][row_class(y, ny)][4];
+		*ly = lap1(y, ny, 0);
+		if (tab.gs2 != T(0)) { rest += tab.gs2 * static_cast<T>(*ly * lz); }
+	}
+	return rest;
+}
+template <typename T>
+__device__ __forceinline__ T diag_x(const DevTables<T>& tab, int ndim, T rest, int x, int nx, int ly, int lz)
+{
+	T acc = rest + tab.band[0][row_class(x, nx)][4];
+	if (tab.gs2 != T(0) && ndim >= 2) { acc += tab.gs2 * static_cast<T>(lap1(x, nx, 0) * (ly + lz)); }
+	return acc;
+}
+template <typename T>
+__device__ __forceinline__ T jacobi_inverse(T d)
+{
+	return d != T(0) ? T(1) / d : T(1);
+}
+
 constexpr int kDiagRows = 8;
 
 template <typename T>
@@ -68,31 +100,138 @@
 	const bool outside = g.ndim == 3 && (z < 0 || z >= g.size[2]);
 	T   zpart = 0;
 	int lz    = 0;
-	if (g.ndim == 3 && !outside) {
-		zpart = tab.band[2][row_class(z, g.size[2])][4];
-		lz    = lap1(z, g.size[2], 0);
-	}
+	if (g.ndim == 3 && !outside) { zpart = diag_zpart(tab, z, g.size[2], &lz); }
 	for (int r = 0; r < kDiagRows; ++r) {
 		const int y = blockIdx.y * kDiagRows + r;
 		if (y >= ny) { break; }
-		T   rest = zpart;
-		int ly   = 0;
-		if (g.ndim >= 2) {
-			rest += tab.band[1][row_class(y, ny)][4];
-			ly = lap1(y, ny, 0);
-			if (tab.gs2 != T(0)) { rest += tab.gs2 * static_cast<T>(ly * lz); }
-		}
+		int     ly   = 0;
+		const T rest = diag_rest(tab, g.ndim, zpart, y, ny, lz, &ly);
 		const int64_t at = (static_cast<int64_t>(zl) * ny + y) * nx;
 		for (int x = blockIdx.x * blockDim.x + threadIdx.x; x < nx; x += gridDim.x * blockDim.x) {
 			T d = diag[at + x];
 			if (!outside && tab.any) {
-				T acc = rest + tab.band[0][row_class(x, nx)][4];
-				if (tab.gs2 != T(0) && g.ndim >= 2) { acc += tab.gs2 * static_cast<T>(lap1(x, nx, 0) * (ly + lz)); }
-				d += acc;
+				d += diag_x(tab, g.ndim, rest, x, nx, ly, lz);
 				diag[at + x] = d;
 			}
-			if (minv) { minv[at + x] = d != T(0) ? T(1) / d : T(1); }
-		}
+			if (minv) { minv[at + x] = jacobi_inverse(d); }
+		}
+	}
+}
+
+__device__ __forceinline__ int class_coord(int c, int n)
+{
+	if (n <= 9) { return c < n ? c : n - 1; }
+	return c < 4 ? c : (c == 4 ? 4 : n - 9 + c);
+}
+
+template <typename T>
+__device__ __forceinline__ bool same_bits(T a, T b)
+{
+	using U = typename std::conditional<sizeof(T) == 4, uint32_t, unsigned long long>::type;
+	U ua, ub;
+	memcpy(&ua, &a, sizeof(T));
+	memcpy(&ub, &b, sizeof(T));
+	return ua == ub;
+}
+
+template <typename T>
+__global__ void minv_table_kernel(Geom g, DevTables<T> tab, T* __restrict__ table)
+{
+	constexpr int V = MinvClassView<T>::V, NPX = MinvClassView<T>::NPX;
+	const int nx = g.size[0], ny = g.size[1], nz = g.size[2];
+	for (int k = threadIdx.x; k < 81 * NPX * V; k += blockDim.x) {
+		const int j = k % V, pat = (k / V) % NPX, cy = (k / (V * NPX)) % 9, cz = k / (V * NPX * 9);
+		const int half = 4 / V;
+		const int x = pat < half ? pat * V + j : (pat == half ? 4 : nx - 4 + (pat - half - 1) * V + j);
+		int       lz = 0, ly = 0;
+		const T   zpart = diag_zpart(tab, class_coord(cz, nz), nz, &lz);
+		const T   rest  = diag_rest(tab, 3, zpart, class_coord(cy, ny), ny, lz, &ly);
+		T         d     = T(0);
+		if (tab.any) { d += diag_x(tab, 3, rest, x, nx, ly, lz); }
+		table[k] = jacobi_inverse(d);
+	}
+}
+
+struct BoxGeom
+{
+	int tiles_x, tiles_y, tile_x, halo_x, rows, radius;
+	__device__ bool holds(int bx, int by, int x, int y) const
+	{
+		return bx >= 0 && bx < tiles_x && by >= 0 && by < tiles_y && x >= bx * tile_x - halo_x && x < (bx + 1) * tile_x + halo_x &&
+		       y >= by * rows - radius && y < (by + 1) * rows + radius;
+	}
+};
+
+template <typename T>
+__global__ void __launch_bounds__(kThreads) minv_flags_kernel(Geom g, const T* __restrict__ minv, const T* __restrict__ table, BoxGeom bg,
+                                                              uint32_t* __restrict__ seg_bits, uint8_t* __restrict__ plane_flags)
+{
+	constexpr int V = MinvClassView<T>::V, NPX = MinvClassView<T>::NPX;
+	const int nx = g.size[0], ny = g.size[1], z = blockIdx.z;
+	const int zs = minv_plane_slot<V>(z, g.size[2]);
+	for (int r = 0; r < kDiagRows; ++r) {
+		const int y = blockIdx.y * kDiagRows + r;
+		if (y >= ny) { break; }
+		const int64_t at = (static_cast<int64_t>(z) * ny + y) * nx;
+		const int     ys = zs + minv_row_class(y, ny) * NPX;
+		for (int x = blockIdx.x * blockDim.x + threadIdx.x; x < nx; x += gridDim.x * blockDim.x) {
+			const int x0 = x - x % V;
+			if (same_bits(minv[at + x], table[(ys + minv_pack_xclass<V>(x0, nx)) * V + (x - x0)])) { continue; }
+			const int64_t i = at + x;
+			atomicOr(&seg_bits[i >> 10], 1u << ((i >> 5) & 31));
+			for (int by = y / bg.rows - 1; by <= y / bg.rows + 1; ++by) {
+				for (int bx = x / bg.tile_x - 1; bx <= x / bg.tile_x + 1; ++bx) {
+					if (bg.holds(bx, by, x, y)) { plane_flags[(static_cast<int64_t>(by) * bg.tiles_x + bx) * g.nzl + z] = 1; }
+				}
+			}
+		}
+	}
+}
+
+__global__ void minv_count_kernel(int64_t words, const uint32_t* __restrict__ seg_bits, int64_t nflags, const uint8_t* __restrict__ plane_flags,
+                                  unsigned long long* counts)
+{
+	unsigned long long a = 0, b = 0;
+	const int64_t stride = static_cast<int64_t>(gridDim.x) * blockDim.x;
+	for (int64_t i = static_cast<int64_t>(blockIdx.x) * blockDim.x + threadIdx.x; i < words; i += stride) { a += __popc(seg_bits[i]); }
+	for (int64_t i = static_cast<int64_t>(blockIdx.x) * blockDim.x + threadIdx.x; i < nflags; i += stride) { b += plane_flags[i] != 0; }
+	if (a) { atomicAdd(&counts[0], a); }
+	if (b) { atomicAdd(&counts[1], b); }
+}
+
+template <typename T>
+__global__ void __launch_bounds__(kThreads) minv_seen_kernel(Geom g, const T* __restrict__ minv, MinvClassView<T> mc, BoxGeom bg, T* __restrict__ upd,
+                                                             T* __restrict__ sten)
+{
+	constexpr int V = MinvClassView<T>::V;
+	using P         = typename MinvPack<T>::type;
+	const int     nx = g.size[0], ny = g.size[1], nxp = nx / V;
+	const P*      tab = reinterpret_cast<const P*>(mc.table);
+	const int64_t npacks = g.N / V;
+	for (int64_t k = static_cast<int64_t>(blockIdx.x) * blockDim.x + threadIdx.x; k < npacks; k += static_cast<int64_t>(gridDim.x) * blockDim.x) {
+		const int     x0 = static_cast<int>(k % nxp) * V;
+		const int64_t row = k / nxp;
+		const int     y = static_cast<int>(row % ny), z = static_cast<int>(row / ny);
+		const int     slot = minv_plane_slot<V>(z, g.size[2]) + minv_slot<V>(x0, y, nx, ny);
+		const P       stored = reinterpret_cast<const P*>(minv)[k];
+		reinterpret_cast<P*>(upd)[k] = minv_pack_at(mc, tab, minv, k, slot);
+		P    seen = stored;
+		bool first = true, split = false;
+		for (int by = y / bg.rows - 1; by <= y / bg.rows + 1; ++by) {
+			for (int bx = x0 / bg.tile_x - 1; bx <= x0 / bg.tile_x + 1; ++bx) {
+				if (!bg.holds(bx, by, x0, y)) { continue; }
+				const P v = mc.plane_flags[(static_cast<int64_t>(by) * bg.tiles_x + bx) * g.nzl + z] ? stored : tab[slot];
+				for (int j = 0; j < V && !first; ++j) {
+					split = split || !same_bits(reinterpret_cast<const T*>(&v)[j], reinterpret_cast<const T*>(&seen)[j]);
+				}
+				seen  = v;
+				first = false;
+			}
+		}
+		if (split) {
+			for (int j = 0; j < V; ++j) { reinterpret_cast<T*>(&seen)[j] = static_cast<T>(NAN); }
+		}
+		reinterpret_cast<P*>(sten)[k] = seen;
 	}
 }
 
@@ -196,6 +335,92 @@
 	FI_LAUNCH(kern, grid, kThreads, 0, s, g, to_dev<T>(t), d_diag, d_minv);
 }
 
+int minv_classes_mode()
+{
+	const char* e = getenv("FI_B200_MINV");
+	const std::string m = e ? e : "";
+	return m == "stored" ? kMinvStored : (m == "all" ? kMinvAll : kMinvUpdate);
+}
+
+namespace {
+template <typename T>
+bool box_geom(const Geom& g, const StencilTables& t, BoxGeom* bg)
+{
+	if (!stencil_tma_3d_fused_box<T>(g, t, &bg->rows, &bg->radius, &bg->tile_x, &bg->halo_x)) { return false; }
+	bg->tiles_x = div_up(g.size[0], bg->tile_x);
+	bg->tiles_y = div_up(g.size[1], bg->rows);
+	return true;
+}
+}
+
+template <typename T>
+void build_minv_classes(const Geom& g, const StencilTables& t, const T* minv, MinvClasses<T>& mc, cudaStream_t s)
+{
+	constexpr int V = MinvClassView<T>::V, NPX = MinvClassView<T>::NPX;
+	mc.of = nullptr;
+	BoxGeom bg;
+	if (g.ndim != 3 || g.sharded() || g.tile || g.size[0] % V != 0 || g.size[0] < 10 || !box_geom<T>(g, t, &bg)) { return; }
+	cudaEvent_t e0, e1;
+	FI_CUDA(cudaEventCreate(&e0));
+	FI_CUDA(cudaEventCreate(&e1));
+	FI_CUDA(cudaEventRecord(e0, s));
+	const int64_t words  = div_up(g.N, static_cast<int64_t>(1024));
+	const int64_t nflags = static_cast<int64_t>(bg.tiles_x) * bg.tiles_y * g.nzl;
+	mc.table.resize(static_cast<size_t>(81 * NPX * V));
+	mc.seg_bits.resize(static_cast<size_t>(words));
+	mc.plane_flags.resize(static_cast<size_t>(nflags));
+	mc.seg_bits.zero(s);
+	mc.plane_flags.zero(s);
+	DevBuf<unsigned long long> counts(2);
+	counts.zero(s);
+	FI_LAUNCH(minv_table_kernel<T>, 1, kThreads, 0, s, g, to_dev<T>(t), mc.table.data());
+	const dim3 grid(std::min(div_up(g.size[0], kThreads), 64), div_up(g.size[1], kDiagRows), g.nzl);
+	FI_REQUIRE(grid.y <= 65535 && grid.z <= 65535, FI_ERR_RANGE, "lattice too large along y or z for the M^-1 flag kernel's grid");
+	FI_LAUNCH(minv_flags_kernel<T>, grid, kThreads, 0, s, g, minv, static_cast<const T*>(mc.table.data()), bg, mc.seg_bits.data(), mc.plane_flags.data());
+	FI_LAUNCH(minv_count_kernel, static_cast<int>(std::min<int64_t>(div_up(std::max(words, nflags), static_cast<int64_t>(kThreads)), sm_count() * 4)), kThreads, 0, s,
+	          words, static_cast<const uint32_t*>(mc.seg_bits.data()), nflags, static_cast<const uint8_t*>(mc.plane_flags.data()), counts.data());
+	unsigned long long h[2];
+	FI_CUDA(cudaMemcpyAsync(h, counts.data(), sizeof(h), cudaMemcpyDeviceToHost, s));
+	FI_CUDA(cudaEventRecord(e1, s));
+	FI_CUDA(cudaEventSynchronize(e1));
+	FI_CUDA(cudaEventElapsedTime(&mc.build_ms, e0, e1));
+	cudaEventDestroy(e0);
+	cudaEventDestroy(e1);
+	mc.segments            = div_up(g.N, static_cast<int64_t>(32));
+	mc.flagged_segments    = static_cast<int64_t>(h[0]);
+	mc.tile_planes         = nflags;
+	mc.flagged_tile_planes = static_cast<int64_t>(h[1]);
+	mc.tile_rows           = bg.rows;
+	mc.radius              = bg.radius;
+	mc.tile_x              = bg.tile_x;
+	mc.halo_x              = bg.halo_x;
+	mc.update_ok  = 2 * mc.flagged_segments <= mc.segments;
+	mc.stencil_ok = 2 * mc.flagged_tile_planes <= mc.tile_planes;
+	mc.of         = minv;
+}
+
+template <typename T>
+void minv_as_seen(const Geom& g, const T* minv, const MinvClasses<T>& mc, T* upd, T* sten, cudaStream_t s)
+{
+	BoxGeom bg{};
+	const bool have = mc.of == minv && minv != nullptr;
+	FI_REQUIRE(have, FI_ERR_UNSUPPORTED, "no M^-1 class table for this lattice");
+	bg.rows    = mc.tile_rows;
+	bg.radius  = mc.radius;
+	bg.tile_x  = mc.tile_x;
+	bg.halo_x  = mc.halo_x;
+	bg.tiles_x = div_up(g.size[0], bg.tile_x);
+	bg.tiles_y = div_up(g.size[1], bg.rows);
+	const int64_t npacks = g.N / MinvClassView<T>::V;
+	FI_LAUNCH(minv_seen_kernel<T>, static_cast<int>(std::max<int64_t>(1, std::min<int64_t>(div_up(npacks, static_cast<int64_t>(kThreads)), sm_count() * 8))),
+	          kThreads, 0, s, g, minv, mc.view(), bg, upd, sten);
+}
+
+template void build_minv_classes<float>(const Geom&, const StencilTables&, const float*, MinvClasses<float>&, cudaStream_t);
+template void build_minv_classes<double>(const Geom&, const StencilTables&, const double*, MinvClasses<double>&, cudaStream_t);
+template void minv_as_seen<float>(const Geom&, const float*, const MinvClasses<float>&, float*, float*, cudaStream_t);
+template void minv_as_seen<double>(const Geom&, const double*, const MinvClasses<double>&, double*, double*, cudaStream_t);
+
 int stencil_partial_slots(const Geom& g) { return div_up(g.N, kThreads) + 8; }
 
 template <typename T>
diff --git a/field_interpolation_b200/csrc/stencil_tma.cu b/field_interpolation_b200/csrc/stencil_tma.cu
--- a/field_interpolation_b200/csrc/stencil_tma.cu
+++ b/field_interpolation_b200/csrc/stencil_tma.cu
@@ -24,24 +24,29 @@
 	static constexpr int BOX_BYTES  = BXP * BY * 16;
 };
 
-template <typename T, int R, int S, bool Fused, bool GS, int TY = 8>
+constexpr int kMcWords = 32;
+
+template <typename T, int R, int S, bool Fused, bool GS, int TY = 8, bool MC = false>
 constexpr size_t smem_bytes()
 {
 	using G = Tile<T, R, TY>;
 	return 128  + static_cast<size_t>(S) * (Fused ? 3 : 1) * G::TILE_BYTES + static_cast<size_t>(G::ring(GS)) * G::TILE_BYTES +
-	       S * sizeof(uint64_t) + 9 * (2 * R + 1) * sizeof(T) + 32 * sizeof(double) + 64;
-}
-
-template <typename T, int R, int S, bool Fused, int MINB, bool Epi, bool GS, int TY>
+	       S * sizeof(uint64_t) + 9 * (2 * R + 1) * sizeof(T) + 32 * sizeof(double) + 64 +
+	       (MC ? 81 * MinvClassView<T>::NPX * 16 + kMcWords * 4 + S * 4 + 16 : 0);
+}
+
+template <typename T, int R, int S, bool Fused, int MINB, bool Epi, bool GS, int TY, bool MC = false>
 __global__ void __launch_bounds__(256, MINB)
     stencil3d_tma_kernel(const __grid_constant__ CUtensorMap map_a,
                          const __grid_constant__ CUtensorMap map_b,
                          const __grid_constant__ CUtensorMap map_c,
                          int nx, int ny, int nzl, int zo0, int zo1, int zoff, int nzg, int zchunk, TmaTables<T> tab, T gs2,
                          T* __restrict__ q, T* __restrict__ p_new,
-                         const PcgState* st, int par, double* dot_out, double* partial, unsigned* ticket, const int* done, EpiArgs<T> epi)
+                         const PcgState* st, int par, double* dot_out, double* partial, unsigned* ticket, const int* done, EpiArgs<T> epi,
+                         MinvClassView<T> mc)
 {
 	static_assert(!(Fused && Epi), "the epilogue mode takes a plain input");
+	static_assert(Fused || !MC, "the class table replaces the M^-1 stage of the fused mode");
 	using G           = Tile<T, R, TY>;
 	constexpr int V   = G::V;
 	constexpr int NP  = G::NP;
@@ -65,6 +70,10 @@
 	uint64_t* full  = reinterpret_cast<uint64_t*>(ring_base + static_cast<size_t>(RING) * G::TILE_BYTES);
 	T*        zband = reinterpret_cast<T*>(full + S);
 	double*   red   = reinterpret_cast<double*>((reinterpret_cast<uintptr_t>(zband + 9 * W) + 7) & ~uintptr_t(7));
+	constexpr int NPX = MinvClassView<T>::NPX;
+	Pack*     mtab  = reinterpret_cast<Pack*>((reinterpret_cast<uintptr_t>(red + 32) + 15) & ~uintptr_t(15));
+	uint32_t* mbits = reinterpret_cast<uint32_t*>(mtab + 81 * NPX);
+	int*      mstage = reinterpret_cast<int*>(mbits + kMcWords);
 
 	const int tid = threadIdx.x, tx = tid & 31, ty = tid >> 5;
 	const int x0t = blockIdx.x * (G::TXP * V);
@@ -114,12 +123,23 @@
 
 	const int lp0    = zb - R;
 	const int n_iter = ze + R - lp0;
+	if (MC) {
+		for (int k = tid; k < 81 * NPX; k += 256) { mtab[k] = reinterpret_cast<const Pack*>(mc.table)[k]; }
+		const uint8_t* pf = mc.plane_flags + (static_cast<size_t>(blockIdx.y) * gridDim.x + blockIdx.x) * nzl;
+		for (int w = ty; w < kMcWords; w += 8) {
+			const int      i = w * 32 + tx, lp = lp0 + i;
+			const unsigned b = __ballot_sync(0xffffffffu, i < n_iter && lp >= 0 && lp < nzl && pf[lp] != 0);
+			if (tx == 0) { mbits[w] = b; }
+		}
+	}
 	auto issue = [&](int i) {
-		const int s = i % S;
-		mbar_expect_tx(&full[s], NA * G::BOX_BYTES);
+		const int  s = i % S;
+		const bool load_m = !MC || ((mbits[i >> 5] >> (i & 31)) & 1u);
+		if (MC) { mstage[s] = load_m ? 1 : 0; }
+		mbar_expect_tx(&full[s], (Fused && !load_m ? NA - 1 : NA) * G::BOX_BYTES);
 		tma_load_3d(stage_ptr(s, 0), &map_a, &full[s], x0t - NP * V, y0t - R, lp0 + i);
 		if (Fused) {
-			tma_load_3d(stage_ptr(s, 1), &map_b, &full[s], x0t - NP * V, y0t - R, lp0 + i);
+			if (load_m) { tma_load_3d(stage_ptr(s, 1), &map_b, &full[s], x0t - NP * V, y0t - R, lp0 + i); }
 			tma_load_3d(stage_ptr(s, 2), &map_c, &full[s], x0t - NP * V, y0t - R, lp0 + i);
 		}
 	};
@@ -140,11 +160,15 @@
 	const bool has_ch = GS && has_yh && tx < 2 * NP;
 	const int  ch_at  = yh_row * G::BXP + (tx < NP ? tx : G::TXP + tx);
 
-	auto direction = [&](const Pack* sa, const Pack* sb, const Pack* sc, int at) -> Pack {
+	const int bx0 = x0t - NP * V, by0 = y0t - R;
+	auto slot_of = [&](int at) { return MC ? minv_slot<V>(bx0 + (at % G::BXP) * V, by0 + at / G::BXP, nx, ny) : 0; };
+	const int own_m = slot_of(own_at), yh_m = slot_of(yh_at), xh_m = slot_of(xh_at), ch_m = slot_of(ch_at);
+
+	auto direction = [&](const Pack* sa, const Pack* sb, const Pack* sc, int at, const Pack* mt, int m_at) -> Pack {
 		if (!Fused) { return sa[at]; }
 		PU rr, mm, pp, out;
 		rr.v = sa[at];
-		mm.v = sb[at];
+		mm.v = MC && mt ? mt[m_at] : sb[at];
 		pp.v = sc[at];
 #pragma unroll
 		for (int j = 0; j < V; ++j) { out.a[j] = mm.a[j] * rr.a[j] + beta * pp.a[j]; }
@@ -182,13 +206,14 @@
 			const Pack* sb = Fused ? stage_ptr(stage, 1) : nullptr;
 			const Pack* sc = Fused ? stage_ptr(stage, 2) : nullptr;
 			Pack*       rg = ring_ptr(slot);
+			const Pack* mt = MC && !mstage[stage] ? mtab + minv_plane_slot<V>(lp + zoff, nzg) : nullptr;
 			if (has_own) {
-				pipe[k].v  = direction(sa, sb, sc, own_at);
+				pipe[k].v  = direction(sa, sb, sc, own_at, mt, own_m);
 				rg[own_at] = pipe[k].v;
 			}
-			if (has_yh) { rg[yh_at] = direction(sa, sb, sc, yh_at); }
-			if (has_xh) { rg[xh_at] = direction(sa, sb, sc, xh_at); }
-			if (has_ch) { rg[ch_at] = direction(sa, sb, sc, ch_at); }
+			if (has_yh) { rg[yh_at] = direction(sa, sb, sc, yh_at, mt, yh_m); }
+			if (has_xh) { rg[xh_at] = direction(sa, sb, sc, xh_at, mt, xh_m); }
+			if (has_ch) { rg[ch_at] = direction(sa, sb, sc, ch_at, mt, ch_m); }
 			if (Fused && in_xy && lp >= wlo && lp < whi) { *reinterpret_cast<Pack*>(pout + static_cast<size_t>(lp) * plane) = pipe[k].v; }
 			__syncthreads();
 			if (tid == 0 && i + S < n_iter) { issue(i + S); }
@@ -374,7 +399,8 @@
 
 template <typename T, int R, int S, bool Fused, int MINB, bool Epi, bool GS, int TY>
 void launch_ty(const Geom& g, const StencilTables& t, int chunks, const T* a, const T* b, const T* c, T* q, T* p_new, const PcgState* st, int par,
-               double* d_dot_out, double* d_partial, unsigned* d_ticket, const int* d_done, cudaStream_t s, const EpiArgs<T>& epi)
+               double* d_dot_out, double* d_partial, unsigned* d_ticket, const int* d_done, cudaStream_t s, const EpiArgs<T>& epi,
+               const MinvClasses<T>* mcl)
 {
 	using G = Tile<T, R, TY>;
 	TmaTables<T> tab;
@@ -391,20 +417,27 @@
 	const int zchunk  = div_up(nown, chunks);
 	chunks            = div_up(nown, zchunk);
 	dim3 grid(tiles_x, tiles_y, chunks);
-	auto kern = stencil3d_tma_kernel<T, R, S, Fused, MINB, Epi, GS, TY>;
-	constexpr size_t smem = smem_bytes<T, R, S, Fused, GS, TY>();
+	auto run = [&](auto kern, size_t smem, bool& configured, const MinvClassView<T>& v) {
+		if (!configured) {
+			FI_CUDA(cudaFuncSetAttribute(kern, cudaFuncAttributeMaxDynamicSharedMemorySize, static_cast<int>(smem)));
+			configured = true;
+		}
+		FI_LAUNCH(kern, grid, 256, smem, s, ma, mb, mc, g.size[0], g.size[1], g.nzl, g.zown0, g.zown1, g.zoff, g.size[2], zchunk, tab,
+		          static_cast<T>(t.gs2), q, p_new, st, par, d_dot_out, d_partial, d_ticket, d_done, epi, v);
+	};
+	if constexpr (Fused) {
+		if (mcl && mcl->for_stencil(b) && mcl->tile_rows == TY && mcl->radius == R && zchunk + 2 * R <= 32 * kMcWords) {
+			static bool configured = false;
+			run(stencil3d_tma_kernel<T, R, S, Fused, MINB, Epi, GS, TY, true>, smem_bytes<T, R, S, Fused, GS, TY, true>(), configured, mcl->view());
+			return;
+		}
+	}
 	static bool configured = false;
-	if (!configured) {
-		FI_CUDA(cudaFuncSetAttribute(kern, cudaFuncAttributeMaxDynamicSharedMemorySize, static_cast<int>(smem)));
-		configured = true;
-	}
-	FI_LAUNCH(kern, grid, 256, smem, s, ma, mb, mc, g.size[0], g.size[1], g.nzl, g.zown0, g.zown1, g.zoff, g.size[2], zchunk, tab,
-	          static_cast<T>(t.gs2), q, p_new, st, par, d_dot_out, d_partial, d_ticket, d_done, epi);
-}
-
-template <typename T, int R, int S, bool Fused, int MINB, bool Epi, bool GS>
-void launch_gs(const Geom& g, const StencilTables& t, const T* a, const T* b, const T* c, T* q, T* p_new, const PcgState* st, int par,
-               double* d_dot_out, double* d_partial, unsigned* d_ticket, const int* d_done, cudaStream_t s, const EpiArgs<T>& epi = EpiArgs<T>())
+	run(stencil3d_tma_kernel<T, R, S, Fused, MINB, Epi, GS, TY>, smem_bytes<T, R, S, Fused, GS, TY>(), configured, MinvClassView<T>());
+}
+
+template <typename T, int R, int S, int MINB>
+int tile_rows(const Geom& g, int* chunks)
 {
 	using G8 = Tile<T, R, 8>;
 	int c8 = 1, c7 = 1;
@@ -423,23 +456,35 @@
 		};
 		seven = forced == 7 || (forced != 8 && busiest(7, c7) < 0.97 * busiest(8, c8));
 	}
+	*chunks = seven ? c7 : c8;
+	return seven ? 7 : 8;
+}
+
+template <typename T, int R, int S, bool Fused, int MINB, bool Epi, bool GS>
+void launch_gs(const Geom& g, const StencilTables& t, const T* a, const T* b, const T* c, T* q, T* p_new, const PcgState* st, int par,
+               double* d_dot_out, double* d_partial, unsigned* d_ticket, const int* d_done, cudaStream_t s, const EpiArgs<T>& epi,
+               const MinvClasses<T>* mcl)
+{
+	int chunks = 1;
+	const int rows = tile_rows<T, R, S, MINB>(g, &chunks);
 	if constexpr (R <= 2) {
-		if (seven) {
-			launch_ty<T, R, S, Fused, MINB, Epi, GS, 7>(g, t, c7, a, b, c, q, p_new, st, par, d_dot_out, d_partial, d_ticket, d_done, s, epi);
+		if (rows == 7) {
+			launch_ty<T, R, S, Fused, MINB, Epi, GS, 7>(g, t, chunks, a, b, c, q, p_new, st, par, d_dot_out, d_partial, d_ticket, d_done, s, epi, mcl);
 			return;
 		}
 	}
-	launch_ty<T, R, S, Fused, MINB, Epi, GS, 8>(g, t, c8, a, b, c, q, p_new, st, par, d_dot_out, d_partial, d_ticket, d_done, s, epi);
+	launch_ty<T, R, S, Fused, MINB, Epi, GS, 8>(g, t, chunks, a, b, c, q, p_new, st, par, d_dot_out, d_partial, d_ticket, d_done, s, epi, mcl);
 }
 
 template <typename T, int R, int S, bool Fused, int MINB, bool Epi = false>
 void launch(const Geom& g, const StencilTables& t, const T* a, const T* b, const T* c, T* q, T* p_new, const PcgState* st, int par,
-            double* d_dot_out, double* d_partial, unsigned* d_ticket, const int* d_done, cudaStream_t s, const EpiArgs<T>& epi = EpiArgs<T>())
+            double* d_dot_out, double* d_partial, unsigned* d_ticket, const int* d_done, cudaStream_t s, const EpiArgs<T>& epi = EpiArgs<T>(),
+            const MinvClasses<T>* mcl = nullptr)
 {
 	if (t.gs2 != 0.0) {
-		launch_gs<T, R, S, Fused, MINB, Epi, true>(g, t, a, b, c, q, p_new, st, par, d_dot_out, d_partial, d_ticket, d_done, s, epi);
+		launch_gs<T, R, S, Fused, MINB, Epi, true>(g, t, a, b, c, q, p_new, st, par, d_dot_out, d_partial, d_ticket, d_done, s, epi, mcl);
 	} else {
-		launch_gs<T, R, S, Fused, MINB, Epi, false>(g, t, a, b, c, q, p_new, st, par, d_dot_out, d_partial, d_ticket, d_done, s, epi);
+		launch_gs<T, R, S, Fused, MINB, Epi, false>(g, t, a, b, c, q, p_new, st, par, d_dot_out, d_partial, d_ticket, d_done, s, epi, mcl);
 	}
 }
 
@@ -451,29 +496,64 @@
 	       (g.sharded() || g.size[2] >= 8) && encode_fn() != nullptr;
 }
 
+inline int stencil_variant()
+{
+	static const int variant = [] {
+		const char* e = getenv("FI_B200_STENCIL_VARIANT");
+		return e ? atoi(e) : 0;
+	}();
+	return variant;
+}
+
+template <int R_, int S_, int MINB_>
+struct Cfg
+{
+	static constexpr int R = R_, S = S_, MINB = MINB_;
+};
+template <typename T, typename F>
+void with_config(const StencilTables& t, F&& f)
+{
+	if (t.radius <= 1) {
+		f(Cfg<1, 3, 2>{});
+	} else if (t.radius == 2) {
+		if (stencil_variant() == 3 && std::is_same<T, float>::value) {
+			f(Cfg<2, 2, 3>{});
+		} else if (stencil_variant() == 4 && std::is_same<T, float>::value) {
+			f(Cfg<2, 4, 2>{});
+		} else {
+			f(Cfg<2, 3, 2>{});
+		}
+	} else {
+		f(Cfg<4, 2, 1>{});
+	}
+}
+
 template <typename T, bool Fused>
 void dispatch(const Geom& g, const StencilTables& t, const T* a, const T* b, const T* c, T* q, T* p_new, const PcgState* st, int par,
-              double* d_dot_out, double* d_partial, unsigned* d_ticket, const int* d_done, cudaStream_t s)
-{
-	if (t.radius <= 1) {
-		launch<T, 1, 3, Fused, 2>(g, t, a, b, c, q, p_new, st, par, d_dot_out, d_partial, d_ticket, d_done, s);
-	} else if (t.radius == 2) {
-		static const int variant = [] {
-			const char* e = getenv("FI_B200_STENCIL_VARIANT");
-			return e ? atoi(e) : 0;
-		}();
-		if (variant == 3 && std::is_same<T, float>::value) {
-			launch<T, 2, 2, Fused, 3>(g, t, a, b, c, q, p_new, st, par, d_dot_out, d_partial, d_ticket, d_done, s);
-		} else if (variant == 4 && std::is_same<T, float>::value) {
-			launch<T, 2, 4, Fused, 2>(g, t, a, b, c, q, p_new, st, par, d_dot_out, d_partial, d_ticket, d_done, s);
-		} else {
-			launch<T, 2, 3, Fused, 2>(g, t, a, b, c, q, p_new, st, par, d_dot_out, d_partial, d_ticket, d_done, s);
-		}
-	} else {
-		launch<T, 4, 2, Fused, 1>(g, t, a, b, c, q, p_new, st, par, d_dot_out, d_partial, d_ticket, d_done, s);
-	}
-}
-
+              double* d_dot_out, double* d_partial, unsigned* d_ticket, const int* d_done, cudaStream_t s, const MinvClasses<T>* mcl = nullptr)
+{
+	with_config<T>(t, [&](auto cfg) {
+		using C = decltype(cfg);
+		launch<T, C::R, C::S, Fused, C::MINB>(g, t, a, b, c, q, p_new, st, par, d_dot_out, d_partial, d_ticket, d_done, s, EpiArgs<T>(), mcl);
+	});
+}
+
+}
+
+template <typename T>
+bool stencil_tma_3d_fused_box(const Geom& g, const StencilTables& t, int* rows, int* radius, int* tile_x, int* halo_x)
+{
+	if (!eligible<T>(g, t)) { return false; }
+	with_config<T>(t, [&](auto cfg) {
+		using C   = decltype(cfg);
+		using G   = Tile<T, C::R, 8>;
+		int chunks = 1;
+		*rows   = tile_rows<T, C::R, C::S, C::MINB>(g, &chunks);
+		*radius = C::R;
+		*tile_x = G::TXP * G::V;
+		*halo_x = G::NP * G::V;
+	});
+	return true;
 }
 
 template <typename T>
@@ -488,10 +568,10 @@
 template <typename T>
 bool stencil_tma_3d_fused(const Geom& g, const StencilTables& t, const T* r, const T* minv, const T* p_old, T* p_new, T* q,
                           const PcgState* st, int par, double* d_dot_out, double* d_partial, unsigned* d_ticket, const int* d_done,
-                          cudaStream_t s)
+                          cudaStream_t s, const MinvClasses<T>* mcl)
 {
 	if (!eligible<T>(g, t)) { return false; }
-	dispatch<T, true>(g, t, r, minv, p_old, q, p_new, st, par, d_dot_out, d_partial, d_ticket, d_done, s);
+	dispatch<T, true>(g, t, r, minv, p_old, q, p_new, st, par, d_dot_out, d_partial, d_ticket, d_done, s, mcl);
 	return true;
 }
 
@@ -521,7 +601,9 @@
 template bool stencil_tma_3d_epilogue<float>(const Geom&, const StencilTables&, const float*, const float*, float*, const float*, float*, float*, float, float, cudaStream_t);
 template bool stencil_tma_3d<float>(const Geom&, const StencilTables&, const float*, float*, double*, double*, unsigned*, const int*, cudaStream_t);
 template bool stencil_tma_3d<double>(const Geom&, const StencilTables&, const double*, double*, double*, double*, unsigned*, const int*, cudaStream_t);
-template bool stencil_tma_3d_fused<float>(const Geom&, const StencilTables&, const float*, const float*, const float*, float*, float*, const PcgState*, int, double*, double*, unsigned*, const int*, cudaStream_t);
-template bool stencil_tma_3d_fused<double>(const Geom&, const StencilTables&, const double*, const double*, const double*, double*, double*, const PcgState*, int, double*, double*, unsigned*, const int*, cudaStream_t);
-
-}
+template bool stencil_tma_3d_fused<float>(const Geom&, const StencilTables&, const float*, const float*, const float*, float*, float*, const PcgState*, int, double*, double*, unsigned*, const int*, cudaStream_t, const MinvClasses<float>*);
+template bool stencil_tma_3d_fused<double>(const Geom&, const StencilTables&, const double*, const double*, const double*, double*, double*, const PcgState*, int, double*, double*, unsigned*, const int*, cudaStream_t, const MinvClasses<double>*);
+template bool stencil_tma_3d_fused_box<float>(const Geom&, const StencilTables&, int*, int*, int*, int*);
+template bool stencil_tma_3d_fused_box<double>(const Geom&, const StencilTables&, int*, int*, int*, int*);
+
+}
diff --git a/include/fi_b200.h b/include/fi_b200.h
--- a/include/fi_b200.h
+++ b/include/fi_b200.h
@@ -106,6 +106,7 @@
 FI_API int fi_field_use_fast_stencil(fi_field* f, int32_t enable);
 FI_API int fi_field_rhs(fi_field* f, int32_t precision, void* atb);
 FI_API int fi_field_diagonal(fi_field* f, int32_t precision, void* diag);
+FI_API int fi_field_preconditioner(fi_field* f, int32_t precision, void* minv, void* minv_update, void* minv_stencil, double* stats);
 
 FI_API int fi_field_solve(fi_field* f, const fi_solve_options* opt, const float* guess, float* solution, int32_t loc,
                    fi_solve_stats* stats);
```
